# ML200/RoyalTracer-DX

Hardware: AMD Instinct MI355X
Metric: Mrays/s + ms/frame at 1080p, 8-bounce Cornell Box (higher is better)
Workload: dtype f32; 1 GPU; cornell_1080p_64spp_8b; scene=generated: Cornell Box (32 triangles, 2 emissive), width=1920, height=1080, spp=64, max_bounces=8, nee_samples=1, rr_start=3, flags=1, triangles=32, parallelism=pixel-tiles/1, tile_size=64

## Files before the change

### include/rtx.h

```cpp
#ifndef RTX_H
#define RTX_H
#include <stdint.h>
#include <stddef.h>

#ifdef __cplusplus
extern "C" {
#endif

#define RTX_OK               0
#define RTX_ERR_INVALID     -1
#define RTX_ERR_NO_DEVICE   -2
#define RTX_ERR_HIP         -3
#define RTX_ERR_STATE       -4
#define RTX_ERR_OOM         -5

typedef struct rtx_ctx rtx_ctx;

typedef struct rtx_params {
    uint32_t width, height;
    uint32_t spp;
    uint32_t sample_base;
    uint32_t max_bounces;
    uint32_t nee_samples;
    uint32_t rr_start;
// ... 17 lines not shown
typedef struct rtx_stats {
    uint64_t rays_primary, rays_extension, rays_shadow;
    uint64_t paths;
    double   kernel_ms[RTX_K_COUNT];
    uint64_t kernel_launches[RTX_K_COUNT];
    uint64_t kernel_items[RTX_K_COUNT];
    double   render_ms;
    uint32_t bvh_nodes, triangles, lights, materials;
    uint64_t primary_hits;
    uint32_t bvh_refits, bvh_refs;
    uint64_t restir_stale_history_reads;
} rtx_stats;

enum { RTX_OPT_KERNEL_TIMING = 1,
       RTX_OPT_PATHS_PER_BATCH = 2,
       RTX_OPT_SORT_MATERIALS = 3,
       RTX_OPT_LDS_NODES = 4,
       RTX_OPT_SMALL_SCENE = 5,
       RTX_OPT_FUSED_BOUNCE = 6,
       RTX_OPT_BOUNCE_VARIANT = 7,
       RTX_OPT_REFILL_MIN = 8,
       RTX_OPT_STACK_PRIVATE = 9,
       RTX_OPT_TRACE_SCHED = 10,
       RTX_OPT_GPU_REFIT = 11,
       RTX_OPT_RESTIR_WAVEFRONT = 19,
       RTX_OPT_OCCLUDER_CACHE = 21,
       RTX_OPT_SHADE_DENSE = 23,
       RTX_OPT_RESTIR_LANES = 22,
       RTX_OPT_RESTIR_LANE_MIN = 29,
       RTX_OPT_RESTIR_CHUNKS = 20,
       RTX_OPT_OVERLAP_SHADOW = 18,
       RTX_OPT_COMPACT_STATE = 16,
       RTX_OPT_WORK_STEALING = 15,
       RTX_OPT_FUSED_BVH = 14,
       RTX_OPT_LPT_ORDER = 13,
       RTX_OPT_TAPER = 25,
       RTX_OPT_MERGE_RAYS = 24,
       RTX_OPT_OCTANT_SORT = 32,
       RTX_OPT_PARTIAL_REFIT = 37,
       RTX_OPT_LDS_NODES_CLOSEST = 36,
       RTX_OPT_RESTIR_KEYS = 35,
       RTX_OPT_NODE_STRIDE = 34,
       RTX_OPT_SAMPLE_INTERLEAVE = 33,
       RTX_OPT_ASYNC = 31,
       RTX_OPT_TRACE_COUNTERS = 30,
       RTX_OPT_BVH_REINSERT = 26,
       RTX_OPT_BVH_SPLIT = 27,
       RTX_OPT_ANYHIT_ORDER = 28,
       RTX_OPT_GPU_BUILD = 38,
       RTX_OPT_DEFORM_REBUILD = 40,
       RTX_OPT_STACK_CAP = 39,
       RTX_OPT_SHARED_PRIMARY = 41,
       RTX_OPT_DENOISE_LDS_STEP = 42,
       RTX_OPT_BLOCKS_PER_CU = 12     };

int  rtx_create(int device_ordinal, rtx_ctx** out);
void rtx_destroy(rtx_ctx*);
const char* rtx_last_error(rtx_ctx*);
int  rtx_set_option(rtx_ctx*, int option, int64_t value);
int  rtx_set_stream(rtx_ctx*, void* hip_stream);

int  rtx_set_materials(rtx_ctx*, const void* mats128, uint32_t count);
int  rtx_add_mesh(rtx_ctx*, const void* verts28, uint32_t nverts, const uint32_t* indices, uint32_t nidx,
                  const uint32_t* material_ids, uint32_t* mesh_out);
int  rtx_add_instance(rtx_ctx*, uint32_t mesh, const float o2w[16], uint32_t* inst_out);
int  rtx_set_instance_transform(rtx_ctx*, uint32_t inst, const float o2w[16]);
int  rtx_set_instance_visible(rtx_ctx*, uint32_t inst, int visible);
int  rtx_update_mesh_vertices(rtx_ctx*, uint32_t mesh, const void* verts28, uint32_t nverts);
#define RTX_TEX_SRGB 1u
enum { RTX_MAP_KD = 0, RTX_MAP_OPACITY = 2 };
enum { RTX_MAP_NORMAL = 4 };
int  rtx_set_mesh_uvs(rtx_ctx*, uint32_t mesh, const float* uv2 , uint32_t nidx);
int  rtx_set_texture(rtx_ctx*, uint32_t tex , const void* rgba8, uint32_t width, uint32_t height, uint32_t flags);
int  rtx_set_material_map(rtx_ctx*, uint32_t material, uint32_t slot, int32_t tex );
int  rtx_debug_texture_sample(rtx_ctx*, uint32_t tex, const float* uv2, uint32_t n, float* out4);
int  rtx_debug_albedo(rtx_ctx*, const float* rays8, const float* hits4, uint32_t n, float* out4);
int  rtx_debug_opacity(rtx_ctx*, const float* hits4, uint32_t n, float* out2);
int  rtx_debug_shading_normal(rtx_ctx*, const float* rays8, const float* hits4, uint32_t n, float* out4);
int  rtx_debug_tri_tangents(rtx_ctx*, uint32_t first, uint32_t count, float* out6);
#define RTX_ENV_HIDDEN 1u
int  rtx_set_environment(rtx_ctx*, const float* rgb32f , uint32_t n, const float env_to_world[16] , float scale, uint32_t flags);
int  rtx_debug_env_sample(rtx_ctx*, const uint32_t* seeds2, uint32_t n, float* out12);
int  rtx_debug_env_eval(rtx_ctx*, const float* dirs3, uint32_t n, float* out8);
int  rtx_debug_env_tables(rtx_ctx*, float* texels4, float* marginal, float* conditional);
int  rtx_commit_scene(rtx_ctx*);
int  rtx_save_scene_cache(rtx_ctx*, const char* path);
int  rtx_load_scene_cache(rtx_ctx*, const char* path);
int  rtx_set_camera(rtx_ctx*, const float view[16], const float proj[16]);
typedef struct rtx_lens {
    float    aperture_radius;
    float    focus_distance;
    uint32_t reserved[2];
} rtx_lens;
int  rtx_set_lens(rtx_ctx*, const rtx_lens* );
int  rtx_focus_distance_at(rtx_ctx*, uint32_t width, uint32_t height, uint32_t x, uint32_t y, float* distance_out);

int  rtx_bind_accum(rtx_ctx*, void* device_rgba32f, size_t bytes);
int  rtx_clear_accum(rtx_ctx*, uint32_t width, uint32_t height);
int  rtx_render(rtx_ctx*, const rtx_params*);
typedef struct rtx_adaptive {
    uint32_t min_spp, step_spp, max_spp;
    float    threshold, dark_floor;
    uint32_t reserved[3];
} rtx_adaptive;
typedef struct rtx_adaptive_result {
    uint32_t passes;
// ... 73 lines not shown
```

### include/rtx_host.h

```cpp
#ifndef RTX_HOST_H
#define RTX_HOST_H
#include "rtx.h"
#ifdef __cplusplus
extern "C" {
#endif

typedef struct rtxh_scene rtxh_scene;

rtxh_scene* rtxh_scene_cornell(void);
rtxh_scene* rtxh_scene_sponza_class(uint32_t target_tris, uint32_t seed);
rtxh_scene* rtxh_scene_bistro_class(uint32_t target_tris, uint32_t seed);
rtxh_scene* rtxh_scene_sponza_class_hard(uint32_t target_tris, uint32_t seed);
rtxh_scene* rtxh_scene_bistro_class_hard(uint32_t target_tris, uint32_t seed);
rtxh_scene* rtxh_scene_from_obj(const char* const* files, uint32_t nfiles, const char* mtl_dir);
#define RTXH_OBJ_NO_TEXTURES 1u
#define RTXH_OBJ_NO_CUTOUTS  2u
#define RTXH_OBJ_KD_ALPHA    4u
#define RTXH_OBJ_NO_NORMAL_MAPS  8u
#define RTXH_OBJ_BUMP_AS_NORMAL 16u
#define RTXH_OBJ_NORMAL_FLIP_Y  32u
rtxh_scene* rtxh_scene_from_obj_ex(const char* const* files, uint32_t nfiles, const char* mtl_dir, uint32_t flags);
rtxh_scene* rtxh_scene_from_obj_ex2(const char* const* files, uint32_t nfiles, const char* mtl_dir, uint32_t flags, float bump_height);
int         rtxh_scene_save(const rtxh_scene*, const char* path);
rtxh_scene* rtxh_scene_load(const char* path);
void        rtxh_scene_free(rtxh_scene*);
const char* rtxh_last_error(void);

uint32_t    rtxh_scene_num_materials(const rtxh_scene*);
const void* rtxh_scene_materials(const rtxh_scene*);
#define RTXH_NUM_MAP_SLOTS 13
enum { RTXH_MAP_KA = 0, RTXH_MAP_KD, RTXH_MAP_KS, RTXH_MAP_KE, RTXH_MAP_NS, RTXH_MAP_BUMP, RTXH_MAP_D, RTXH_MAP_DISP, RTXH_MAP_REFL, RTXH_MAP_PR, RTXH_MAP_PM, RTXH_MAP_PS, RTXH_MAP_NORM };
typedef struct rtxh_material_ext { float Ni, Ns, Pcr, aniso, anisor; int32_t illum; float Ka[3], Tf[3]; int32_t map[RTXH_NUM_MAP_SLOTS]; } rtxh_material_ext;
int         rtxh_scene_material_ext(const rtxh_scene*, uint32_t material, rtxh_material_ext* out);
uint32_t    rtxh_scene_num_textures(const rtxh_scene*);
const char* rtxh_scene_texture(const rtxh_scene*, uint32_t i);
int         rtxh_scene_texture_pixels(const rtxh_scene*, uint32_t i, const void** rgba8, uint32_t* width, uint32_t* height);
int         rtxh_scene_opacity_map(const rtxh_scene*, uint32_t material);
int         rtxh_scene_normal_map(const rtxh_scene*, uint32_t material);
int         rtxh_scene_mesh_uvs(const rtxh_scene*, uint32_t i, const float** uv2, uint32_t* nidx);
int         rtxh_read_image(const char* path, void* rgba8, uint64_t capacity, uint32_t* width, uint32_t* height);
int         rtxh_read_hdr_image(const char* path, float* rgb32f, uint64_t capacity, uint32_t* width, uint32_t* height);
int         rtxh_env_from_latlong(const float* rgb32f, uint32_t width, uint32_t height, uint32_t n, float* out);
uint32_t    rtxh_scene_num_meshes(const rtxh_scene*);
int         rtxh_scene_mesh(const rtxh_scene*, uint32_t i, const void** verts28, uint32_t* nverts,
                            const uint32_t** indices, uint32_t* nidx, const uint32_t** material_ids);
uint32_t    rtxh_scene_num_instances(const rtxh_scene*);
int         rtxh_scene_instance(const rtxh_scene*, uint32_t i, uint32_t* mesh, float o2w[16]);
uint64_t    rtxh_scene_num_triangles(const rtxh_scene*);
int         rtxh_scene_set_mesh_vertices(rtxh_scene*, uint32_t mesh, const void* verts28, uint32_t nverts);
int         rtxh_scene_camera(const rtxh_scene*, float eye[3], float center[3], float up[3], float* fovy_deg, float* zn, float* zf);
int         rtxh_scene_set_camera(rtxh_scene*, const float eye[3], const float center[3], const float up[3]);
int         rtxh_scene_view_proj(const rtxh_scene*, float aspect, float view[16], float proj[16]);
int         rtxh_scene_upload(const rtxh_scene*, rtx_ctx*, float aspect);

void rtxh_lookat(const float eye[3], const float center[3], const float up[3], float view16[16]);
void rtxh_perspective_fov_rh(float fovy_rad, float aspect, float zn, float zf, float proj16[16]);
void rtxh_generate_ess_lut(float roughness, float lut16[16]);
void rtxh_mat4_inverse(const float m16[16], float out16[16]);
float rtxh_half_round(float x);
int  rtxh_bvh_check(const float* world_tris9, uint32_t ntris, uint32_t* nodes_out, uint32_t* depth_out, uint32_t* max_leaf_out);
int  rtxh_bvh8_check(const float* world_tris9, uint32_t ntris, uint32_t* nodes8_out, uint32_t* stack_out);
int  rtxh_bvh8_stats(const float* world_tris9, uint32_t ntris, uint32_t hist[6], uint32_t* nodes8_out);
int  rtxh_bvh_option(const char* key, double value);
int  rtxh_bvh_replay(const float* world_tris9, uint32_t ntris, const float* rays8, uint32_t nrays, int any, uint32_t any_order, float* out4, uint32_t* refs_out);
int  rtxh_bvh_refit_check(const float* before_tris9, const float* after_tris9, uint32_t ntris);

int  rtxh_scene_small_records(const rtxh_scene*, float* recs20, int32_t* tri_ids2, uint32_t max_recs, uint32_t* nrec_out, float* delta_out, float* cm_out);
int  rtxh_scene_small_occluders(const rtxh_scene*, uint32_t* nocc_out);
int  rtxh_scene_anyhit_order(const rtxh_scene*, uint32_t* order_out);

typedef struct rtxh_renderer rtxh_renderer;
rtxh_renderer* rtxh_renderer_create(uint32_t width, uint32_t height, const char* name, int device);
int  rtxh_renderer_set_scene(rtxh_renderer*, const rtxh_scene*);
rtx_params* rtxh_renderer_params(rtxh_renderer*);
int  rtxh_renderer_set_mode(rtxh_renderer*, int mode);
rtx_params* rtxh_renderer_restir_params(rtxh_renderer*);
rtx_ctx* rtxh_renderer_context(rtxh_renderer*);
int  rtxh_renderer_on_init(rtxh_renderer*);
int  rtxh_renderer_on_update(rtxh_renderer*);
int  rtxh_renderer_set_instance_transform(rtxh_renderer*, uint32_t instance, const float o2w[16]);
int  rtxh_renderer_set_instance_visible(rtxh_renderer*, uint32_t instance, int visible);
int  rtxh_renderer_set_mesh_vertices(rtxh_renderer*, uint32_t mesh, const void* verts28, uint32_t nverts);
int  rtxh_renderer_on_render(rtxh_renderer*);
int  rtxh_renderer_read_accum(rtxh_renderer*, float* rgba32f, size_t bytes);
int  rtxh_renderer_read_output(rtxh_renderer*, uint8_t* rgba8, size_t bytes);
int  rtxh_renderer_on_key_up(rtxh_renderer*, uint8_t key);
uint32_t rtxh_renderer_display_layer(const rtxh_renderer*);
void rtxh_renderer_destroy(rtxh_renderer*);

int  rtxh_write_png(const char* path, const uint8_t* rgba8, uint32_t width, uint32_t height);
int  rtxh_write_ppm(const char* path, const uint8_t* rgba8, uint32_t width, uint32_t height);
int  rtxh_write_exr(const char* path, const float* rgba32f_accum, uint32_t width, uint32_t height);

#ifdef __cplusplus
}
#endif
#endif
```

### royaltracer-dx_amd/__init__.py

```python
import ctypes as C
import os
import numpy as np

_HERE = os.path.dirname(os.path.abspath(__file__))
LIB_PATH = os.environ.get("RTX_LIB_PATH") or os.path.join(_HERE, "librtx_hip.so")

if not os.path.exists(LIB_PATH):
    raise ImportError(
        f"{LIB_PATH} is missing: build it with `make -C {_HERE}` (hipcc --offload-arch=gfx950) "
        "or `python -c 'import __graft_entry__ as g; g.build()'`.  There is no CPU fallback.")

if os.environ.get("RTX_NO_TORCH_PRELOAD", "0") != "1":
    try:
        import torch
    except Exception:
        pass

lib = C.CDLL(LIB_PATH)

RTX_OK = 0
FLAG_LAMBERT_ONLY = 1
FLAG_JITTER = 2
FLAG_TRANSMISSION = 4
FLAG_BLOCK_TILES = 8
K_RAYGEN, K_TRACE, K_SHADE, K_SHADOW, K_ACCUM, K_SORT, K_BOUNCE, K_ADAPT, K_COUNT = 0, 1, 2, 3, 4, 5, 6, 7, 8
KERNEL_NAMES = {K_RAYGEN: "raygen", K_TRACE: "trace_closest", K_SHADE: "shade", K_SHADOW: "trace_shadow", K_ACCUM: "accumulate", K_SORT: "sort", K_BOUNCE: "bounce_fused", K_ADAPT: "adaptive"}
OPT_KERNEL_TIMING, OPT_PATHS_PER_BATCH, OPT_SORT_MATERIALS, OPT_LDS_NODES, OPT_SMALL_SCENE, OPT_FUSED_BOUNCE, OPT_BOUNCE_VARIANT = 1, 2, 3, 4, 5, 6, 7
OPT_REFILL_MIN, OPT_STACK_PRIVATE, OPT_TRACE_SCHED, OPT_GPU_REFIT, OPT_BLOCKS_PER_CU, OPT_LPT_ORDER, OPT_FUSED_BVH, OPT_WORK_STEALING, OPT_COMPACT_STATE, OPT_OVERLAP_SHADOW = 8, 9, 10, 11, 12, 13, 14, 15, 16, 18
OPT_RESTIR_WAVEFRONT, OPT_RESTIR_CHUNKS, OPT_OCCLUDER_CACHE, OPT_RESTIR_LANES, OPT_SHADE_DENSE, OPT_MERGE_RAYS, OPT_TAPER = 19, 20, 21, 22, 23, 24, 25
OPT_BVH_REINSERT, OPT_BVH_SPLIT, OPT_ANYHIT_ORDER, OPT_RESTIR_LANE_MIN, OPT_TRACE_COUNTERS, OPT_ASYNC, OPT_OCTANT_SORT, OPT_SAMPLE_INTERLEAVE, OPT_NODE_STRIDE, OPT_RESTIR_KEYS, OPT_LDS_NODES_CLOSEST, OPT_PARTIAL_REFIT = 26, 27, 28, 29, 30, 31, 32, 33, 34, 35, 36, 37
OPT_GPU_BUILD = 38
OPT_STACK_CAP = 39
OPT_DEFORM_REBUILD = 40
OPT_SHARED_PRIMARY = 41
OPT_DENOISE_LDS_STEP = 42
TEX_SRGB = 1
MAP_KD = 0
MAP_OPACITY = 2
MAP_NORMAL = 4
ENV_HIDDEN = 1


class RtxError(RuntimeError):
    pass


class Params(C.Structure):
    _fields_ = [(n, C.c_uint32) for n in (
        "width", "height", "spp", "sample_base", "max_bounces", "nee_samples", "rr_start",
        "frame_seed", "flags", "tile_size", "shard_rank", "shard_count")]

    def __init__(self, width=1920, height=1080, spp=1, sample_base=1, max_bounces=8, nee_samples=1,
                 rr_start=3, frame_seed=1, flags=0, tile_size=64, shard_rank=0, shard_count=1):
        super().__init__(width, height, spp, sample_base, max_bounces, nee_samples, rr_start,
                         frame_seed, flags, tile_size, shard_rank, shard_count)

    def copy(self, **kw):
        d = {n: getattr(self, n) for n, _ in self._fields_}
        d.update(kw)
        return Params(**d)


class Stats(C.Structure):
    _fields_ = [("rays_primary", C.c_uint64), ("rays_extension", C.c_uint64), ("rays_shadow", C.c_uint64),
                ("paths", C.c_uint64), ("kernel_ms", C.c_double * K_COUNT), ("kernel_launches", C.c_uint64 * K_COUNT),
                ("kernel_items", C.c_uint64 * K_COUNT), ("render_ms", C.c_double),
                ("bvh_nodes", C.c_uint32), ("triangles", C.c_uint32), ("lights", C.c_uint32), ("materials", C.c_uint32),
                ("primary_hits", C.c_uint64), ("bvh_refits", C.c_uint32), ("bvh_refs", C.c_uint32), ("restir_stale_history_reads", C.c_uint64)]

    @property
    def rays(self):
        return self.rays_primary + self.rays_extension + self.rays_shadow


_vp, _u32, _fp = C.c_void_p, C.c_uint32, C.POINTER(C.c_float)
_u32p = C.POINTER(C.c_uint32)


def _sig(name, restype, *argtypes):
    f = getattr(lib, name)
    f.restype = restype
    f.argtypes = list(argtypes)
    return f


_sig("rtx_create", C.c_int, C.c_int, C.POINTER(_vp))
_sig("rtx_destroy", None, _vp)
_sig("rtx_last_error", C.c_char_p, _vp)
# ... 98 lines not shown
_sig("rtxh_scene_bistro_class", _vp, _u32, _u32)
_sig("rtxh_scene_sponza_class_hard", _vp, _u32, _u32)
_sig("rtxh_scene_bistro_class_hard", _vp, _u32, _u32)
_sig("rtxh_scene_from_obj", _vp, C.POINTER(C.c_char_p), _u32, C.c_char_p)
_sig("rtxh_scene_from_obj_ex", _vp, C.POINTER(C.c_char_p), _u32, C.c_char_p, _u32)
_sig("rtxh_scene_opacity_map", C.c_int, _vp, _u32)
_sig("rtxh_scene_from_obj_ex2", _vp, C.POINTER(C.c_char_p), _u32, C.c_char_p, _u32, C.c_float)
_sig("rtxh_scene_normal_map", C.c_int, _vp, _u32)
_sig("rtxh_scene_free", None, _vp)
_sig("rtxh_scene_save", C.c_int, _vp, C.c_char_p)
_sig("rtxh_scene_load", _vp, C.c_char_p)
_sig("rtxh_last_error", C.c_char_p)
_sig("rtxh_scene_num_materials", _u32, _vp)
_sig("rtxh_scene_materials", _vp, _vp)
class MaterialExt(C.Structure):
    _fields_ = [("Ni", C.c_float), ("Ns", C.c_float), ("Pcr", C.c_float), ("aniso", C.c_float), ("anisor", C.c_float), ("illum", C.c_int32),
                ("Ka", C.c_float * 3), ("Tf", C.c_float * 3), ("map", C.c_int32 * 13)]


MAP_SLOTS = ("Ka", "Kd", "Ks", "Ke", "Ns", "bump", "d", "disp", "refl", "Pr", "Pm", "Ps", "norm")
_sig("rtxh_scene_material_ext", C.c_int, _vp, _u32, C.POINTER(MaterialExt))
_sig("rtxh_scene_num_textures", _u32, _vp)
_sig("rtxh_scene_texture", C.c_char_p, _vp, _u32)
_sig("rtxh_scene_texture_pixels", C.c_int, _vp, _u32, C.POINTER(_vp), _u32p, _u32p)
_sig("rtxh_scene_mesh_uvs", C.c_int, _vp, _u32, C.POINTER(_vp), _u32p)
_sig("rtxh_read_image", C.c_int, C.c_char_p, _vp, C.c_uint64, _u32p, _u32p)
_sig("rtxh_read_hdr_image", C.c_int, C.c_char_p, _vp, C.c_uint64, _u32p, _u32p)
_sig("rtxh_env_from_latlong", C.c_int, _vp, _u32, _u32, _u32, _vp)
_sig("rtxh_scene_num_meshes", _u32, _vp)
_sig("rtxh_scene_mesh", C.c_int, _vp, _u32, C.POINTER(_vp), _u32p, C.POINTER(_vp), _u32p, C.POINTER(_vp))
_sig("rtxh_scene_num_instances", _u32, _vp)
_sig("rtxh_scene_instance", C.c_int, _vp, _u32, _u32p, _fp)
_sig("rtxh_scene_num_triangles", C.c_uint64, _vp)
_sig("rtxh_scene_camera", C.c_int, _vp, _fp, _fp, _fp, _fp, _fp, _fp)
_sig("rtxh_scene_view_proj", C.c_int, _vp, C.c_float, _fp, _fp)
_sig("rtxh_scene_upload", C.c_int, _vp, _vp, C.c_float)
_sig("rtxh_lookat", None, _fp, _fp, _fp, _fp)
_sig("rtxh_perspective_fov_rh", None, C.c_float, C.c_float, C.c_float, C.c_float, _fp)
_sig("rtxh_generate_ess_lut", None, C.c_float, _fp)
_sig("rtxh_mat4_inverse", None, _fp, _fp)
_sig("rtxh_half_round", C.c_float, C.c_float)
_sig("rtxh_bvh_check", C.c_int, _vp, _u32, _u32p, _u32p, _u32p)
_sig("rtxh_bvh_refit_check", C.c_int, _vp, _vp, _u32)
_sig("rtxh_bvh8_check", C.c_int, _vp, _u32, _u32p, _u32p)
_sig("rtxh_bvh8_stats", C.c_int, _vp, _u32, _vp, _u32p)
_sig("rtxh_bvh_option", C.c_int, C.c_char_p, C.c_double)
_sig("rtxh_bvh_replay", C.c_int, _vp, _u32, _vp, _u32, C.c_int, _u32, _vp, _u32p)
_sig("rtxh_scene_small_occluders", C.c_int, _vp, _u32p)
_sig("rtxh_scene_anyhit_order", C.c_int, _vp, _u32p)
_sig("rtxh_write_png", C.c_int, C.c_char_p, _vp, _u32, _u32)
_sig("rtxh_write_ppm", C.c_int, C.c_char_p, _vp, _u32, _u32)
_sig("rtxh_write_exr", C.c_int, C.c_char_p, _vp, _u32, _u32)
_sig("rtxh_scene_small_records", C.c_int, _vp, _vp, _vp, _u32, _u32p, _fp, _fp)
_sig("rtxh_scene_set_camera", C.c_int, _vp, _fp, _fp, _fp)
_sig("rtxh_scene_set_mesh_vertices", C.c_int, _vp, _u32, _vp, _u32)
_sig("rtxh_renderer_set_mesh_vertices", C.c_int, _vp, _u32, _vp, _u32)
_sig("rtxh_renderer_create", _vp, _u32, _u32, C.c_char_p, C.c_int)
_sig("rtxh_renderer_set_scene", C.c_int, _vp, _vp)
_sig("rtxh_renderer_params", C.POINTER(Params), _vp)
_sig("rtxh_renderer_restir_params", C.POINTER(Params), _vp)
_sig("rtxh_renderer_set_mode", C.c_int, _vp, C.c_int)
_sig("rtxh_renderer_context", _vp, _vp)
_sig("rtxh_renderer_on_init", C.c_int, _vp)
_sig("rtxh_renderer_on_update", C.c_int, _vp)
_sig("rtxh_renderer_set_instance_transform", C.c_int, _vp, _u32, _vp)
_sig("rtxh_renderer_set_instance_visible", C.c_int, _vp, _u32, C.c_int)
_sig("rtxh_renderer_on_render", C.c_int, _vp)
_sig("rtxh_renderer_read_accum", C.c_int, _vp, _vp, C.c_size_t)
_sig("rtxh_renderer_read_output", C.c_int, _vp, _vp, C.c_size_t)
_sig("rtxh_renderer_on_key_up", C.c_int, _vp, C.c_uint8)
_sig("rtxh_renderer_display_layer", _u32, _vp)
_sig("rtxh_renderer_destroy", None, _vp)


def _f32(a):
    return np.ascontiguousarray(a, dtype=np.float32)


def _ptr(a):
    return a.ctypes.data_as(_vp)


def _fptr(a):
    return a.ctypes.data_as(_fp)


class Scene:

    def __init__(self, handle):
        if not handle:
            raise RtxError("scene creation failed: " + lib.rtxh_last_error().decode())
        self._h = handle
        n = lib.rtxh_scene_num_materials(handle)
        buf = (C.c_float * (n * 32)).from_address(lib.rtxh_scene_materials(handle)) if n else []
        self.materials = np.array(buf, dtype=np.float32).reshape(n, 32)
        self.textures = [lib.rtxh_scene_texture(handle, i).decode() for i in range(lib.rtxh_scene_num_textures(handle))]
        self.material_ext = []
        for i in range(n):
            x = MaterialExt()
            if lib.rtxh_scene_material_ext(handle, i, C.byref(x)) != RTX_OK:
                break
            self.material_ext.append(dict(Ni=x.Ni, Ns=x.Ns, Pcr=x.Pcr, aniso=x.aniso, anisor=x.anisor, illum=x.illum, Ka=list(x.Ka), Tf=list(x.Tf),
                                          maps={MAP_SLOTS[k]: self.textures[x.map[k]] for k in range(13) if x.map[k] >= 0}))
        self.texture_pixels = []
        for i in range(len(self.textures)):
            px, tw, th = _vp(), _u32(), _u32()
# ... 50 lines not shown
        if bump is not None and bump != "normal":
            return cls(lib.rtxh_scene_from_obj_ex2(arr, len(files), mtl_dir.encode(), flags, float(bump)))
        return cls(lib.rtxh_scene_from_obj_ex(arr, len(files), mtl_dir.encode(), flags))

    def set_camera(self, eye, center, up=(0.0, 1.0, 0.0)):
        e, c, u = (np.asarray(v, np.float32) for v in (eye, center, up))
        lib.rtxh_scene_set_camera(self._h, _fptr(e), _fptr(c), _fptr(u))
        self.eye, self.center, self.up = e, c, u

    def set_mesh_vertices(self, mesh, verts):
        v = _f32(verts).reshape(-1, 7)
        if lib.rtxh_scene_set_mesh_vertices(self._h, int(mesh), _ptr(v), len(v)) != RTX_OK:
            raise RtxError("rtxh_scene_set_mesh_vertices failed: " + lib.rtxh_last_error().decode())
        old = self.meshes[mesh]
        self.meshes[mesh] = (v.copy(), old[1], old[2])
        self.cache_path = None

    def bounds(self):
        lo, hi = np.full(3, np.inf, np.float32), np.full(3, -np.inf, np.float32)
        for mesh, m in self.instances:
            v = self.meshes[mesh][0][:, :3]
            if len(v):
                M = np.asarray(m, np.float32).reshape(4, 4)
                w = v @ M[:3, :3] + M[3, :3]
                lo, hi = np.minimum(lo, w.min(0)), np.maximum(hi, w.max(0))
        return lo, hi

    def frame_bounds(self):
        lo, hi = self.bounds()
        c, ext = (lo + hi) * 0.5, hi - lo
        ax = 0 if ext[0] >= ext[2] else 2
        eye, ctr = c.copy(), c.copy()
        eye[1] = ctr[1] = lo[1] + 0.4 * ext[1]
        eye[ax] = c[ax] - 0.35 * ext[ax]
        self.set_camera(eye, ctr)

    def save(self, path):
        if lib.rtxh_scene_save(self._h, str(path).encode()) != RTX_OK:
            raise RtxError("rtxh_scene_save failed: " + lib.rtxh_last_error().decode())

    @classmethod
    def load(cls, path):
        s = cls(lib.rtxh_scene_load(str(path).encode()))
        s.cache_path = str(path)
        return s

    def small_records(self):
        recs, ids = np.zeros((64, 20), np.float32), np.zeros((64, 2), np.int32)
        n, d, cm = _u32(), C.c_float(), C.c_float()
        if lib.rtxh_scene_small_records(self._h, _ptr(recs), _ptr(ids), 64, C.byref(n), C.byref(d), C.byref(cm)) != RTX_OK or n.value == 0:
            return None
        return recs[:n.value], ids[:n.value], d.value, cm.value

    def small_occluders(self):
        n = _u32()
        if lib.rtxh_scene_small_occluders(self._h, C.byref(n)) != RTX_OK:
            raise RtxError("rtxh_scene_small_occluders failed")
        return n.value

    def anyhit_order(self):
        n = _u32()
        if lib.rtxh_scene_anyhit_order(self._h, C.byref(n)) != RTX_OK:
            raise RtxError("rtxh_scene_anyhit_order failed")
        return n.value

    def view_proj(self, aspect):
        v, p = np.zeros(16, np.float32), np.zeros(16, np.float32)
        lib.rtxh_scene_view_proj(self._h, C.c_float(aspect), _fptr(v), _fptr(p))
        return v, p


def lookat(eye, center, up):
    e, c, u, v = _f32(eye), _f32(center), _f32(up), np.zeros(16, np.float32)
    lib.rtxh_lookat(_fptr(e), _fptr(c), _fptr(u), _fptr(v))
    return v


def perspective_fov_rh(fovy_rad, aspect, zn, zf):
    p = np.zeros(16, np.float32)
    lib.rtxh_perspective_fov_rh(fovy_rad, aspect, zn, zf, _fptr(p))
    return p


def generate_ess_lut(roughness):
    lut = np.zeros(16, np.float32)
    lib.rtxh_generate_ess_lut(roughness, _fptr(lut))
    return lut


def mat4_inverse(m):
    m, o = _f32(m).reshape(16), np.zeros(16, np.float32)
    lib.rtxh_mat4_inverse(_fptr(m), _fptr(o))
    return o


def half_round(x):
    return lib.rtxh_half_round(C.c_float(x))


def read_image(path):
    w, h = _u32(), _u32()
    if lib.rtxh_read_image(str(path).encode(), None, 0, C.byref(w), C.byref(h)) != RTX_OK:
        raise RtxError("read_image: " + lib.rtxh_last_error().decode())
    out = np.zeros((h.value, w.value, 4), np.uint8)
    lib.rtxh_read_image(str(path).encode(), _ptr(out), out.nbytes, C.byref(w), C.byref(h))
    return out
# ... 579 lines not shown
```

### royaltracer-dx_amd/csrc/rtx_api.hip

```cpp
#include "rtx_ctx.hpp"
#include <cmath>

thread_local std::string g_create_err;

void options_to_scene(rtx_ctx* c, bool committed) {
    DevScene& s = c->dsc; const rtx_ctx::Options& o = c->opt;
    s.trace_cnt = o.trace_counters ? (unsigned long long*)c->d_trace_cnt.p : nullptr;
    s.refill_min = o.refill_min; s.trace_sched = o.trace_sched; s.sort_materials = o.sort_materials; s.occluder_cache = o.occluder_cache; s.shade_dense = o.shade_dense > 0 ? 1u : 0u;
    if (committed) {
        s.any_order = o.any_order_opt < 0 ? c->scene.built.any_order : (uint32_t)o.any_order_opt;
        s.any_order_occ = o.any_order_opt < 0 ? 0u : (uint32_t)o.any_order_opt;
    }
}

int render_checks(rtx_ctx* c, const rtx_params* p, bool zero_bounces_ok, DevFrame& f) {
    BIND(c);
    if (!c->committed) { c->err = "render: scene not committed"; return RTX_ERR_STATE; }
    if (!c->camera_set) { c->err = "render: camera not set"; return RTX_ERR_STATE; }
    const int r = make_frame(c, p, f);
    if (r) return r;
    if (zero_bounces_ok) {
        if (p->max_bounces > 64 || p->nee_samples > 16) { c->err = "params: max_bounces <= 64, nee_samples <= 16"; return RTX_ERR_INVALID; }
        return RTX_OK;
    }
    if (p->max_bounces == 0 || p->max_bounces > 64) { c->err = "params: max_bounces must be in [1, 64]"; return RTX_ERR_INVALID; }
    if (p->nee_samples > 16) { c->err = "params: nee_samples must be <= 16"; return RTX_ERR_INVALID; }
    return RTX_OK;
}
void stats_begin(rtx_ctx* c) {
    memset(c->stats.kernel_ms, 0, sizeof(c->stats.kernel_ms));
    memset(c->stats.kernel_launches, 0, sizeof(c->stats.kernel_launches));
    memset(c->stats.kernel_items, 0, sizeof(c->stats.kernel_items));
    c->stats.rays_primary = c->stats.rays_extension = c->stats.rays_shadow = c->stats.paths = c->stats.primary_hits = 0; c->stats.render_ms = 0;
    c->ev.used = 0; c->timed.clear();
}

int ensure_accum(rtx_ctx* c, uint32_t w, uint32_t h, bool clear) {
    const size_t need = (size_t)w * h * 16;
    if (c->ext_accum) {
        if (c->ext_accum_bytes < need) { c->err = "bound accumulation buffer is smaller than width*height*16 bytes"; return RTX_ERR_INVALID; }
    } else {
        const bool fresh = !c->d_accum.p || c->acc_w != w || c->acc_h != h;
        HIPCHK(c, c->d_accum.ensure(need));
        clear = clear || fresh;
    }
    c->acc_w = w; c->acc_h = h;
    if (clear) { HIPCHK(c, hipMemsetAsync(c->accum_ptr(), 0, need, c->stream)); c->ad.pure = true; c->ad.cleared = true; }
    return RTX_OK;
}

static void block_grid(uint64_t TX, uint64_t TY, uint32_t N, uint32_t& gx, uint32_t& gy) {
    double best = 1e300; gx = N; gy = 1;
    for (uint32_t a = 1; a <= N; a++) {
        if (N % a) continue;
        const uint32_t b = N / a;
        const double cost = (double)((TX + a - 1) / a) + (double)((TY + b - 1) / b);
        if (cost < best) { best = cost; gx = a; gy = b; }
    }
}
const char* validate_tiling(const rtx_params* p, uint32_t& ts, uint32_t& cnt, uint64_t& npl, uint32_t* gx_out, uint32_t* gy_out) {
    if (!p || !p->width || !p->height) return "params: width/height must be non-zero";
    ts = p->tile_size ? p->tile_size : 64;
    if (ts < 16 || ts > 1024 || (ts & (ts - 1))) return "params: tile_size must be a power of two in [16, 1024] (0 = 64)";
    cnt = p->shard_count ? p->shard_count : 1;
// ... 43 lines not shown
    if (e != hipSuccess || n <= 0) {
        g_create_err = std::string("no HIP device: ") + (e != hipSuccess ? hipGetErrorString(e) : "device count is 0") +
                       " (this library has no CPU fallback)";
        return RTX_ERR_NO_DEVICE;
    }
    if (device_ordinal < 0 || device_ordinal >= n) { g_create_err = "device ordinal out of range"; return RTX_ERR_NO_DEVICE; }
    if ((e = hipSetDevice(device_ordinal)) != hipSuccess) { g_create_err = hipGetErrorString(e); return RTX_ERR_NO_DEVICE; }
    rtx_ctx* c = new rtx_ctx();
    c->device = device_ordinal;
    hipDeviceProp_t prop;
    if (hipGetDeviceProperties(&prop, device_ordinal) == hipSuccess) c->num_cus = prop.multiProcessorCount;
    if ((e = c->streams.acquire(device_ordinal)) != hipSuccess) {
        g_create_err = hipGetErrorString(e); delete c; return RTX_ERR_HIP;
    }
    c->stream = c->streams.set.s[0]; c->own_stream = true;
    (void)hipEventCreate(&c->ev.begin); (void)hipEventCreate(&c->ev.end);
    *out = c;
    return RTX_OK;
}

void rtx_destroy(rtx_ctx* c) {
    if (!c) return;
    (void)hipSetDevice(c->device);
    if (c->own_stream && c->stream) (void)hipStreamSynchronize(c->stream);
    else (void)hipDeviceSynchronize();
    delete c;
}

const char* rtx_last_error(rtx_ctx* c) { return c ? c->err.c_str() : g_create_err.c_str(); }

int rtx_set_option(rtx_ctx* c, int option, int64_t value) {
    if (!c) return RTX_ERR_INVALID;
    switch (option) {
    case RTX_OPT_KERNEL_TIMING: c->opt.timing = value != 0; return RTX_OK;
    case RTX_OPT_ASYNC: c->opt.async = value != 0; return RTX_OK;
    case RTX_OPT_OCTANT_SORT: c->opt.octant_sort = (int)value; return RTX_OK;
    case RTX_OPT_NODE_STRIDE: if (value != 0 && value != 80 && value != 128) { c->err = "node stride must be 0 (auto), 80 or 128"; return RTX_ERR_INVALID; } if (c->opt.node_stride != (int)value) { c->opt.node_stride = (int)value; c->committed = false; } return RTX_OK;
    case RTX_OPT_RESTIR_KEYS: c->opt.restir_keys = value != 0; return RTX_OK;
    case RTX_OPT_SAMPLE_INTERLEAVE: c->opt.sample_interleave = value != 0; return RTX_OK;
    case RTX_OPT_TRACE_COUNTERS:
        c->opt.trace_counters = value != 0;
        if (c->opt.trace_counters) { HIPCHK(c, c->d_trace_cnt.ensure(4 * sizeof(unsigned long long))); HIPCHK(c, hipMemsetAsync(c->d_trace_cnt.p, 0, 32, c->stream)); }
        options_to_scene(c, c->committed);
        return RTX_OK;
    case RTX_OPT_BVH_REINSERT: if (value < 0 || value > 16) { c->err = "bvh_reinsert must be in [0, 16]"; return RTX_ERR_INVALID; } c->host.bvh.reinsert_passes = (int)value; c->host.topo_dirty = true; c->committed = false; return RTX_OK;
    case RTX_OPT_BVH_SPLIT: if (value < 0 || value > 1000000000) { c->err = "bvh_split must be in [0, 1e9] (parts per billion of the scene's surface area)"; return RTX_ERR_INVALID; } c->host.bvh.split_alpha = (double)value * 1e-9; c->host.topo_dirty = true; c->committed = false; return RTX_OK;
    case RTX_OPT_ANYHIT_ORDER: if (value < -1 || value > 2) { c->err = "anyhit_order must be -1 (probe), 0, 1 or 2"; return RTX_ERR_INVALID; } c->opt.any_order_opt = (int)value; options_to_scene(c, c->committed); return RTX_OK;
    case RTX_OPT_PATHS_PER_BATCH: if (value < 4096) { c->err = "paths_per_batch must be >= 4096"; return RTX_ERR_INVALID; } c->opt.paths_per_batch = (uint64_t)value; return RTX_OK;
    case RTX_OPT_SORT_MATERIALS: c->opt.sort_materials = value != 0; options_to_scene(c, c->committed); return RTX_OK;
    case RTX_OPT_LDS_NODES: c->opt.lds_nodes_opt = (int)value; c->committed = false; return RTX_OK;
    case RTX_OPT_PARTIAL_REFIT: c->opt.partial_refit = value != 0; return RTX_OK;
    case RTX_OPT_LDS_NODES_CLOSEST: c->opt.lds_closest_opt = (int)value; if (c->committed) pick_lds_closest(c); return RTX_OK;
    case RTX_OPT_SMALL_SCENE: c->opt.small_scene = value != 0; c->committed = false; return RTX_OK;
    case RTX_OPT_FUSED_BOUNCE: c->opt.fused = value != 0; return RTX_OK;
    case RTX_OPT_BOUNCE_VARIANT: c->opt.bounce_variant = value == 2 ? 2 : (value != 0 ? 1 : 0); return RTX_OK;
    case RTX_OPT_SHARED_PRIMARY: c->opt.shared_primary = value != 0; return RTX_OK;
    case RTX_OPT_STACK_PRIVATE: c->opt.stack_private = (int)value; c->committed = false; return RTX_OK;
    case RTX_OPT_LPT_ORDER: c->opt.lpt_order = value != 0; return RTX_OK;
    case RTX_OPT_FUSED_BVH: c->opt.fused_bvh = value != 0; return RTX_OK;
    case RTX_OPT_WORK_STEALING: c->opt.work_stealing = value != 0; return RTX_OK;
    case RTX_OPT_COMPACT_STATE: c->opt.compact_state = value != 0; return RTX_OK;
    case RTX_OPT_OVERLAP_SHADOW: c->opt.overlap_shadow = value != 0; return RTX_OK;
    case RTX_OPT_BLOCKS_PER_CU: if (value < 0 || value > 64) { c->err = "blocks_per_cu must be in [0, 64]"; return RTX_ERR_INVALID; } c->opt.blocks_per_cu = (uint32_t)value; return RTX_OK;
    case RTX_OPT_TAPER: if (value < 0 || value > 8) { c->err = "taper must be in [0, 8]"; return RTX_ERR_INVALID; } c->opt.taper = value != 0; c->opt.taper_levels = value == 1 ? 4u : (uint32_t)std::max<long long>(value, 1); return RTX_OK;
    case RTX_OPT_MERGE_RAYS: if (value < 0 || value > (1 << 20)) { c->err = "merge_rays must be in [0, 2^20]"; return RTX_ERR_INVALID; } c->opt.merge_rays = (uint32_t)value; return RTX_OK;
    case RTX_OPT_GPU_REFIT: c->opt.gpu_refit = value != 0; return RTX_OK;
    case RTX_OPT_GPU_BUILD: c->opt.gpu_build = value != 0; return RTX_OK;
    case RTX_OPT_DEFORM_REBUILD: if (value < 0 || value > 1000000) { c->err = "deform_rebuild must be 0 (refit), 1 (rebuild) or a percentage >= 2"; return RTX_ERR_INVALID; } c->opt.deform_rebuild = (int)value; return RTX_OK;
    case RTX_OPT_STACK_CAP: if (value < 0 || value > 30 || (value > 0 && value < 4)) { c->err = "stack_cap must be 0 (the whole stack in LDS) or in [4, 30]"; return RTX_ERR_INVALID; } c->opt.stack_cap = (uint32_t)value; c->committed = false; return RTX_OK;
    case RTX_OPT_SHADE_DENSE: c->opt.shade_dense = (int)value; options_to_scene(c, c->committed); return RTX_OK;
    case RTX_OPT_OCCLUDER_CACHE: c->opt.occluder_cache = value != 0; options_to_scene(c, c->committed); return RTX_OK;
    case RTX_OPT_RESTIR_WAVEFRONT: c->opt.restir_wave = value != 0; return RTX_OK;
    case RTX_OPT_RESTIR_LANE_MIN: if (value < 256 || value > (1ll << 31)) { c->err = "restir_lane_min must be in [256, 2^31]"; return RTX_ERR_INVALID; } c->opt.restir_lane_min = (uint32_t)value; return RTX_OK;
    case RTX_OPT_RESTIR_LANES: if (value < 1 || value > 4) { c->err = "restir_lanes must be in [1, 4]"; return RTX_ERR_INVALID; } c->opt.restir_lanes = (uint32_t)value; return RTX_OK;
    case RTX_OPT_RESTIR_CHUNKS: if (value < 1 || value > 64) { c->err = "restir_chunks must be in [1, 64]"; return RTX_ERR_INVALID; } c->opt.restir_chunks = (uint32_t)value; return RTX_OK;
    case RTX_OPT_TRACE_SCHED: if (value > 7) { c->err = "trace_sched must be in [0, 7]"; return RTX_ERR_INVALID; } c->opt.trace_sched = (uint32_t)value; options_to_scene(c, c->committed); return RTX_OK;
    case RTX_OPT_REFILL_MIN: if (value < 1 || value > 64) { c->err = "refill_min must be in [1, 64]"; return RTX_ERR_INVALID; } c->opt.refill_min = (uint32_t)value; options_to_scene(c, c->committed); return RTX_OK;
    case RTX_OPT_DENOISE_LDS_STEP: if (value != 0 && value != 1 && value != 2 && value != 4) { c->err = "denoise_lds_step must be 0, 1, 2 or 4"; return RTX_ERR_INVALID; } c->dn.lds_step = (uint32_t)value; return RTX_OK;
    default: c->err = "unknown option"; return RTX_ERR_INVALID;
    }
}

int rtx_set_stream(rtx_ctx* c, void* s) {
    BIND(c);
    if (c->own_stream && c->stream) HIPCHK(c, hipStreamSynchronize(c->stream));
    else HIPCHK(c, hipDeviceSynchronize());
    if (c->own_stream) { c->stream = nullptr; c->own_stream = false; }
    if (s) { c->stream = (hipStream_t)s; c->own_stream = false; }
    else { c->stream = c->streams.set.s[0]; c->own_stream = true; }
    return RTX_OK;
}

int rtx_set_materials(rtx_ctx* c, const void* mats128, uint32_t count) {
    if (!c) return RTX_ERR_INVALID;
    if (!c->host.set_materials(mats128, count)) { c->err = c->host.err; return RTX_ERR_INVALID; }
    c->committed = false; return RTX_OK;
}
int rtx_add_mesh(rtx_ctx* c, const void* verts28, uint32_t nverts, const uint32_t* indices, uint32_t nidx, const uint32_t* material_ids, uint32_t* mesh_out) {
    if (!c) return RTX_ERR_INVALID;
    if (!c->host.add_mesh(verts28, nverts, indices, nidx, material_ids, mesh_out)) { c->err = c->host.err; return RTX_ERR_INVALID; }
    c->committed = false; return RTX_OK;
}
int rtx_add_instance(rtx_ctx* c, uint32_t mesh, const float o2w[16], uint32_t* inst_out) {
    if (!c || !o2w) return RTX_ERR_INVALID;
    if (!c->host.add_instance(mesh, o2w, inst_out)) { c->err = c->host.err; return RTX_ERR_INVALID; }
    c->committed = false; return RTX_OK;
// ... 151 lines not shown
```

### royaltracer-dx_amd/csrc/rtx_commit.hip

```cpp
#include "rtx_ctx.hpp"

void pick_lds_closest(rtx_ctx* c) {
    DevScene& s = c->dsc;
    c->scene.lds_nodes_closest = 0;
    const bool small_tree = (size_t)s.nnodes * sizeof(Node8GPU) <= ((size_t)16 << 20);
    if (!s.nsmall && s.nnodes > s.lds_nodes && c->opt.lds_nodes_opt < 0 && (c->opt.lds_closest_opt >= 0 || small_tree)) {
        auto fit1k = [&](uint32_t nodes) { DevScene t = s; t.lds_nodes = nodes; return (160u * 1024u) / (uint32_t)((trace_lds_bytes(t) + 64 + 1023) & ~(size_t)1023); };
        uint32_t n = c->opt.lds_closest_opt >= 0 ? std::min<uint32_t>((uint32_t)c->opt.lds_closest_opt, s.nnodes) : std::min<uint32_t>(73u, s.nnodes);
        if (c->opt.lds_closest_opt < 0) while (n > s.lds_nodes && fit1k(n) < 6u) n--;
        DevScene t = s; t.lds_nodes = n;
        if (n > s.lds_nodes && trace_lds_bytes(t) <= 64 * 1024) c->scene.lds_nodes_closest = n;
    }
}

extern "C" {

static int upload_lights(rtx_ctx* c) {
    const BuiltScene& B = c->scene.built;
    std::vector<float>& cdf = c->scene.h_cdf;
    cdf.resize(B.lights.size());
    for (size_t i = 0; i < cdf.size(); i++) cdf[i] = B.lights[i].cdf;
    int r = upload(c, c->scene.d_lights, B.lights);
    if (r) return r;
    return upload(c, c->scene.d_cdf, cdf);
}
static int upload_built(rtx_ctx* c) {
    BuiltScene& B = c->scene.built;
    int r;
    if ((r = upload(c, c->scene.d_nodes, B.nodes8))) return r;
    if ((r = upload(c, c->scene.d_tris, B.tris8))) return r;
    c->scene.n_nodes8 = (uint32_t)B.nodes8.size(); c->scene.n_tris8 = (uint32_t)B.tris8.size(); c->scene.dev_built = false;
    if (!B.nodes8.empty()) c->scene.root8 = B.nodes8[0]; else memset(&c->scene.root8, 0, sizeof(c->scene.root8));
    if ((r = upload(c, c->scene.d_shade, B.shade))) return r;
    if ((r = upload(c, c->scene.d_small, B.small_recs))) return r;
    if ((r = upload(c, c->scene.d_small_tris, B.small_tris))) return r;
    if ((r = upload(c, c->scene.d_small_poly, B.small_poly))) return r;
    if ((r = upload(c, c->scene.d_mats, B.mats))) return r;
    if ((r = upload(c, c->scene.d_insts, B.insts))) return r;
    return upload_lights(c);
}
static int finalise_scene(rtx_ctx* c);

static void fill_tex_lut(std::vector<float>& lut) {
    lut.resize(768);
    for (int b = 0; b < 256; b++) {
        lut[512 + b] = std::max(((float)b - 128.0f) / 127.0f, -1.0f);
        lut[b] = (float)b / 255.0f;
        const double cs = b / 255.0;
        lut[256 + b] = (float)(cs <= 0.04045 ? cs / 12.92 : pow((cs + 0.055) / 1.055, 2.4));
    }
}
static int sync_textures(rtx_ctx* c, bool renumbered, bool deformed) {
    SceneHost& H = c->host; rtx_ctx::Scene& S = c->scene;
    S.built.maps_active = H.maps_active();
    const bool cut = S.built.cutouts_active = H.cutouts_active();
    const bool nrm = S.built.normals_active = H.normals_active();
    const bool active = S.built.maps_active || cut || nrm;
    int r;
    if (H.tex_dirty) {
        std::vector<TexDesc> desc(H.textures.size()); std::vector<uint32_t> pool;
        for (size_t i = 0; i < H.textures.size(); i++) {
            const TexHost& t = H.textures[i];
            desc[i] = TexDesc{(uint32_t)pool.size(), t.width, t.height, t.flags};
            pool.insert(pool.end(), t.rgba.begin(), t.rgba.end());
        }
        std::vector<int32_t> maps(H.mats128.size() / 32, -1);
        for (size_t m = 0; m < maps.size() && m < H.map_kd.size(); m++) maps[m] = H.map_kd[m];
        if ((r = upload(c, S.d_tex_desc, desc)) || (r = upload(c, S.d_texels, pool)) || (r = upload(c, S.d_map_kd, maps))) return r;
        if (!H.any_normal_map()) S.d_map_nrm.release();
        else {
            std::vector<int32_t> nmaps(H.mats128.size() / 32, -1);
            for (size_t m = 0; m < nmaps.size() && m < H.map_normal.size(); m++) nmaps[m] = H.map_normal[m];
            if ((r = upload(c, S.d_map_nrm, nmaps))) return r;
        }
        if (!S.d_tex_lut.p) { std::vector<float> lut; fill_tex_lut(lut); if ((r = upload(c, S.d_tex_lut, lut))) return r; }
        S.ntex = (uint32_t)desc.size();
    }
    if (active && (H.tex_dirty || renumbered || !S.tri_uv_valid)) {
        std::vector<float> uv; H.fill_tri_uv(uv);
        if ((r = upload(c, S.d_tri_uv, uv))) return r;
        S.tri_uv_valid = true;
    }
    if (!active && S.tri_uv_valid) { S.d_tri_uv.release(); S.tri_uv_valid = false; }
    if (cut && (H.tex_dirty || renumbered || !S.tri_cut_valid)) {
        std::vector<int32_t> tc; H.fill_tri_cut(tc);
        if ((r = upload(c, S.d_tri_cut, tc))) return r;
        S.tri_cut_valid = true;
    }
    if (!cut && S.tri_cut_valid) { S.d_tri_cut.release(); S.tri_cut_valid = false; }
// ... 195 lines not shown
    for (uint32_t ord = 1; ord < 3u; ord++) if (cost[ord] < 0.95 * cost[0] && cost[ord] < cost[best_out]) best_out = ord;
    return RTX_OK;
}

static int refit_resident(rtx_ctx* c, bool deform) {
    BuiltScene& B = c->scene.built;
    int r;
    if (deform && (r = ensure_cost_baseline(c, nullptr))) return r;
    const bool mats_changed = c->host.mats_dirty;
    if (!c->host.refresh_transforms(B)) { c->err = c->host.err; return RTX_ERR_INVALID; }
    if (mats_changed && (r = upload(c, c->scene.d_mats, B.mats))) return r;
    if ((r = upload(c, c->scene.d_insts, B.insts))) return r;
    if ((r = upload_lights(c))) return r;
    if ((r = upload_objtris_once(c))) return r;
    if (deform) {
        if ((r = reflatten_dirty_meshes(c))) return r;
        if (!c->scene.dev_built) { B.objtris.clear(); B.objtris.shrink_to_fit(); c->scene.host_mirror_stale = true; }
    }
    HIPCHK(c, c->scene.d_node_aabb.ensure((size_t)c->scene.n_nodes8 * 32));
    size_t nmoved = 0; for (uint32_t m : B.inst_moved) nmoved += m;
    const bool partial = c->opt.partial_refit && c->scene.node_aabb_valid && B.inst_moved.size() == B.insts.size() && nmoved < B.insts.size();
    if (!partial) return full_refit(c);
    if ((r = upload(c, c->scene.d_inst_moved, B.inst_moved))) return r;
    if ((r = upload_hidden(c))) return r;
    HIPCHK(c, c->scene.d_tri_dirty.ensure(c->scene.n_tris8)); HIPCHK(c, c->scene.d_node_dirty.ensure(c->scene.n_nodes8));
    launch_refit(c->stream, (Node8GPU*)c->scene.d_nodes.p, B.level_start8.data(), (uint32_t)B.level_start8.size() - 1, (TriGPU*)c->scene.d_tris.p, c->scene.n_tris8,
                 (const TriShade*)c->scene.d_shade.p, (const InstGPU*)c->scene.d_insts.p, (const F4*)c->scene.d_objtris.p, (F4*)c->scene.d_node_aabb.p, (uint32_t*)c->scene.d_scale.p,
                 (const uint32_t*)c->scene.d_inst_moved.p, (uint8_t*)c->scene.d_tri_dirty.p, (uint8_t*)c->scene.d_node_dirty.p, hidden_words(c));
    HIPCHK(c, hipGetLastError());
    return RTX_OK;
}

static int build_and_upload(rtx_ctx* c) {
    BuiltScene& B = c->scene.built;
    int r;
    c->scene.device_scene_valid = false; c->scene.objtris_uploaded = false; c->scene.node_aabb_valid = false; c->scene.host_mirror_stale = false;
    size_t ntri_all = 0; for (const InstHost& in : c->host.insts) ntri_all += c->host.meshes[in.mesh].idx.size() / 3;
    const bool on_gpu = c->opt.gpu_build && ntri_all > 4096u && c->host.bvh.split_alpha <= 0.0;
    if (!(on_gpu ? c->host.prepare_device_build(B) : c->host.build(B))) { c->err = c->host.err; return RTX_ERR_INVALID; }
    if (!on_gpu) {
        if ((r = upload_built(c))) return r;
        if (B.any_hidden && c->scene.n_nodes8 && B.level_start8.size() >= 2) {
            if ((r = upload_objtris_once(c))) return r;
            if ((r = full_refit(c))) return r;
            TO_HOST(c, &c->scene.root8, c->scene.d_nodes.p, sizeof(Node8GPU));
        }
        return RTX_OK;
    }
    const uint32_t nt = B.built_tris;
    if ((r = upload(c, c->scene.d_mats, B.mats))) return r;
    if ((r = upload(c, c->scene.d_insts, B.insts))) return r;
    if ((r = upload_lights(c))) return r;
    if ((r = flatten_on_device(c, nt))) return r; c->scene.objtris_uploaded = true;
    for (DevBuf* b : {&c->scene.d_small, &c->scene.d_small_tris, &c->scene.d_small_poly}) HIPCHK(c, b->ensure(16));
    HIPCHK(c, c->scene.d_tris.ensure((size_t)nt * sizeof(TriGPU)));
    if (!c->scene.builder) c->scene.builder.reset(new GpuBvhBuilder());
    BvhBuildOptions bo = c->host.bvh; if (bo.ploc_radius <= 0) bo.ploc_radius = 16;
    const std::string e = c->scene.builder->build(c->stream, (const F4*)c->scene.d_objtris.p, (const TriShade*)c->scene.d_shade.p, (const InstGPU*)c->scene.d_insts.p, nt, bo, (TriGPU*)c->scene.d_tris.p, c->scene.build_info);
    if (!e.empty()) { c->err = e; return RTX_ERR_HIP; }
    const GpuBuildResult& G = c->scene.build_info;
    HIPCHK(c, c->scene.d_nodes.ensure((size_t)G.nnodes8 * sizeof(Node8GPU)));
    HIPCHK(c, hipMemcpyAsync(c->scene.d_nodes.p, c->scene.builder->nodes(), (size_t)G.nnodes8 * sizeof(Node8GPU), hipMemcpyDeviceToDevice, c->stream));
    c->scene.n_nodes8 = G.nnodes8; c->scene.n_tris8 = G.ntris8; c->scene.dev_built = true; B.bvh_pad = 2e-6f * G.scale;
    B.level_start8 = G.level_start8; B.stack8 = G.stack8;
    if ((r = full_refit(c))) return r;
    if (c->scene.n_nodes8) { if ((r = enqueue_tree_cost(c, c->scene.d_cost_base))) return r; c->scene.cost_base_state = 1; }
    TO_HOST(c, &c->scene.root8, c->scene.d_nodes.p, sizeof(Node8GPU));
    if (getenv("RTX_BUILD_TIMES")) fprintf(stderr, "[build] GPU: prims %.2f ms, sort %.2f ms, PLOC %.2f ms (%u rounds -> %u clusters), top on the host %.2f ms, layout %.2f ms: %u wide nodes, stack %u\n",
                                           G.ms_prims, G.ms_sort, G.ms_ploc, G.ploc_iterations, G.clusters_top, G.ms_top_host, G.ms_layout, G.nnodes8, G.stack8);
    return RTX_OK;
}

int rtx_commit_scene(rtx_ctx* c) {
    BIND(c);
    const bool deform = !c->host.dirty_meshes.empty();
    for (uint32_t m : c->host.dirty_meshes)
        if (m < c->scene.pool_meshes && std::find(c->scene.pool_dirty.begin(), c->scene.pool_dirty.end(), m) == c->scene.pool_dirty.end()) c->scene.pool_dirty.push_back(m);
    if (deform && c->opt.deform_rebuild == 1) c->host.topo_dirty = true;
    if (c->host.topo_dirty || c->host.mats_dirty || !c->scene.committed_once)
        for (size_t i = 0; i < c->host.matids.size(); i++)
            if (c->host.matids[i] >= c->host.mats128.size() / 32) { c->err = "commit: material id out of range"; return RTX_ERR_INVALID; }
    c->scene.committed_once = true;
    int r;
    {   size_t ntri_all = 0; for (const InstHost& in : c->host.insts) ntri_all += c->host.meshes[in.mesh].idx.size() / 3;
        if (c->host.tex_dirty && ntri_all <= kSmallSceneMaxTris && (c->host.maps_active() != c->scene.built.maps_active || c->host.cutouts_active() != c->scene.built.cutouts_active || c->host.normals_active() != c->scene.built.normals_active)) c->host.topo_dirty = true;
        if (c->host.env_dirty && ntri_all <= kSmallSceneMaxTris && (c->host.env.n != 0) != c->scene.built.env_active) c->host.topo_dirty = true; }
    bool build = !(c->opt.gpu_refit && gpu_refittable(c) && !c->host.topo_dirty);
    const BuiltScene& B0 = c->scene.built;
    if (!build && !c->scene.dev_built && !B0.leaf_order.empty() && B0.leaf_order.size() <= kSmallSceneMaxTris && B0.any_hidden && !c->host.any_hidden()) build = true;
    bool flipped = false;
    for (size_t ii = 0; ii < c->host.insts.size() && !flipped; ii++) flipped = (ii < B0.inst_hidden.size() && B0.inst_hidden[ii] != 0u) != c->host.is_hidden(ii);
    const bool tex_only = !build && (c->host.tex_dirty || c->host.env_dirty) && c->host.only_maps_changed(B0);
    const bool probe = (build || !flipped) && !tex_only;
    if (!build && !tex_only) {
        if ((r = refit_resident(c, deform))) return r;
        c->scene.cost_now_state = 0;
        if (deform && c->opt.deform_rebuild >= 2) {
            double cost[2];
            if ((r = tree_costs(c, cost))) return r;
            if (cost[0] * 100.0 > cost[1] * (double)c->opt.deform_rebuild) { c->host.topo_dirty = true; build = true; }
        }
    }
    if (build) {
        c->scene.cost_base_state = c->scene.cost_now_state = 0;
        if ((r = build_and_upload(c))) return r;
    }
    c->host.dirty_meshes.clear();
// ... 5 lines not shown
        if ((r = probe_anyhit_order_on_device(c, best))) return r;
        c->scene.built.any_order = best;
        if (c->opt.any_order_opt < 0) c->dsc.any_order = best;
    }
    return r;
}

int rtx_save_scene_cache(rtx_ctx* c, const char* path) {
    if (!c) return RTX_ERR_INVALID;
    if (!c->committed) { c->err = "save_scene_cache: scene not committed"; return RTX_ERR_STATE; }
    if (c->scene.host_mirror_stale) { c->err = "save_scene_cache: the per-triangle records were re-derived on the GPU after rtx_update_mesh_vertices and the host holds no current copy; commit with RTX_OPT_DEFORM_REBUILD 1 (host builder) to save a cache"; return RTX_ERR_STATE; }
    if (c->scene.built.any_hidden) { c->err = "save_scene_cache: an instance is hidden (rtx_set_instance_visible): the device's boxes and triangle records leave it out and the file format holds no visibility; show every instance and commit to save a cache"; return RTX_ERR_STATE; }
    if (c->host.env.n) { c->err = "save_scene_cache: an environment is bound (rtx_set_environment) and the file format holds no environment; clear it and commit to save a cache"; return RTX_ERR_STATE; }
    if (c->host.any_normal_map()) { c->err = "save_scene_cache: a material has a normal map (rtx_set_material_map, RTX_MAP_NORMAL) and the file format holds no texels; unmap every material and commit to save a cache"; return RTX_ERR_STATE; }
    if (c->host.any_opacity_map()) { c->err = "save_scene_cache: a material has an opacity map (rtx_set_material_map, RTX_MAP_OPACITY) and the file format holds no texels; unmap every material and commit to save a cache"; return RTX_ERR_STATE; }
    if (c->host.any_map()) { c->err = "save_scene_cache: a material has a texture map (rtx_set_material_map) and the file format holds no texels; unmap every material and commit to save a cache"; return RTX_ERR_STATE; }
    if (c->scene.dev_built) { c->err = "save_scene_cache: the tree was built on the GPU (RTX_OPT_GPU_BUILD) and has no host mirror; commit with the host builder to save a cache"; return RTX_ERR_STATE; }
    if (!save_scene_cache(c->host, c->scene.built, path, c->err)) return RTX_ERR_INVALID;
    return RTX_OK;
}
int rtx_load_scene_cache(rtx_ctx* c, const char* path) {
    BIND(c);
    if (!load_scene_cache(path, c->host, c->scene.built, c->err)) return RTX_ERR_INVALID;
    c->committed = false; c->scene.device_scene_valid = false; c->scene.objtris_uploaded = false; c->scene.node_aabb_valid = false;
    c->scene.host_mirror_stale = false; c->scene.cost_base_state = c->scene.cost_now_state = 0;
    c->scene.pool_meshes = 0; c->scene.pool_verts = c->scene.pool_idx = c->scene.pool_matids = 0; c->scene.pool_vert_base.clear(); c->scene.pool_idx_base.clear(); c->scene.pool_dirty.clear();
    int r = upload_built(c);
    if (r) return r;
    c->host.tex_dirty = true;
    if ((r = sync_textures(c, true, false))) return r;
    c->host.env = EnvHost{}; c->host.env_dirty = true;
    if ((r = sync_environment(c))) return r;
    return finalise_scene(c);
}

static int refresh_wide_nodes(rtx_ctx* c) {
    if (!c->scene.wide_nodes || !c->scene.n_nodes8) return RTX_OK;
    HIPCHK(c, c->scene.d_nodes_wide.ensure((size_t)c->scene.n_nodes8 * 128));
    HIPCHK(c, hipMemcpy2DAsync(c->scene.d_nodes_wide.p, 128, c->scene.d_nodes.p, sizeof(Node8GPU), sizeof(Node8GPU), c->scene.n_nodes8, hipMemcpyDeviceToDevice, c->stream));
    return RTX_OK;
}
static int finalise_scene(rtx_ctx* c) {
    BuiltScene& B = c->scene.built;
    HIPCHK(c, hipStreamSynchronize(c->stream));
    c->scene.device_scene_valid = true;
    DevScene& s = c->dsc;
    s.nodes = (const Node8GPU*)c->scene.d_nodes.p; s.nnodes = c->scene.n_nodes8;
    s.nodes_f = (const F4*)c->scene.d_nodes.p; s.node_v4 = 5u;
    c->scene.wide_nodes = s.nnodes && (c->opt.node_stride == 128 || (c->opt.node_stride == 0 && (size_t)s.nnodes * sizeof(Node8GPU) > ((size_t)16 << 20)));
    { const int rw = refresh_wide_nodes(c); if (rw) return rw; }
    if (c->scene.wide_nodes && c->opt.node_stride == 128) { s.nodes_f = (const F4*)c->scene.d_nodes_wide.p; s.node_v4 = 8u; }
    s.tris = (const TriGPU*)c->scene.d_tris.p; s.ntris = c->scene.n_tris8;
    s.shade = (const TriShade*)c->scene.d_shade.p;
    s.small = (const SmallRecPair*)c->scene.d_small.p; s.small_tris = (const TriGPU*)c->scene.d_small_tris.p; s.small_poly = (const F4*)c->scene.d_small_poly.p; s.small_cm = B.small_cm; s.small_delta = B.small_delta;
    s.mats = (const MatGPU*)c->scene.d_mats.p; s.nmat = (uint32_t)B.mats.size();
    s.insts = (const InstGPU*)c->scene.d_insts.p; s.ninst = (uint32_t)B.insts.size();
    s.lights = (const LightGPU*)c->scene.d_lights.p; s.nlights = (uint32_t)B.lights.size(); s.cdf = (const float*)c->scene.d_cdf.p;
    s.total_weight = B.total_weight;
    s.tex_desc = (const TexDesc*)c->scene.d_tex_desc.p; s.ntex = c->scene.ntex; s.texels = (const uint32_t*)c->scene.d_texels.p; s.tex_lut = (const float*)c->scene.d_tex_lut.p;
    s.env_n = c->host.env.n; s.env_flags = c->host.env.flags; memcpy(s.env_rot, c->host.env.rot, sizeof(s.env_rot));
    const bool env_lit = s.env_n && c->scene.env_total > 0.0;
    s.env_tex = env_lit ? (const F4*)c->scene.d_env_tex.p : nullptr; s.env_marg = env_lit ? (const float*)c->scene.d_env_marg.p : nullptr; s.env_cond = env_lit ? (const float*)c->scene.d_env_cond.p : nullptr;
    const bool uv_active = B.maps_active || B.cutouts_active || B.normals_active;
    s.tri_uv = uv_active ? (const float*)c->scene.d_tri_uv.p : nullptr; s.map_kd = uv_active ? (const int32_t*)c->scene.d_map_kd.p : nullptr;
    s.tri_cut = B.cutouts_active ? (const int32_t*)c->scene.d_tri_cut.p : nullptr;
    s.tri_tan = B.normals_active ? (const float*)c->scene.d_tri_tan.p : nullptr; s.map_nrm = B.normals_active ? (const int32_t*)c->scene.d_map_nrm.p : nullptr;
    s.stack_depth = B.stack8;
    s.stack_ovf = nullptr; s.stack_ovf_stride = 0;
    if (c->opt.stack_cap && B.stack8 > c->opt.stack_cap && B.stack8 <= 30) {
        const uint32_t stride = 1u << 22;
        HIPCHK(c, c->scene.d_stack_ovf.ensure((size_t)(B.stack8 - c->opt.stack_cap) * stride * 8));
        s.stack_depth = c->opt.stack_cap; s.stack_ovf = (unsigned long long*)c->scene.d_stack_ovf.p; s.stack_ovf_stride = stride;
    }
    s.stack_private = c->opt.stack_private == 1 ? 1u : 0u;
    if (s.stack_depth > 30) { c->err = "commit: BVH too deep for the traversal stack (more than 30 levels of 8-wide nodes with two or more internal children)"; return RTX_ERR_INVALID; }
    const size_t stack_bytes = (size_t)s.stack_depth * 256 * kStackEntryBytes;
    const size_t hard = 64 * 1024;
    size_t budget = hard > stack_bytes ? hard - stack_bytes : 0;
    uint32_t want_nodes;
    if (c->opt.lds_nodes_opt >= 0) want_nodes = (uint32_t)c->opt.lds_nodes_opt;
    else {
        want_nodes = 73;
    }
    s.lds_nodes = std::min<uint32_t>(std::min<uint32_t>(want_nodes, s.nnodes), (uint32_t)(budget / 80));
    budget -= (size_t)s.lds_nodes * 80;
    uint32_t want_tris = s.ntris <= 256 ? s.ntris : 0u;
    s.lds_tris = (size_t)want_tris * 48 <= budget ? want_tris : 0u;
    s.nsmall = 0; s.nsmall_occ = 0;
    {
        float ext[3] = {1.0f, 1.0f, 1.0f}; uint32_t bits[3] = {0, 0, 0};
        s.cell_o[0] = s.cell_o[1] = s.cell_o[2] = 0.0f;
        if (c->scene.n_nodes8) {
            const Node8GPU& R0 = c->scene.root8;
            s.cell_o[0] = R0.px; s.cell_o[1] = R0.py; s.cell_o[2] = R0.pz;
            for (int a = 0; a < 3; a++) ext[a] = std::max(1e-20f, 255.0f * std::ldexp(1.0f, (int)((R0.e_imask >> (8 * a)) & 0xffu) - 127));
        }
        for (int k = 0; k < 8; k++) { int best = 0; for (int a = 1; a < 3; a++) if (ext[a] / (float)(1u << bits[a]) > ext[best] / (float)(1u << bits[best])) best = a; bits[best]++; }
        for (int a = 0; a < 3; a++) s.cell_s[a] = (float)(1u << bits[a]) / ext[a];
        s.cell_bits = bits[0] | (bits[1] << 4) | (bits[2] << 8);
    }
    options_to_scene(c, true);
    if (c->opt.small_scene && B.small_nrec && B.small_tris.size() * 48 <= budget + (size_t)s.lds_tris * 48) {
        s.nsmall = B.small_nrec; s.nsmall_occ = B.small_nocc; s.lds_tris = (uint32_t)B.small_tris.size();
    }
    if (trace_lds_bytes(s) > 64 * 1024) { c->err = "commit: BVH too deep for the LDS traversal stack"; return RTX_ERR_INVALID; }
    if (c->opt.lds_nodes_opt < 0 && !s.nsmall && s.lds_nodes > 9u) {
        auto fit = [&](uint32_t nodes) { DevScene t = s; t.lds_nodes = nodes; return (160u * 1024u) / (uint32_t)((trace_lds_bytes(t) + 64 + 1023) & ~(size_t)1023); };
// ... 26 lines not shown
```

### royaltracer-dx_amd/csrc/rtx_ctx.hpp

```cpp
#pragma once
#include <hip/hip_runtime.h>
#include <algorithm>
#include <cstdio>
#include <cstdlib>
#include <cstring>
#include <memory>
#include <string>
#include <vector>
#include "../../include/rtx.h"
#include "rtx_kernels.hpp"
#include "rtx_scene_host.hpp"
#include "rtx_build.hpp"
#include "rtx_devmem.hpp"
#include "rtx_staging.hpp"

using namespace rtx;

#pragma GCC visibility push(hidden)

struct TimedLaunch { int cls; hipEvent_t a, b; };

struct rtx_ctx {
    StreamLease streams;
    int device = 0;
    hipStream_t stream = nullptr; bool own_stream = false;
    int num_cus = 256;
    std::string err;
    Staging staging;
    Events ev;
    std::vector<TimedLaunch> timed;
    rtx_stats stats{};

    struct Options {
        bool timing = false;
        bool async = false;
        int octant_sort = 0;
        int node_stride = 0;
        int restir_keys = 1;
        int sample_interleave = 1;
        bool trace_counters = false;
        int any_order_opt = -1;
        uint64_t paths_per_batch = 128u << 20;
        uint32_t sort_materials = 0;
        int lds_nodes_opt = -1;
        int partial_refit = 1;
        int lds_closest_opt = -1;
        bool small_scene = true;
        bool fused = true;
        int bounce_variant = 2;
        bool shared_primary = true;
        int stack_private = -1;
        bool lpt_order = true;
        bool fused_bvh = false;
        bool work_stealing = false;
        bool compact_state = true;
        bool overlap_shadow = true;
        uint32_t blocks_per_cu = 0;
        bool taper = true; uint32_t taper_levels = 4;
        uint32_t merge_rays = 1024;
        bool gpu_refit = true;
        int gpu_build = 0;
        int deform_rebuild = 0;
        uint32_t stack_cap = 11;
        int shade_dense = 0;
        uint32_t occluder_cache = 0;
        bool restir_wave = true;
        uint32_t restir_lane_min = 1u << 16;
        uint32_t restir_lanes = 2;
        uint32_t restir_chunks = 4;
        uint32_t trace_sched = 6;
        uint32_t refill_min = 12;
    } opt;
    DevBuf d_trace_cnt;

    SceneHost host;
    bool committed = false;
    float view[16], proj[16], prev_view[16], prev_proj[16]; bool camera_set = false; DevBuf d_cam;
    rtx_lens lens{};
    DevBuf d_accum; void* ext_accum = nullptr; size_t ext_accum_bytes = 0; uint32_t acc_w = 0, acc_h = 0;
    DevBuf d_srgb;
    F4* accum_ptr() { return (F4*)(ext_accum ? ext_accum : d_accum.p); }

    DevScene dsc{};
    struct Scene {
        BuiltScene built;
        bool committed_once = false;
        DevBuf d_nodes, d_tris, d_small, d_small_tris, d_small_poly, d_shade, d_mats, d_insts, d_lights, d_cdf;
        std::vector<float> h_cdf; std::vector<uint32_t> h_one;
        uint32_t n_nodes8 = 0, n_tris8 = 0; Node8GPU root8{}; bool dev_built = false; std::unique_ptr<GpuBvhBuilder> builder; GpuBuildResult build_info;
        DevBuf d_work_insts; std::vector<FlatInst> h_work; std::vector<uint32_t> pool_dirty;
        bool host_mirror_stale = false;
        DevBuf d_cost_base, d_cost_now; int cost_base_state = 0, cost_now_state = 0; double cost_base = 0.0, cost_now = 0.0;
        DevBuf d_pool_verts, d_pool_idx, d_pool_matids, d_flat_insts; size_t pool_verts = 0, pool_idx = 0, pool_matids = 0, pool_meshes = 0; std::vector<uint32_t> pool_vert_base, pool_idx_base; std::vector<FlatInst> h_flat;
        DevBuf d_inst_hidden;
        DevBuf d_inst_moved, d_tri_dirty, d_node_dirty; bool node_aabb_valid = false;
        DevBuf d_objtris, d_node_aabb, d_scale;
        bool device_scene_valid = false, objtris_uploaded = false;
        DevBuf d_nodes_wide; bool wide_nodes = false;
        uint32_t lds_nodes_closest = 0;
        DevBuf d_stack_ovf;
        DevBuf d_tri_uv, d_map_kd, d_tex_desc, d_texels, d_tex_lut; bool tri_uv_valid = false; uint32_t ntex = 0;
        DevBuf d_tri_cut; bool tri_cut_valid = false;
        DevBuf d_tri_tan, d_map_nrm; bool tri_tan_valid = false;
        DevBuf d_env_tex, d_env_marg, d_env_cond; double env_total = 0.0;
    } scene;

    struct PathFrame {
        DevBuf d_ray_o, d_ray_d, d_thr, d_rad, d_hit, d_sh_o, d_sh_d, d_sh_c, d_queue[2], d_counters;
        DevBuf d_alt_o, d_alt_d, d_alt_thr;
        DevBuf d_hitmask, d_order, d_pmask;
        DevBuf d_prim_rec, d_prim_hits;
        DevBuf d_oct[2], d_perm;
        DevBuf d_hitq;
        DevBuf d_heads;
        PinnedBuf h_counters;
        uint64_t pred_paths = 0; std::vector<uint64_t> pred_q, pred_s; uint32_t pred_nee1 = 0;
        hipStream_t aux = nullptr;
        struct Pending { bool active = false; size_t ncnt = 0; uint32_t nbatches = 0, G = 0, mb = 0, nee = 0, nee1 = 1; bool fused = false, fused_bvh = false; } pending;
    } pt;

    struct Adaptive {
        DevBuf d_half, d_count, d_flag, d_list, d_out;
        bool pure = true;
        bool cleared = true;
        uint32_t key[3] = {0, 0, 0};
    } ad;

    struct Denoise {
        DevBuf d_guides, d_pp[2], d_out, d_partial, d_count;
        uint32_t w = 0, h = 0; bool valid = false;
        Events ev;
        uint32_t lds_step = 4;
    } dn;

    struct Restir {
        DevBuf d_res_di, d_res_gi, d_sdata, d_last_di, d_last_gi, d_last_sd, d_p1cnt, d_p1scratch; size_t p1_slots = 0, last_slots = 0;
        DevBuf d_rs_key_a, d_rs_key_b;
        DevBuf d_halo, d_own; uint32_t halo_count = 0, own_count = 0; uint32_t halo_key[6] = {0, 0, 0, 0, 0, 0};
        uint32_t hist[4] = {0, 0, 0, 0}; bool hist_all = true;
        struct RsArea { DevBuf state, hit, cls, fin, cold, occ, cand, sho, shd, pay, cnt; } rs_area[4];
// ... 44 lines not shown
```

### royaltracer-dx_amd/csrc/rtx_k_bounce_small.hpp

```cpp
#pragma once
#include "rtx_bounce_small_parts.hpp"
#include "rtx_k_bounce_wave.hpp"

namespace rtx {

struct ShadowLds { F4* o; F4* d; uint32_t* n ; uint8_t* occ; };
__device__ __forceinline__ ShadowLds block_shadow_lds() {
    __shared__ F4 s_sho[kBlock], s_shd[kBlock];
    __shared__ uint32_t s_shn[2];
    __shared__ uint8_t s_occ[kBlock];
    if (threadIdx.x < 2) s_shn[threadIdx.x] = 0;
    return {s_sho, s_shd, s_shn, s_occ};
}
__device__ __forceinline__ bool block_shadow(const DevScene& sc, const SmallRecPair* small, const TraceLds& L, const ShadowLds& sh, uint32_t& par, bool push, const F4& so, const F4& sd, uint32_t* s_cnt_j, Prof* pf) {
    const uint32_t slot = block_push(push, &sh.n[par]);
    if (push) { sh.o[slot] = so; sh.d[slot] = sd; }
    __syncthreads();
    PF_MARK(5);
    const uint32_t ns = sh.n[par];
    if ((threadIdx.x & ~63u) < ns) {
        const bool mine = threadIdx.x < ns;
        const F4 ro = mine ? sh.o[threadIdx.x] : F4{0, 0, 0, 0}, rd = mine ? sh.d[threadIdx.x] : F4{0, 0, 1, 0};
        float st_, su_, sv_; uint32_t sprim;
        traverse_small<true>(sc, small, L, mk3(ro.x, ro.y, ro.z), mk3(rd.x, rd.y, rd.z), fabsf(ro.w), mine ? rd.w : 0.0f, st_, su_, sv_, sprim, shadow_records(sc, mine, ro.w), ~0ull, pf, 6);
// ... 68 lines not shown
                if (active) {
                    S.pid = myq[i];
                    const uint32_t sl = __umulhi(S.pid, pin.div_mul) >> pin.div_shift, v = S.pid - sl * f.npl;
                    const uint32_t pl = f.list ? f.list[v >> 8] * (uint32_t)kBlock + (v & 255u) : v;
                    const F4 r0 = pin.rec[pl], r1 = pin.rec[(size_t)pin.npl + pl], r2 = pin.rec[(size_t)2 * pin.npl + pl], ro = pin.rec[(size_t)3 * pin.npl];
                    seed_sample(f2u(r2.w), f2u(r1.w), f.sample_first + sl, f.frame_seed, S.s0, S.s1);
                    S.o = mk3(ro.x, ro.y, ro.z); S.d = mk3(r0.x, r0.y, r0.z); S.thr = mk3(1.0f, 1.0f, 1.0f); S.prev_pdf = 1.0f;
                    sf.pos = mk3(r1.x, r1.y, r1.z); sf.normal = mk3(r2.x, r2.y, r2.z); sf.mat = f2u(r0.w) & 0x7FFFFFFFu; sf.near_hull = (f2u(r0.w) >> 31) != 0u;
                    prim = 0u;
                }
            } else {
                if (active) { S = load_path(p, myq[i]); const F4 h = p.hit[S.pid]; t = h.x; u = h.y; v = h.z; prim = f2u(h.w); }
            }
            PF_MARK(2);
            shade_block<HAVE_HIT, LAMBERT, COMPACT>(sc, small, L, f, p, T, sh, par, S, sf, t, u, v, prim, active, sbounce, nee, last, s_cnt, mynext, state_out((uint32_t)qb, stride, bounce), pf);
        }
        n = end_bounce<false>(s_cnt, nullptr, qrows, srows, bounce, G, qid, nee);
    }
    PF_FLUSH;
}

template <bool LAMBERT, int RING>
__device__ __forceinline__ void bounce_small_block(const DevScene& sc, const SmallRecPair* small, const DevFrame& f_in, const DevPaths& p, uint32_t bounce_first, uint32_t bounce_end,
                                                   uint32_t* queue_a, uint32_t* queue_b, uint32_t* qrows, uint32_t* srows, const uint32_t* order) {
    extern __shared__ F4 lds[];
    __shared__ uint32_t s_cnt[1 + kMaxNee];
    const DevFrame f = frame_with_lambert<LAMBERT>(f_in);
    const uint32_t qid = order ? order[blockIdx.x] : blockIdx.x;
    wave_stamp(0u);
    if (threadIdx.x <= kMaxNee) s_cnt[threadIdx.x] = 0;
    const ShadowLds sh = block_shadow_lds();
    STAGE_SMALL_TABLES(T, sc);
    const uint32_t G = gridDim.x;
    uint32_t n = qrows[(size_t)bounce_first * G + qid];
    const uint32_t nee = sc.nlights ? f.nee_samples : 0u;
    const TraceLds L = stage_lds(sc, lds);
    __syncthreads();
    const size_t qb = (size_t)qid * f.qcap;
    uint32_t par = 0;
    PF_BEGIN;
    for (uint32_t bounce = bounce_first; bounce < bounce_end; bounce++) {
        const bool last = (bounce + 1u == f.max_bounces);
        const float tmin = bounce_tmin(bounce);
        const uint32_t* myq = ((bounce & 1u) ? queue_b : queue_a) + qb;
        uint32_t* mynext = ((bounce & 1u) ? queue_a : queue_b) + qb;
        if constexpr (!RING) {
            for (uint32_t base = 0; base < n; base += kBlock) {
                PF_MARK(0);
                PathState S = idle_path(); Surf sf = idle_surf();
                float t = 0.0f, u = 0.0f, v = 0.0f; uint32_t prim = kMissPrim;
                const uint32_t i = base + threadIdx.x;
                const bool active = i < n;
                if (active) S = load_path(p, myq[i]);
                traverse_small<false>(sc, small, L, S.o, S.d, tmin, active ? kTMax : 0.0f, t, u, v, prim, sc.nsmall, ~0ull, pf, 1);
                PF_MARK(2);
                shade_block<0, LAMBERT, false>(sc, small, L, f, p, T, sh, par, S, sf, t, u, v, prim, active, bounce, nee, last, s_cnt, mynext, 0u, pf);
            }
        } else {
            constexpr uint32_t kRing = 512u;
            __shared__ uint32_t s_rpid[kRing];
            __shared__ F4 s_rhit[kRing];
            __shared__ uint32_t s_ring[1], s_rc[3];
            if (threadIdx.x < 3) s_rc[threadIdx.x] = 0;
            if (threadIdx.x == 3) s_ring[0] = 0;
            __syncthreads();
            uint32_t next_in = 0;
            uint32_t prod = 0, rk = 0;
            for (;;) {
                PF_MARK(0);
                PathState S = idle_path(); Surf sf = idle_surf();
                float t = 0.0f, u = 0.0f, v = 0.0f; uint32_t prim = kMissPrim;
                while (next_in < n && prod - s_ring[0] < kBlock) {
                    const uint32_t i = next_in + threadIdx.x;
                    const bool act = i < n;
                    uint32_t pid = 0; f3 ro = mk3(0, 0, 0), rd = mk3(0, 0, 1);
                    if (act) { pid = myq[i]; const F4 a = p.ray_o[pid], b = p.ray_d[pid]; ro = mk3(a.x, a.y, a.z); rd = mk3(b.x, b.y, b.z); }
                    float ht, hu, hv; uint32_t hp;
                    traverse_small<false>(sc, small, L, ro, rd, tmin, act ? kTMax : 0.0f, ht, hu, hv, hp, sc.nsmall, ~0ull, pf, 1);
                    const bool hit = act && hp != kMissPrim;
                    const uint32_t slot = prod + block_push(hit, &s_rc[rk]);
                    if (hit) { s_rpid[slot & (kRing - 1u)] = pid; s_rhit[slot & (kRing - 1u)] = {ht, hu, hv, u2f(hp)}; }
                    next_in += kBlock;
                    __syncthreads();
                    prod += s_rc[rk];
                    if (threadIdx.x == 0) s_rc[rk == 0u ? 2u : rk - 1u] = 0;
                    rk = rk == 2u ? 0u : rk + 1u;
                }
                const uint32_t head = s_ring[0], avail = prod - head;
                if (avail == 0u) break;
                const uint32_t take = avail < (uint32_t)kBlock ? avail : (uint32_t)kBlock;
                const bool active = threadIdx.x < take;
                if (active) {
                    const uint32_t e = (head + threadIdx.x) & (kRing - 1u);
                    S = load_path(p, s_rpid[e]);
                    const F4 h = s_rhit[e]; t = h.x; u = h.y; v = h.z; prim = f2u(h.w);
                }
                __syncthreads();
                if (threadIdx.x == 0) s_ring[0] = head + take;
                PF_MARK(2);
                shade_block<0, LAMBERT, false>(sc, small, L, f, p, T, sh, par, S, sf, t, u, v, prim, active, bounce, nee, last, s_cnt, mynext, 0u, pf);
                __syncthreads();
            }
        }
        n = end_bounce<false>(s_cnt, nullptr, qrows, srows, bounce, G, qid, nee);
    }
    PF_FLUSH;
    wave_stamp(1u);
}

template <int WAVES, int HAVE_HIT, bool LAMBERT, int RING, bool COMPACT>
__global__ __launch_bounds__(kBlock, WAVES) void k_bounce_small(DevScene sc, const SmallRecPair* __restrict__ small, DevFrame f_in, DevPaths p,
                                                         uint32_t bounce_first, uint32_t bounce_end,
                                                         uint32_t* __restrict__ queue_a, uint32_t* __restrict__ queue_b ,
                                                         uint32_t* __restrict__ qrows ,
                                                         uint32_t* __restrict__ srows ,
                                                         const uint32_t* __restrict__ order ,
                                                         PrimIn pin ) {
    static_assert(HAVE_HIT == 0 || RING == 0, "bounce 0 has no extension trace, hence no ring: launch_bounce_small");
    static_assert(!COMPACT || HAVE_HIT != 0 || RING == 2, "the block-scheduled bodies keep the path state in place: launch_bounce_small");
    if constexpr (HAVE_HIT != 0) bounce_small_first<HAVE_HIT, LAMBERT, COMPACT>(sc, small, f_in, p, bounce_first, bounce_end, queue_a, queue_b, qrows, srows, order, pin);
    else if constexpr (RING == 2) bounce_small_wave<LAMBERT, COMPACT>(sc, small, f_in, p, bounce_first, bounce_end, queue_a, queue_b, qrows, srows, order);
    else bounce_small_block<LAMBERT, RING>(sc, small, f_in, p, bounce_first, bounce_end, queue_a, queue_b, qrows, srows, order);
}

}
```

### royaltracer-dx_amd/csrc/rtx_k_bounce_wave.hpp

```cpp
#pragma once
#include "rtx_bounce_small_parts.hpp"

namespace rtx {

__device__ __forceinline__ void wave_lds_sync() {
    __builtin_amdgcn_fence(__ATOMIC_RELEASE, "wavefront");
    __builtin_amdgcn_wave_barrier();
    __builtin_amdgcn_fence(__ATOMIC_ACQUIRE, "wavefront");
}

template <bool LAMBERT, bool COMPACT>
__device__ __forceinline__ void bounce_small_wave(const DevScene& sc, const SmallRecPair* __restrict__ small, const DevFrame& f_in, const DevPaths& p, uint32_t bounce_first, uint32_t bounce_end,
                                                  uint32_t* __restrict__ queue_a, uint32_t* __restrict__ queue_b, uint32_t* __restrict__ qrows, uint32_t* __restrict__ srows, const uint32_t* __restrict__ order) {
    extern __shared__ F4 lds[];
    constexpr uint32_t kWaves = kBlock / 64u, kHitBuf = 64u, kShBuf = 64u;
    __shared__ uint32_t s_cnt[1 + kMaxNee];
    __shared__ uint32_t s_in;
    __shared__ uint32_t s_hpid[kWaves * kHitBuf];
    __shared__ F4 s_hhit[kWaves * kHitBuf];
    __shared__ F4 s_so[kWaves * kShBuf], s_sd[kWaves * kShBuf], s_sc[kWaves * kShBuf];
    const DevFrame f = frame_with_lambert<LAMBERT>(f_in);
    const uint32_t qid = order ? order[blockIdx.x] : blockIdx.x;
    wave_stamp(0u);
    if (threadIdx.x <= kMaxNee) s_cnt[threadIdx.x] = 0;
// ... 2 lines not shown
    const uint32_t G = gridDim.x;
    uint32_t n = qrows[(size_t)bounce_first * G + qid];
    const uint32_t nee = sc.nlights ? f.nee_samples : 0u;
    const TraceLds L = stage_lds(sc, lds);
    __syncthreads();
    const size_t qb = (size_t)qid * f.qcap;
    const uint32_t stride = COMPACT ? state_set_stride(p) : 0u;
    const uint32_t lane = lane_id();
    const uint32_t wv = (uint32_t)__builtin_amdgcn_readfirstlane((int)(threadIdx.x >> 6));
    uint32_t* const hpid = s_hpid + wv * kHitBuf; F4* const hhit = s_hhit + wv * kHitBuf;
    F4* const sho = s_so + wv * kShBuf; F4* const shd = s_sd + wv * kShBuf; F4* const shc = s_sc + wv * kShBuf;
    PF_BEGIN;
    for (uint32_t bounce = bounce_first; bounce < bounce_end; bounce++) {
        const bool last = (bounce + 1u == f.max_bounces);
        const float tmin = bounce_tmin(bounce);
        const uint32_t* myq = ((bounce & 1u) ? queue_b : queue_a) + qb;
        uint32_t* mynext = ((bounce & 1u) ? queue_a : queue_b) + qb;
        const uint32_t in0 = state_in((uint32_t)qb, stride, bounce), out0 = state_out((uint32_t)qb, stride, bounce);
        uint32_t hcnt = 0;
        uint32_t shcnt = 0;
        bool in_done = false;
        uint32_t scnt = 0;
        auto shadow_block = [&](uint32_t k) {
            wave_lds_sync();
            const bool mine = lane < k;
            const uint32_t e = lane;
            const F4 ro = mine ? sho[e] : F4{0, 0, 0, 0}, rd = mine ? shd[e] : F4{0, 0, 1, 0};
            float st_, su_, sv_; uint32_t sprim;
            traverse_small<true>(sc, small, L, mk3(ro.x, ro.y, ro.z), mk3(rd.x, rd.y, rd.z), fabsf(ro.w), mine ? rd.w : 0.0f, st_, su_, sv_, sprim, shadow_records(sc, mine, ro.w), ~0ull, pf, 6);
            if (mine && sprim == kMissPrim) {
                const F4 c = shc[e];
                const uint32_t pid = f2u(c.w);
                F4 radv = p.rad[pid];
                radv.x = radv.x + c.x; radv.y = radv.y + c.y; radv.z = radv.z + c.z;
                p.rad[pid] = radv;
            }
            wave_lds_sync();
            PF_MARK(8);
        };
        for (;;) {
            PF_MARK(0);
            bool full = false, carry = false;
            uint32_t cpid = 0, cprim = kMissPrim, ce = 0, hnext = 0; float ct = 0.0f, cu = 0.0f, cv = 0.0f;
            while (!in_done && !full) {
                uint32_t c0 = 0;
                if (lane == 0) c0 = atomicAdd(&s_in, 64u);
                c0 = (uint32_t)__builtin_amdgcn_readfirstlane((int)c0);
                if (c0 >= n) { in_done = true; break; }
                const uint32_t i = c0 + lane;
                const bool act = i < n;
                uint32_t pid = 0; f3 ro = mk3(0, 0, 0), rd = mk3(0, 0, 1);
                if (act) { pid = COMPACT ? i : myq[i]; const uint32_t src = COMPACT ? in0 + i : pid; const F4 a = p.ray_o[src], b = p.ray_d[src]; ro = mk3(a.x, a.y, a.z); rd = mk3(b.x, b.y, b.z); }
                float ht, hu, hv; uint32_t hp;
                traverse_small<false>(sc, small, L, ro, rd, tmin, act ? kTMax : 0.0f, ht, hu, hv, hp, sc.nsmall, ~0ull, pf, 1);
                const bool hit = act && hp != kMissPrim;
                const unsigned long long hmask = __ballot(hit);
                const uint32_t e = hcnt + __builtin_amdgcn_mbcnt_hi((uint32_t)(hmask >> 32), __builtin_amdgcn_mbcnt_lo((uint32_t)hmask, 0u));
                if (hit && e < kHitBuf) { hpid[e] = pid; hhit[e] = {ht, hu, hv, u2f(hp)}; }
                const uint32_t tot = hcnt + (uint32_t)__popcll(hmask);
                if (tot >= kHitBuf) { full = true; hnext = tot - kHitBuf; carry = hit && e >= kHitBuf; ce = e - kHitBuf; cpid = pid; ct = ht; cu = hu; cv = hv; cprim = hp; }
                else hcnt = tot;
            }
            const uint32_t take = full ? 64u : hcnt;
            if (take == 0u) break;
            const bool active = lane < take;
            PathState S = idle_path();
            float t = 0.0f, u = 0.0f, v = 0.0f; uint32_t prim = kMissPrim;
            wave_lds_sync();
            if (active) {
                const uint32_t e = hpid[lane];
                S = load_path(p, COMPACT ? in0 + e : e);
                if (COMPACT) S.pid = myq[e];
                const F4 h = hhit[lane]; t = h.x; u = h.y; v = h.z; prim = f2u(h.w);
            }
            wave_lds_sync();
            if (carry) { hpid[ce] = cpid; hhit[ce] = {ct, cu, cv, u2f(cprim)}; }
            hcnt = full ? hnext : 0u;
            PF_MARK(2);
            Surf sf = idle_surf();
            bool shading = false;
            if (active && prim != kMissPrim) { PF_COUNT(3); shading = hit_to_shading<0>(sc, p, T.mats, S, sf, t, u, v, prim, bounce, nee); }
            const f3 outgoing = -S.d, pos = sf.pos;
            const MatGPU* mp = T.mats + (shading ? sf.mat : 0u);
            f3 normal = sf.normal;
            const float eta_p = LAMBERT ? 0.0f : transmission_eta(*mp, f.flags, outgoing, normal);
            PF_MARK(3);
            for (uint32_t j = 0; j < nee; j++) {
                bool push = false;
                F4 so = {0, 0, 0, 0}, sd = {0, 0, 1, 0}; f3 con = mk3(0, 0, 0);
                if (shading) { PF_COUNT(4); push = nee_sample(sc, *mp, f.flags, nee, S, pos, normal, outgoing, so, sd, con, sf.near_hull, eta_p, nullptr, T.cdf, T.lights); }
                PF_MARK(4);
                const unsigned long long pmask = __ballot(push);
                const uint32_t npush = (uint32_t)__popcll(pmask);
                if (lane == j) shcnt += npush;
                const uint32_t e = scnt + __builtin_amdgcn_mbcnt_hi((uint32_t)(pmask >> 32), __builtin_amdgcn_mbcnt_lo((uint32_t)pmask, 0u));
                if (push && e < kShBuf) { sho[e] = so; shd[e] = sd; shc[e] = {con.x, con.y, con.z, u2f(S.pid)}; }
                const uint32_t tot = scnt + npush;
                PF_MARK(5);
                if (tot >= kShBuf) {
                    shadow_block(kShBuf);
                    if (push && e >= kShBuf) { sho[e - kShBuf] = so; shd[e - kShBuf] = sd; shc[e - kShBuf] = {con.x, con.y, con.z, u2f(S.pid)}; }
                    scnt = tot - kShBuf;
                } else scnt = tot;
                if (nee > 1u && scnt) { shadow_block(scnt); scnt = 0; }
            }
            continue_path<COMPACT>(*mp, f, p, bounce, shading && !last, S, pos, normal, outgoing, eta_p, &s_cnt[0], mynext, out0, pf);
            PF_MARK(9);
// ... 11 lines not shown
```

### royaltracer-dx_amd/csrc/rtx_k_raygen.hpp

```cpp
#pragma once
#include "rtx_shade.hpp"

namespace rtx {

template <bool LIST, bool LENS>
__global__ __launch_bounds__(kBlock) void k_raygen(DevFrame f, DevPaths p, const CameraGPU* __restrict__ cam_p, uint32_t* __restrict__ queue, uint32_t* __restrict__ qcount, uint32_t compact) {
    __shared__ CameraGPU cam;
    __shared__ uint32_t s_n;
    stage_camera(cam, cam_p);
    if (threadIdx.x == 0) s_n = 0;
    __syncthreads();
    uint32_t* myq = queue + (size_t)blockIdx.x * f.qcap;
    const uint32_t nchunks = f.chunks_per_sample * f.batch_spp;
    for (uint32_t k = 0, row0 = 0, c; row0 < nchunks; k++) {
        if (!dealt_chunk(f, k, row0, nchunks, c)) continue;
        uint32_t sl = c / f.chunks_per_sample, cl = c - sl * f.chunks_per_sample;
        uint32_t pl = cl * kBlock + threadIdx.x;
        if (f.interleave) {
            const uint32_t sh = f.interleave, S = 1u << sh;
            const uint32_t per = S * f.chunks_per_sample, sg = c / per, r = c - sg * per;
            sl = sg * S + (threadIdx.x & (S - 1u));
            pl = r * (kBlock >> sh) + (threadIdx.x >> sh);
        }
        const uint32_t pid = sl * f.npl + pl;
// ... 11 lines not shown
            myq[slot] = pid;
        }
    }
    __syncthreads();
    if (threadIdx.x == 0) qcount[blockIdx.x] = s_n;
}

__global__ __launch_bounds__(kBlock) void k_packet_masks(DevScene sc, DevFrame f, const CameraGPU* __restrict__ cam_p, unsigned long long* __restrict__ masks) {
    __shared__ CameraGPU cam;
    stage_camera(cam, cam_p);
    __syncthreads();
    const uint32_t blk = blockIdx.x * (kBlock / 64u) + (threadIdx.x >> 6);
    if (blk >= f.npl / 64u) return;
    uint32_t x = 0, y = 0;
    (void)slot_to_pixel(f, blk * 64u, x, y);
    const unsigned long long keep = packet_keep_mask(sc, cam, f, x & ~7u, y & ~7u);
    if (lane_id() == 0) masks[blk] = keep;
}

template <bool LIST, bool LENS>
__global__ __launch_bounds__(kBlock) void k_raygen_trace_small(DevScene sc, const SmallRecPair* __restrict__ small, DevFrame f, DevPaths p, const CameraGPU* __restrict__ cam_p,
                                                               uint32_t* __restrict__ queue, uint32_t* __restrict__ qcount, uint32_t* __restrict__ gencount,
                                                               const unsigned long long* __restrict__ masks ) {
    extern __shared__ F4 lds[];
    __shared__ CameraGPU cam;
    __shared__ uint32_t s_n[2];
    stage_camera(cam, cam_p);
    if (threadIdx.x < 2) s_n[threadIdx.x] = 0;
    const TraceLds L = stage_lds(sc, lds);
    __syncthreads();
    uint32_t* myq = queue + (size_t)blockIdx.x * f.qcap;
    uint32_t generated = 0;
    const uint32_t nchunks = f.chunks_per_sample * f.batch_spp;
    for (uint32_t k = 0, row0 = 0; row0 < nchunks; k++) {
        const uint32_t nk = f.taper_levels ? taper_row_width(k, gridDim.x, f.taper_levels) : gridDim.x;
        uint32_t pos = blockIdx.x;
        if (f.taper_levels && blockIdx.x < nk) { pos += (k * 2654435761u) % nk; if (pos >= nk) pos -= nk; }
        const uint32_t c = row0 + pos;
        row0 += nk;
        if (blockIdx.x >= nk || c >= nchunks) continue;
        const uint32_t sl = c / f.chunks_per_sample, cl = c - sl * f.chunks_per_sample;
        const uint32_t pl = real_slot<LIST>(f, cl * kBlock + threadIdx.x);
        const uint32_t pid = sl * f.npl + cl * kBlock + threadIdx.x;
        uint32_t x = 0, y = 0, s0 = 0, s1 = 0;
        const bool valid = slot_to_pixel(f, pl, x, y);
        f3 o = mk3(0, 0, 0), d = mk3(0, 0, 1);
        if (valid) {
            camera_sample<LENS>(cam, f, x, y, f.sample_first + sl, o, d, s0, s1);
            generated++;
        }
        const unsigned long long km = masks[pl >> 6];
        const unsigned long long keep = ((unsigned long long)(uint32_t)__builtin_amdgcn_readfirstlane((int)(uint32_t)(km >> 32)) << 32) | (uint32_t)__builtin_amdgcn_readfirstlane((int)(uint32_t)km);
        float t, u, v; uint32_t prim;
        traverse_small<false>(sc, small, L, o, d, kTMinCam, valid ? kTMax : 0.0f, t, u, v, prim, sc.nsmall, keep);
        const bool hit = valid && prim != kMissPrim;
        const unsigned long long hm = __ballot(hit);
        if (lane_id() == 0) p.hitmask[pid >> 6] = hm;
        if (hit) {
            if (f.max_bounces == 0u) p.rad[pid] = {0.0f, 0.0f, 0.0f, 0.0f};
            p.ray_o[pid] = {o.x, o.y, o.z, u2f(s1)};
            p.ray_d[pid] = {d.x, d.y, d.z, 1.0f};
            p.thr[pid] = {1.0f, 1.0f, 1.0f, u2f(s0)};
            p.hit[pid] = {t, u, v, u2f(prim)};
        }
        const uint32_t slot = block_push(hit, &s_n[0]);
        if (hit) myq[slot] = pid;
    }
    atomicAdd(&s_n[1], generated);
    __syncthreads();
    if (threadIdx.x == 0) { qcount[blockIdx.x] = s_n[0]; gencount[blockIdx.x] = s_n[1]; }
}

__global__ __launch_bounds__(kBlock) void k_primary_surface(DevScene sc, const SmallRecPair* __restrict__ small, DevFrame f, const CameraGPU* __restrict__ cam_p,
                                                            unsigned long long* __restrict__ masks, unsigned long long* __restrict__ hits, F4* __restrict__ rec) {
    extern __shared__ F4 lds[];
    __shared__ CameraGPU cam;
    stage_camera(cam, cam_p);
    const TraceLds L = stage_lds(sc, lds);
    __syncthreads();
    const uint32_t pl = blockIdx.x * kBlock + threadIdx.x;
    if (pl >= f.npl) return;
    uint32_t x0 = 0, y0 = 0, x = 0, y = 0;
    (void)slot_to_pixel(f, pl & ~63u, x0, y0);
    const unsigned long long keep = packet_keep_mask(sc, cam, f, x0 & ~7u, y0 & ~7u);
    const bool valid = slot_to_pixel(f, pl, x, y);
    f3 o = mk3(0, 0, 0), d = mk3(0, 0, 1);
    if (valid) primary_ray(cam, f.width, f.height, x, y, 0.0f, 0.0f, o, d);
    float t, u, v; uint32_t prim;
    traverse_small<false>(sc, small, L, o, d, kTMinCam, valid ? kTMax : 0.0f, t, u, v, prim, sc.nsmall, keep);
    const bool hit = valid && prim != kMissPrim;
    const unsigned long long hm = __ballot(hit);
    const unsigned long long vm = __ballot(valid);
    if (lane_id() == 0) { masks[pl >> 6] = keep; hits[pl >> 6] = hm; hits[(f.npl >> 6) + (pl >> 6)] = vm; }
    if (pl == 0) rec[(size_t)3 * f.npl] = {cam.viewI[12], cam.viewI[13], cam.viewI[14], 0.0f};
    if (hit) {
        const Surf sf = surface(sc, o, d, t, u, v, prim);
        uint32_t h0, h1; seed_pixel(x, y, h0, h1);
        rec[pl] = {d.x, d.y, d.z, u2f((sf.mat < 0x7FFFFFFFu ? sf.mat : 0x7FFFFFFFu) | (sf.near_hull ? 0x80000000u : 0u))};
        rec[(size_t)f.npl + pl] = {sf.pos.x, sf.pos.y, sf.pos.z, u2f(h1)};
        rec[(size_t)2 * f.npl + pl] = {sf.normal.x, sf.normal.y, sf.normal.z, u2f(h0)};
    }
}

template <bool LIST>
__global__ __launch_bounds__(kBlock) void k_raygen_shared(DevFrame f, uint32_t* __restrict__ queue, uint32_t* __restrict__ qcount, uint32_t* __restrict__ gencount,
                                                          const unsigned long long* __restrict__ hits, uint32_t nblk) {
    __shared__ unsigned long long s_hm[kBlock];
    __shared__ uint32_t s_pid[kBlock], s_off[kBlock], s_wave[4], s_gen;
    if (threadIdx.x == 0) s_gen = 0;
    __syncthreads();
    uint32_t* myq = queue + (size_t)blockIdx.x * f.qcap;
    const uint32_t nchunks = f.chunks_per_sample * f.batch_spp;
    const uint32_t period = f.taper_levels ? 1u << (f.taper_levels - 1u) : 1u;
    uint32_t period_sum = 0;
    for (uint32_t j = 0; j < period; j++) period_sum += deal_width(f, j);
    const uint32_t lane = threadIdx.x & 63u, wave = threadIdx.x >> 6;
    uint32_t generated = 0, qn = 0;
    for (uint32_t k0 = 0; deal_row0(f, k0, period, period_sum) < nchunks; k0 += 64u) {
        const uint32_t k = k0 + (threadIdx.x >> 2);
        uint32_t row0 = deal_row0(f, k, period, period_sum), c;
        const bool dealt = dealt_chunk(f, k, row0, nchunks, c);
        unsigned long long hm = 0ull;
        uint32_t pid0 = 0;
        if (dealt) {
            const uint32_t sl = c / f.chunks_per_sample, cl = c - sl * f.chunks_per_sample;
            const uint32_t v = cl * kBlock + (threadIdx.x & 3u) * 64u;
            const uint32_t blk = real_slot<LIST>(f, v) >> 6;
            hm = hits[blk];
            generated += (uint32_t)__popcll(hits[nblk + blk]);
            pid0 = sl * f.npl + v;
        }
        const uint32_t cnt = (uint32_t)__popcll(hm);
        uint32_t inc = cnt;
        for (uint32_t d = 1; d < 64u; d <<= 1) { const uint32_t y = __shfl_up(inc, d); if (lane >= d) inc += y; }
        if (lane == 63u) s_wave[wave] = inc;
        s_hm[threadIdx.x] = hm; s_pid[threadIdx.x] = pid0;
        __syncthreads();
        uint32_t before = 0, total = 0;
        for (uint32_t w = 0; w < 4u; w++) { const uint32_t t = s_wave[w]; if (w < wave) before += t; total += t; }
        s_off[threadIdx.x] = before + inc - cnt;
        __syncthreads();
        for (uint32_t i = wave; i < (uint32_t)kBlock; i += 4u) {
// ... 15 lines not shown
```

### royaltracer-dx_amd/csrc/rtx_kernels.hpp

```cpp
#pragma once
#include <hip/hip_runtime.h>
#include "rtx_types.hpp"

namespace rtx {

struct DevScene {
    const Node8GPU* nodes;  uint32_t nnodes;
    const F4* nodes_f; uint32_t node_v4;
    const TriGPU*   tris;   uint32_t ntris;
    const TriShade* shade;
    const SmallRecPair* small; uint32_t nsmall;
    uint32_t nsmall_occ;
    const F4* small_poly;
    const TriGPU* small_tris;
    float small_cm, small_delta;
    const MatGPU*   mats;   uint32_t nmat;
    const InstGPU*  insts;  uint32_t ninst;
    const LightGPU* lights; uint32_t nlights;
    const float* cdf;
    float total_weight;
    uint32_t lds_nodes, lds_tris;
    uint32_t stack_depth;
    unsigned long long* stack_ovf; uint32_t stack_ovf_stride;
    uint32_t stack_private;
    uint32_t sort_materials;
    uint32_t refill_min, trace_sched;
    uint32_t shade_dense;
    uint32_t any_order;
    float cell_o[3], cell_s[3]; uint32_t cell_bits;
    uint32_t any_order_occ;
    unsigned long long* trace_cnt;
    uint32_t occluder_cache;
    const float* tri_uv;
    const int32_t* map_kd;
    const TexDesc* tex_desc; uint32_t ntex;
    const uint32_t* texels;
    const float* tex_lut;
    const F4* env_tex;
    const float* env_marg;
    const float* env_cond;
    uint32_t env_n, env_flags;
    float env_rot[9];
    const int32_t* tri_cut;
    const float* tri_tan;
    const int32_t* map_nrm;
};

struct DevFrame {
    uint32_t width, height;
    uint32_t tile_size, tile_shift, tiles_x, tiles_y;
    uint32_t shard_rank, shard_count;
    uint32_t blk_gx, blk_gy;
    uint32_t npl;
    uint32_t batch_spp;
    uint32_t sample_first;
    uint32_t max_bounces, nee_samples, rr_start, frame_seed, flags;
    uint32_t nblocks, qcap, chunks_per_sample;
    uint32_t interleave;
    uint32_t taper_levels;
    uint32_t hist_x0, hist_y0, hist_x1, hist_y1; unsigned long long* hist_stale;
    const uint32_t* list;
    float lens_radius, lens_focus;
};

#if defined(__HIPCC__)
#define RTX_TAPER_HD __host__ __device__ __forceinline__
#else
#define RTX_TAPER_HD inline
#endif
RTX_TAPER_HD uint32_t taper_row_width(uint32_t k, uint32_t G, uint32_t levels) {
    const uint32_t m = k & ((1u << (levels - 1u)) - 1u);
    if (m == 0u) return G;
    uint32_t lg = 0; while ((m >> (lg + 1u)) != 0u) lg++;
    return G - (G >> (levels - 1u - lg));
}
#if defined(__HIPCC__)
#define RTX_TILE_HD __host__ __device__ __forceinline__
#else
#define RTX_TILE_HD inline
#endif
RTX_TILE_HD bool shard_tile(const DevFrame& f, uint32_t k, uint32_t& tx, uint32_t& ty) {
    if (f.blk_gx) {
        const uint32_t bx = f.shard_rank % f.blk_gx, by = f.shard_rank / f.blk_gx;
        const uint32_t tx0 = bx * f.tiles_x / f.blk_gx, tx1 = (bx + 1u) * f.tiles_x / f.blk_gx, ty0 = by * f.tiles_y / f.blk_gy, ty1 = (by + 1u) * f.tiles_y / f.blk_gy;
        const uint32_t bw = (f.tiles_x + f.blk_gx - 1u) / f.blk_gx;
        tx = tx0 + k % bw; ty = ty0 + k / bw;
        return tx < tx1 && ty < ty1;
    }
    const uint32_t t = f.shard_rank + k * f.shard_count;
    if (t >= f.tiles_x * f.tiles_y) return false;
    ty = t / f.tiles_x; tx = t - ty * f.tiles_x;
    return true;
}

struct DevPaths {
    F4* ray_o;
    F4* ray_d;
    F4* thr;
// ... 110 lines not shown
```

### royaltracer-dx_amd/csrc/rtx_scene_cache.cpp

```cpp
#include <algorithm>
#include <cstdio>
#include <cstring>
#include <new>
#include <stdexcept>
#include <thread>
#include <fcntl.h>
#include <sys/mman.h>
#include <sys/stat.h>
#include <unistd.h>
#include "rtx_scene_host.hpp"

namespace rtx {
namespace {

constexpr char kMagic[8] = {'R', 'T', 'X', 'S', 'C', 'N', '0', '1'};
constexpr uint32_t kVersion = 3;
struct Header { char magic[8]; uint32_t version, endian; uint32_t layout[8]; uint64_t payload, checksum, nsections; };
struct SecHead { uint32_t tag, elem; uint64_t count; };
static_assert(sizeof(Header) == 72 && sizeof(SecHead) == 16, "cache header layout");
constexpr size_t kHeaderBytes = 80;

void fill_layout(uint32_t l[8]) {
    l[0] = sizeof(Node8GPU); l[1] = sizeof(TriGPU); l[2] = sizeof(TriShade); l[3] = sizeof(MatGPU);
    l[4] = sizeof(InstGPU); l[5] = sizeof(LightGPU); l[6] = sizeof(SmallRecPair); l[7] = sizeof(InstHost);
}

constexpr size_t kChunk = 4u << 20;
inline uint64_t mix(uint64_t h, uint64_t w) { h = (h ^ w) * 0x9E3779B97F4A7C15ull; return h ^ (h >> 29); }
uint64_t hash_chunk(const uint8_t* p, size_t n) {
    uint64_t h[4] = {0x243F6A8885A308D3ull, 0x13198A2E03707344ull, 0xA4093822299F31D0ull, 0x082EFA98EC4E6C89ull};
    size_t i = 0;
    for (; i + 32 <= n; i += 32) { uint64_t w[4]; memcpy(w, p + i, 32); for (int k = 0; k < 4; k++) h[k] = mix(h[k], w[k]); }
    uint64_t tail[4] = {0, 0, 0, 0};
    memcpy(tail, p + i, n - i);
    for (int k = 0; k < 4; k++) h[k] = mix(h[k], tail[k]);
    return mix(mix(mix(mix(n, h[0]), h[1]), h[2]), h[3]);
}
unsigned pool_size() { unsigned n = std::thread::hardware_concurrency(); return n ? std::min(n, 16u) : 4u; }
uint64_t hash_payload(const uint8_t* p, size_t n) {
    const size_t nchunks = (n + kChunk - 1) / kChunk;
    std::vector<uint64_t> part(nchunks);
    const unsigned T = (unsigned)std::min<size_t>(pool_size(), std::max<size_t>(nchunks, 1));
    std::vector<std::thread> th;
    for (unsigned t = 0; t < T; t++)
        th.emplace_back([&, t] { for (size_t c = t; c < nchunks; c += T) part[c] = hash_chunk(p + c * kChunk, std::min(kChunk, n - c * kChunk)); });
    for (auto& x : th) x.join();
    uint64_t h = 0x452821E638D01377ull ^ n;
    for (uint64_t v : part) h = mix(h, v);
    return h;
}
void parallel_copy(void* dst, const void* src, size_t n) {
    if (!n) return;
    if (n < (8u << 20)) { memcpy(dst, src, n); return; }
    const unsigned T = pool_size();
    const size_t per = ((n / T) + 4095) & ~(size_t)4095;
    std::vector<std::thread> th;
    for (unsigned t = 0; t < T; t++) {
        const size_t off = (size_t)t * per;
        if (off >= n) break;
        th.emplace_back([=] { memcpy((uint8_t*)dst + off, (const uint8_t*)src + off, std::min(per, n - off)); });
    }
    for (auto& x : th) x.join();
}

struct Writer {
    std::vector<uint8_t> buf; uint64_t nsec = 0;
    void raw(uint32_t tag, uint32_t elem, uint64_t count, const void* data) {
        SecHead s{tag, elem, count};
        const size_t at = buf.size(), bytes = (size_t)elem * count, padded = (bytes + 15) & ~(size_t)15;
        buf.resize(at + sizeof(s) + padded, 0);
        memcpy(&buf[at], &s, sizeof(s));
        if (bytes) memcpy(&buf[at + sizeof(s)], data, bytes);
        nsec++;
    }
    template <class T> void vec(uint32_t tag, const std::vector<T>& v) { raw(tag, (uint32_t)sizeof(T), v.size(), v.data()); }
};
struct Scalars { uint32_t stack8, small_nrec, small_nocc, max_depth, nmesh, has_cam, pad1, pad2; float bvh_pad, small_cm, small_delta, small_hull_margin, total_weight, f0, f1, f2;
                 float cam[12]; };

struct Reader {
    const uint8_t* p; size_t n, at = 0; std::string* err;
    bool head(uint32_t tag, uint32_t elem, SecHead& s) {
        if (at + sizeof(SecHead) > n) { *err = "scene cache: truncated section table"; return false; }
        memcpy(&s, p + at, sizeof(s)); at += sizeof(s);
        const size_t bytes = (size_t)s.elem * s.count, padded = (bytes + 15) & ~(size_t)15;
        if (s.tag != tag || s.elem != elem || s.count > n || at + padded > n) { *err = "scene cache: unexpected section (tag " + std::to_string(s.tag) + ")"; return false; }
        return true;
    }
    template <class T> bool vec(uint32_t tag, std::vector<T>& v) {
        SecHead s; if (!head(tag, (uint32_t)sizeof(T), s)) return false;
        v.resize(s.count);
        parallel_copy(v.data(), p + at, sizeof(T) * s.count);
        at += (sizeof(T) * s.count + 15) & ~(size_t)15;
        return true;
    }
};

enum : uint32_t { T_SCAL = 1, T_MATS128, T_MATIDS, T_INSTH, T_MESHV, T_MESHI, T_MESHB, T_BMATS, T_NODES8, T_SLOTS8, T_TRIS8, T_LEVELS, T_SMALLR, T_SMALLT, T_SMALLP,
                T_SHADE, T_BINST, T_LIGHTS, T_LIGHTS80, T_AUXREC, T_AUXTXT };

}

bool save_scene_cache(const SceneHost& H, const BuiltScene& B, const char* path, std::string& err, const float* cam12, const CacheAux* aux) {
    if (!path || !*path) { err = "scene cache: empty path"; return false; }
    if (H.topo_dirty || H.mats_dirty || B.tris8.size() < B.shade.size() || B.tris8.size() != B.tri_slots8.size() || (!B.tris8.empty() && B.nodes8.empty())) { err = "scene cache: scene not built"; return false; }
    Writer w;
    Scalars sc{}; sc.stack8 = B.stack8; sc.small_nrec = B.small_nrec; sc.small_nocc = B.small_nocc; sc.max_depth = B.max_depth; sc.nmesh = (uint32_t)H.meshes.size();
    sc.bvh_pad = B.bvh_pad; sc.small_cm = B.small_cm; sc.small_delta = B.small_delta; sc.small_hull_margin = B.small_hull_margin; sc.total_weight = B.total_weight;
    if (cam12) { sc.has_cam = 1; memcpy(sc.cam, cam12, sizeof(sc.cam)); }
    w.raw(T_SCAL, sizeof(Scalars), 1, &sc);
    w.vec(T_MATS128, H.mats128); w.vec(T_MATIDS, H.matids); w.vec(T_INSTH, H.insts);
    for (const MeshHost& m : H.meshes) { w.vec(T_MESHV, m.verts); w.vec(T_MESHI, m.idx); w.raw(T_MESHB, 4, 1, &m.matid_base); }
    w.vec(T_BMATS, B.mats); w.vec(T_NODES8, B.nodes8); w.vec(T_SLOTS8, B.tri_slots8); w.vec(T_TRIS8, B.tris8); w.vec(T_LEVELS, B.level_start8);
    w.vec(T_SMALLR, B.small_recs); w.vec(T_SMALLT, B.small_tris); w.vec(T_SMALLP, B.small_poly);
    w.vec(T_SHADE, B.shade); w.vec(T_BINST, B.insts); w.vec(T_LIGHTS, B.lights); w.vec(T_LIGHTS80, B.lights80);
    const CacheAux none;
    const CacheAux& ax = aux ? *aux : none;
    w.raw(T_AUXREC, ax.rec_bytes ? ax.rec_bytes : 1u, ax.rec_bytes ? ax.records.size() / ax.rec_bytes : 0u, ax.records.data()); w.vec(T_AUXTXT, ax.text);
    Header h{}; memcpy(h.magic, kMagic, 8); h.version = kVersion; h.endian = 0x01020304u; fill_layout(h.layout);
    h.payload = w.buf.size(); h.checksum = hash_payload(w.buf.data(), w.buf.size()); h.nsections = w.nsec;
    uint8_t hb[kHeaderBytes] = {0}; memcpy(hb, &h, sizeof(h));
    const std::string tmp = std::string(path) + ".tmp";
    FILE* f = fopen(tmp.c_str(), "wb");
    if (!f) { err = "scene cache: cannot create " + tmp; return false; }
    const bool ok = fwrite(hb, 1, kHeaderBytes, f) == kHeaderBytes && fwrite(w.buf.data(), 1, w.buf.size(), f) == w.buf.size();
    if (fclose(f) != 0 || !ok) { remove(tmp.c_str()); err = "scene cache: write failed"; return false; }
    if (rename(tmp.c_str(), path) != 0) { remove(tmp.c_str()); err = "scene cache: cannot move into place"; return false; }
    return true;
}

static bool load_scene_cache_impl(const char* path, SceneHost& H, BuiltScene& B, std::string& err, float* cam12, CacheAux* aux) {
    const int fd = path ? open(path, O_RDONLY) : -1;
    if (fd < 0) { err = std::string("scene cache: cannot open ") + (path ? path : "(null)"); return false; }
    struct stat st;
    if (fstat(fd, &st) != 0 || (size_t)st.st_size < kHeaderBytes) { close(fd); err = "scene cache: file too short"; return false; }
    const size_t total = (size_t)st.st_size;
    void* map = mmap(nullptr, total, PROT_READ, MAP_PRIVATE, fd, 0);
    close(fd);
    if (map == MAP_FAILED) { err = "scene cache: mmap failed"; return false; }
    struct Unmap { void* p; size_t n; ~Unmap() { munmap(p, n); } } guard{map, total};
    const uint8_t* base = (const uint8_t*)map;
    Header h; memcpy(&h, base, sizeof(h));
    uint32_t lay[8]; fill_layout(lay);
    if (memcmp(h.magic, kMagic, 8) != 0) { err = "scene cache: not a scene cache file"; return false; }
    if (h.version != kVersion) { err = "scene cache: version " + std::to_string(h.version) + ", this library reads version " + std::to_string(kVersion); return false; }
    if (h.endian != 0x01020304u || memcmp(h.layout, lay, sizeof(lay)) != 0) { err = "scene cache: written with another record layout"; return false; }
    if (h.payload != total - kHeaderBytes) { err = "scene cache: length does not match the header"; return false; }
    if (hash_payload(base + kHeaderBytes, h.payload) != h.checksum) { err = "scene cache: checksum mismatch (corrupt file)"; return false; }
    SceneHost Hn; BuiltScene Bn;
    Reader r{base + kHeaderBytes, (size_t)h.payload, 0, &err};
    SecHead s; Scalars sc;
    if (!r.head(T_SCAL, sizeof(Scalars), s) || s.count != 1) { if (err.empty()) err = "scene cache: bad scalar block"; return false; }
    memcpy(&sc, r.p + r.at, sizeof(sc)); r.at += sizeof(sc);
    if (!r.vec(T_MATS128, Hn.mats128) || !r.vec(T_MATIDS, Hn.matids) || !r.vec(T_INSTH, Hn.insts)) return false;
    if ((uint64_t)sc.nmesh * (3 * sizeof(SecHead) + 16) > h.payload - r.at || (uint64_t)sc.nmesh * 3 > h.nsections) { err = "scene cache: mesh count does not fit the file"; return false; }
    Hn.meshes.resize(sc.nmesh);
    for (MeshHost& m : Hn.meshes) {
        if (!r.vec(T_MESHV, m.verts) || !r.vec(T_MESHI, m.idx)) return false;
        if (!r.head(T_MESHB, 4, s) || s.count != 1) return false;
        memcpy(&m.matid_base, r.p + r.at, 4); r.at += 16;
    }
    if (!r.vec(T_BMATS, Bn.mats) || !r.vec(T_NODES8, Bn.nodes8) || !r.vec(T_SLOTS8, Bn.tri_slots8) || !r.vec(T_TRIS8, Bn.tris8) || !r.vec(T_LEVELS, Bn.level_start8) ||
        !r.vec(T_SMALLR, Bn.small_recs) || !r.vec(T_SMALLT, Bn.small_tris) || !r.vec(T_SMALLP, Bn.small_poly) || !r.vec(T_SHADE, Bn.shade) || !r.vec(T_BINST, Bn.insts) ||
        !r.vec(T_LIGHTS, Bn.lights) || !r.vec(T_LIGHTS80, Bn.lights80)) return false;
    CacheAux ax;
    {
        if (r.at + sizeof(SecHead) > r.n) { err = "scene cache: truncated section table"; return false; }
        SecHead a; memcpy(&a, r.p + r.at, sizeof(a));
        if (a.tag != T_AUXREC || !a.elem || a.elem > 4096u || !r.head(T_AUXREC, a.elem, a)) { if (err.empty()) err = "scene cache: bad auxiliary section"; return false; }
        ax.rec_bytes = a.elem; ax.records.assign(r.p + r.at, r.p + r.at + (size_t)a.elem * a.count);
        r.at += ((size_t)a.elem * a.count + 15) & ~(size_t)15;
        if (!r.vec(T_AUXTXT, ax.text)) return false;
    }
    if (r.at != h.payload) { err = "scene cache: trailing bytes"; return false; }
    const size_t nt = Bn.shade.size(), nmat = Hn.mats128.size() / 32;
    const size_t nrec_pad = ((size_t)sc.small_nrec + 1) & ~(size_t)1;
    const size_t nrefs = Bn.tris8.size();
    bool ok = nrefs >= nt && Bn.tri_slots8.size() == nrefs && Bn.mats.size() == nmat && Bn.insts.size() == Hn.insts.size() && Bn.lights80.size() == Bn.lights.size() * 20 &&
              Hn.mats128.size() % 32 == 0 && (Bn.nodes8.empty() || Bn.level_start8.size() >= 2) && sc.small_nocc <= sc.small_nrec && sc.small_nrec <= kSmallSceneMaxTris &&
              Bn.small_recs.size() * 2 >= nrec_pad && (sc.small_nrec == 0 || (Bn.small_tris.size() >= nrec_pad * 2 && Bn.small_poly.size() >= nrec_pad * 4)) &&
              nrefs < (1u << 31);
    for (uint32_t id : Hn.matids) ok = ok && id < nmat;
    for (const MeshHost& m : Hn.meshes) {
        ok = ok && m.verts.size() % 7 == 0 && m.idx.size() % 3 == 0 && (size_t)m.matid_base + m.idx.size() <= Hn.matids.size();
        const size_t nv = m.verts.size() / 7;
        for (size_t i = 0; ok && i < m.idx.size(); i++) ok = m.idx[i] < nv;
    }
    size_t tri_at = 0;
    for (const InstHost& in : Hn.insts) {
        ok = ok && in.mesh < Hn.meshes.size() && in.tri_base == tri_at;
        if (ok) tri_at += Hn.meshes[in.mesh].idx.size() / 3;
    }
    ok = ok && tri_at == nt;
    for (size_t i = 0; ok && i < nt; i++) ok = Bn.shade[i].inst < Bn.insts.size();
    for (size_t i = 0; ok && i < nrefs; i++) ok = f2u(Bn.tris8[i].v0.w) < nt && Bn.tri_slots8[i] < nrefs;
    for (size_t i = 0; ok && i < Bn.small_tris.size(); i++) { const uint32_t g = f2u(Bn.small_tris[i].v0.w); ok = g < nt || g == kMissPrim; }
    for (size_t i = 0; ok && i < Bn.lights.size(); i++) ok = f2u(Bn.lights80[i * 20 + 7]) < Bn.insts.size();
    for (size_t i = 0; ok && i < Bn.nodes8.size(); i++) {
        const Node8GPU& N = Bn.nodes8[i];
        const uint32_t ninternal = (uint32_t)__builtin_popcount(N.e_imask >> 24);
        uint32_t ntri = 0; for (int sl = 0; sl < 8; sl++) ntri += (uint32_t)__builtin_popcount((N.trivalid >> (4 * sl)) & 0xfu);
        ok = (ninternal == 0 || ((size_t)N.child_base + ninternal <= Bn.nodes8.size() && N.child_base > i)) && (size_t)N.tri_base + ntri <= nrefs;
    }
    if (!ok) { err = "scene cache: inconsistent contents"; return false; }
    {
        const size_t nn = Bn.nodes8.size();
        std::vector<uint32_t> need(nn, 0), level(nn, 0);
        for (size_t i = nn; i-- > 0;) {
            const uint32_t nint = (uint32_t)__builtin_popcount(Bn.nodes8[i].e_imask >> 24);
            uint32_t deep = 0;
            for (uint32_t k = 0; k < nint; k++) deep = std::max(deep, need[(size_t)Bn.nodes8[i].child_base + k]);
            need[i] = (nint > 1 ? 1u : 0u) + deep;
        }
        const uint32_t stack8 = nn ? need[0] : 0u;
        std::vector<uint32_t> levels;
        for (size_t i = 0; i < nn; i++) {
            const uint32_t nint = (uint32_t)__builtin_popcount(Bn.nodes8[i].e_imask >> 24);
            for (uint32_t k = 0; k < nint; k++) level[(size_t)Bn.nodes8[i].child_base + k] = level[i] + 1;
        }
        for (size_t i = 0; i < nn; i++) {
            if (i && level[i] < level[i - 1]) { err = "scene cache: nodes are not in breadth-first order"; return false; }
            if (i == 0 || level[i] != level[i - 1]) levels.push_back((uint32_t)i);
        }
        if (nn) levels.push_back((uint32_t)nn);
        if (stack8 != sc.stack8 || (nn && levels != Bn.level_start8)) { err = "scene cache: stack depth / level table do not match the nodes"; return false; }
    }
    Bn.stack8 = sc.stack8; Bn.small_nrec = sc.small_nrec; Bn.small_nocc = sc.small_nocc; Bn.max_depth = sc.max_depth; Bn.bvh_pad = sc.bvh_pad;
    Bn.small_cm = sc.small_cm; Bn.small_delta = sc.small_delta; Bn.small_hull_margin = sc.small_hull_margin; Bn.total_weight = sc.total_weight; Bn.refit_count = 0;
    Bn.any_order = probe_anyhit_order(Bn);
    Hn.topo_dirty = false; Hn.mats_dirty = false;
    if (cam12) { if (!sc.has_cam) { err = "scene cache: the file holds no camera (written by rtx_save_scene_cache, not rtxh_scene_save)"; return false; } memcpy(cam12, sc.cam, sizeof(sc.cam)); }
    H = std::move(Hn); B = std::move(Bn);
    if (aux) *aux = std::move(ax);
    return true;
}

bool load_scene_cache(const char* path, SceneHost& H, BuiltScene& B, std::string& err, float* cam12, CacheAux* aux) {
    try { return load_scene_cache_impl(path, H, B, err, cam12, aux); }
    catch (const std::bad_alloc&) { err = "scene cache: out of memory while reading"; }
    catch (const std::exception& e) { err = std::string("scene cache: ") + e.what(); }
    return false;
}

}
```

### royaltracer-dx_amd/csrc/rtx_scene_host.cpp

```cpp
#include "rtx_scene_host.hpp"
#include "rtx_normalmap_host.hpp"
#include <algorithm>
#include <cmath>
#include <cstring>
#include <system_error>
#include <thread>

namespace rtx {

float half_round(float x) {
    uint32_t u = f2u(x), sign = u & 0x80000000u, a = u & 0x7FFFFFFFu;
    if (a >= 0x7F800000u) return x;
    if (a >= 0x477FF000u) return u2f(sign | 0x7F800000u);
    if (a < 0x33000001u) return u2f(sign);
    if (a < 0x38800000u) {
        float r = nearbyintf(u2f(a) * 16777216.0f);
        return u2f(sign | f2u(r * (1.0f / 16777216.0f)));
    }
    uint32_t rem = a & 0x1FFFu, base = a & ~0x1FFFu;
    if (rem > 0x1000u || (rem == 0x1000u && (base & 0x2000u))) base += 0x2000u;
    return u2f(sign | base);
}

void mat4_inverse(const float* mf, float* out) {
// ... 266 lines not shown
    }
}

bool SceneHost::refresh_transforms(BuiltScene& B) {
    if (topo_dirty || B.insts.size() != insts.size()) { err = "refresh_transforms: topology changed"; return false; }
    const bool mats_changed = mats_dirty;
    if (mats_dirty) build_materials(B);
    B.inst_moved.assign(insts.size(), 0u);
    B.inst_hidden.resize(insts.size(), 0u);
    bool emitter_flipped = false;
    for (size_t ii = 0; ii < insts.size(); ii++) {
        const InstHost& in = insts[ii];
        const bool flipped = (B.inst_hidden[ii] != 0u) != is_hidden(ii);
        B.inst_moved[ii] = (memcmp(B.insts[ii].o2w, in.o2w, 64) != 0 || mesh_is_dirty(in.mesh) || flipped) ? 1u : 0u;
        if (flipped && !emitter_flipped && instance_emits(ii)) emitter_flipped = true;
        copy_instance(B.insts[ii], in);
    }
    commit_visibility(B);
    if (mats_changed || dirty_mesh_emits() || emitter_flipped) build_lights(B); else refresh_lights(B);
    B.refit_count++;
    return true;
}

void SceneHost::build_materials(BuiltScene& B) {
    const uint32_t nmat = (uint32_t)(mats128.size() / 32);
    B.mats.resize(nmat);
    for (uint32_t i = 0; i < nmat; i++) {
        const float* m = &mats128[(size_t)i * 32];
        MatGPU& g = B.mats[i];
        for (int k = 0; k < 3; k++) { g.Kd[k] = half_round(m[k]); g.Ks[k] = half_round(m[4 + k]); g.Ke[k] = half_round(m[8 + k]); }
        g.Pr = half_round(m[12]); g.Pm = half_round(m[13]);
        g.KeFull[0] = m[8]; g.KeFull[1] = m[9]; g.KeFull[2] = m[10]; g.KeFullLen = length(mk3(m[8], m[9], m[10]));
        g.Ke_len = length(mk3(g.Ke[0], g.Ke[1], g.Ke[2]));
        for (int k = 0; k < 3; k++) g.KdPi[k] = g.Kd[k] / kPI;
        g.pad = 0.0f;
        g.alpha = half_round(m[3]); g.Ni = m[7]; g.pad1 = g.pad2 = 0.0f;
        memcpy(g.LUT, m + 16, 64);
    }
    mats_dirty = false;
}

static uint32_t number_triangle_ranges(SceneHost& H, BuiltScene& B) {
    uint32_t nt = 0;
    for (auto& in : H.insts) { in.tri_base = nt; nt += (uint32_t)(H.meshes[in.mesh].idx.size() / 3); }
    B.insts.resize(H.insts.size());
    for (size_t ii = 0; ii < H.insts.size(); ii++) copy_instance(B.insts[ii], H.insts[ii]);
    H.commit_visibility(B);
    return nt;
}

static void forget_tree(BuiltScene& B, uint32_t nt) {
    B.shade.clear(); B.shade.shrink_to_fit(); B.objtris.clear(); B.objtris.shrink_to_fit();
    B.bvh_pad = 2e-6f; B.nodes.clear(); B.nodes8.clear(); B.tri_slots8.clear(); B.tris8.clear(); B.tris.clear(); B.leaf_order.clear(); B.level_start8.clear();
    B.small_recs.clear(); B.small_tris.clear(); B.small_poly.clear(); B.small_nrec = 0; B.small_nocc = 0; B.built_tris = nt; B.refit_count = 0; B.any_order = 0;
}

bool SceneHost::prepare_device_build(BuiltScene& B) {
    BuildStopwatch sw("[build] ", 28);
    build_materials(B);
    const uint32_t nt = number_triangle_ranges(*this, B);
    sw.lap("materials + instances");
    build_lights(B);
    sw.lap("lights");
    forget_tree(B, nt);
    topo_dirty = false;
    return true;
}

void SceneHost::fill_objtris(BuiltScene& B) const {
    size_t nt = 0; for (const InstHost& in : insts) nt += meshes[in.mesh].idx.size() / 3;
    B.objtris.resize(nt * 3);
    for (const InstHost& in : insts) {
        const MeshHost& m = meshes[in.mesh];
        for (uint32_t t = 0; t < m.idx.size() / 3; t++) put_objtri(m, t, &B.objtris[((size_t)in.tri_base + t) * 3]);
    }
}

static void flatten_range(const SceneHost& H, size_t ii, uint32_t t_lo, uint32_t t_hi, BuiltScene& B, std::vector<float>& wtri, float& scale) {
    const InstHost& in = H.insts[ii]; const MeshHost& m = H.meshes[in.mesh];
    for (uint32_t t = t_lo; t < t_hi; t++) {
        uint32_t g = in.tri_base + t;
        uint32_t i0 = m.idx[t * 3], i1 = m.idx[t * 3 + 1], i2 = m.idx[t * 3 + 2];
        const uint32_t vi[3] = {i0, i1, i2};
        put_objtri(m, t, &B.objtris[(size_t)g * 3]);
        for (int k = 0; k < 3; k++) {
            f3 w = xform_point(in.o2w, vpos(m, vi[k]));
            wtri[(size_t)g * 9 + k * 3] = w.x; wtri[(size_t)g * 9 + k * 3 + 1] = w.y; wtri[(size_t)g * 9 + k * 3 + 2] = w.z;
            scale = std::max(scale, std::max(fabsf(w.x), std::max(fabsf(w.y), fabsf(w.z))));
        }
        TriShade& s = B.shade[g];
        uint32_t mi = m.matid_base + 3 * t;
        s.mat = mi < H.matids.size() ? H.matids[mi] : kMissMat;
        s.inst = (uint32_t)ii;
        f3 p0 = vpos(m, i0);
        f3 cr = cross(vpos(m, i1) - p0, vpos(m, i2) - p0);
        s.area = fabsf(length(cr) * 0.5f);
        f3 flat = normalize(cr);
        s.flat[0] = flat.x; s.flat[1] = flat.y; s.flat[2] = flat.z;
        float* dst[3] = {s.n0, s.n1, s.n2};
        for (int k = 0; k < 3; k++) {
            f3 nk = vnrm(m, vi[k]);
            f3 use = (nk.x != 0.0f && nk.y != 0.0f && nk.z != 0.0f) ? nk : flat;
            dst[k][0] = use.x; dst[k][1] = use.y; dst[k][2] = use.z;
        }
        s.guard_tau = 0.0f;
    }
}

static float flatten_instances(const SceneHost& H, uint32_t nt, BuiltScene& B, std::vector<float>& wtri) {
    wtri.resize((size_t)nt * 9);
    B.shade.resize(nt);
    B.objtris.resize((size_t)nt * 3);
    float scale = 1.0f;
    for (size_t ii = 0; ii < H.insts.size(); ii++) {
        const uint32_t ntm = (uint32_t)(H.meshes[H.insts[ii].mesh].idx.size() / 3);
        const unsigned hwc = std::thread::hardware_concurrency();
        const uint32_t nth = ntm >= 65536u ? std::min<uint32_t>(16u, std::max(1u, hwc ? hwc : 4u)) : 1u;
        std::vector<float> tscale(nth, 1.0f);
        if (nth <= 1) flatten_range(H, ii, 0, ntm, B, wtri, tscale[0]);
        else {
            std::vector<std::thread> pool;
            for (uint32_t k = 0; k < nth; k++) {
                const uint32_t lo_t = (uint32_t)((uint64_t)ntm * k / nth), hi_t = (uint32_t)((uint64_t)ntm * (k + 1) / nth);
                try { pool.emplace_back([&, lo_t, hi_t, k] { flatten_range(H, ii, lo_t, hi_t, B, wtri, tscale[k]); }); } catch (const std::system_error&) { flatten_range(H, ii, lo_t, hi_t, B, wtri, tscale[k]); }
            }
            for (std::thread& th : pool) th.join();
        }
        for (float v : tscale) scale = std::max(scale, v);
    }
    return scale;
}

static void build_or_refit_bvh(SceneHost& H, BuiltScene& B, const std::vector<float>& wtri, uint32_t nt) {
    const bool refit = !H.topo_dirty && B.built_tris == nt && !B.leaf_order.empty() && !B.nodes.empty();
    if (refit) refit_bvh(wtri, B.bvh_pad, B.nodes, B.leaf_order);
    else { build_bvh(wtri, B.bvh_pad, B.nodes, B.leaf_order, B.max_depth, H.bvh); B.built_tris = nt; }
    B.refit_count = refit ? B.refit_count + 1 : 0;
    H.topo_dirty = false;
}

bool SceneHost::build(BuiltScene& B) {
    BuildStopwatch sw("[build] ", 28);
    build_materials(B);
    const uint32_t nt = number_triangle_ranges(*this, B);
    std::vector<float> wtri;
    const float scale = flatten_instances(*this, nt, B, wtri);
    sw.lap("flatten + shade records");
    build_lights(B);
    sw.lap("lights");
    B.bvh_pad = 2e-6f * scale;
    build_or_refit_bvh(*this, B, wtri, nt);
    sw.lap("build_bvh");
    leaf_triangles(wtri, B.leaf_order, B.tris);
    if (!wide_from_binary(B, bvh)) { err = "build: BVH collapse failed"; return false; }
    sw.lap("collapse_bvh8");
    B.maps_active = maps_active(); B.cutouts_active = cutouts_active(); B.normals_active = normals_active(); B.env_active = env.n != 0;
    if (B.any_hidden || B.maps_active || B.cutouts_active || B.normals_active || B.env_active) { B.small_recs.clear(); B.small_tris.clear(); B.small_poly.clear(); B.small_nrec = 0; B.small_nocc = 0; }
    else build_small_scene(B, wtri, scale);
    sw.lap("tris8 / small scene");
    B.any_order = probe_anyhit_order(B);
    sw.lap("probe");
    return true;
}

}
```

### royaltracer-dx_amd/csrc/rtx_scene_host.hpp

```cpp
#pragma once
#include <vector>
#include <string>
#include <stdint.h>
#include "rtx_types.hpp"
#include "rtx_bvh_host.hpp"
#include "rtx_env_host.hpp"

namespace rtx {

float half_round(float x);
void  mat4_inverse(const float* m16, float* out16);
void  normal_matrix(const float* o2w16, float* out16);

struct MeshHost { std::vector<float> verts; std::vector<uint32_t> idx; uint32_t matid_base = 0; std::vector<float> uvs; };
struct TexHost { uint32_t width = 0, height = 0, flags = 0; std::vector<uint32_t> rgba; };
struct InstHost { uint32_t mesh; float o2w[16]; float nrm[16]; float o2w_inv[16]; float prev_o2w[16]; uint32_t tri_base; };

struct BuiltScene {
    std::vector<MatGPU>   mats;
    std::vector<NodeGPU>  nodes;
    std::vector<Node8GPU> nodes8;
    std::vector<uint32_t> tri_slots8;
    std::vector<TriGPU>   tris8;
    uint32_t stack8 = 0;
    std::vector<uint32_t> level_start8;
    std::vector<F4>       objtris;
    float bvh_pad = 0.0f;
    std::vector<TriGPU>   tris;
    std::vector<SmallRecPair> small_recs; std::vector<TriGPU> small_tris; uint32_t small_nrec = 0;
    std::vector<F4> small_poly;
    uint32_t small_nocc = 0;
    float small_cm = 0.0f, small_delta = 0.0f;
    float small_hull_margin = 0.0f;
    std::vector<TriShade> shade;
    std::vector<InstGPU>  insts;
    std::vector<LightGPU> lights;
    std::vector<float>    lights80;
    std::vector<uint32_t> leaf_order;
    uint32_t any_order = 0;
    uint32_t built_tris = 0;
    float total_weight = 0.0f;
    uint32_t max_depth = 0;
    uint32_t refit_count = 0;
    std::vector<uint32_t> inst_hidden;
    bool any_hidden = false;
    bool maps_active = false;
    bool cutouts_active = false;
    bool normals_active = false;
    bool env_active = false;
    std::vector<uint32_t> inst_moved;
};

struct SceneHost {
    std::vector<float> mats128;
    std::vector<MeshHost> meshes;
    std::vector<uint32_t> matids;
    std::vector<InstHost> insts;
    std::string err;
    bool topo_dirty = true;
    bool mats_dirty = true;
    std::vector<uint32_t> dirty_meshes;
    std::vector<uint8_t> inst_hidden;
    std::vector<TexHost> textures;
    std::vector<int32_t> map_kd;
    std::vector<int32_t> map_opacity;
    std::vector<int32_t> map_normal;
    bool tex_dirty = false;
    EnvHost env;
    bool env_dirty = false;
    BvhBuildOptions bvh = bvh_build_options();

    bool set_materials(const void* mats, uint32_t count);
    bool add_mesh(const void* verts28, uint32_t nverts, const uint32_t* idx, uint32_t nidx, const uint32_t* matids, uint32_t* out);
    bool add_instance(uint32_t mesh, const float* o2w, uint32_t* out);
    bool set_instance_transform(uint32_t inst, const float* o2w);
    bool set_instance_visible(uint32_t inst, bool visible, bool* changed);
    bool is_hidden(size_t inst) const { return inst < inst_hidden.size() && inst_hidden[inst] != 0; }
    bool any_hidden() const { for (uint8_t h : inst_hidden) if (h) return true; return false; }
    void commit_visibility(BuiltScene& out) const;
    bool instance_emits(size_t inst) const;
    bool update_mesh_vertices(uint32_t mesh, const void* verts28, uint32_t nverts);
    bool mesh_is_dirty(uint32_t mesh) const { for (uint32_t m : dirty_meshes) if (m == mesh) return true; return false; }
    bool dirty_mesh_emits() const;
// ... 32 lines not shown
```

### royaltracer-dx_amd/csrc/rtx_small_scene.cpp

```cpp
#include "rtx_scene_host.hpp"
#include <algorithm>
#include <array>
#include <cmath>

namespace rtx {

namespace {
struct D3 { double x, y, z; };
inline D3 sub(D3 a, D3 b) { return D3{a.x - b.x, a.y - b.y, a.z - b.z}; }
inline D3 crs(D3 a, D3 b) { return D3{a.y * b.z - a.z * b.y, a.z * b.x - a.x * b.z, a.x * b.y - a.y * b.x}; }
inline double dt(D3 a, D3 b) { return a.x * b.x + a.y * b.y + a.z * b.z; }
inline D3 nrm(D3 a) { double l = sqrt(dt(a, a)); return l > 0 ? D3{a.x / l, a.y / l, a.z / l} : D3{0, 0, 0}; }
inline bool same(D3 a, D3 b) { return a.x == b.x && a.y == b.y && a.z == b.z; }
using TriVerts = std::vector<std::array<D3, 3>>;
struct Rec { double pl[4]; double e[4][4]; int s0, s1; double pv[4][3]; };

Rec make_rec(const std::vector<D3>& poly, D3 nu, int s0, int s1) {
    Rec R; R.s0 = s0; R.s1 = s1;
    for (int k = 0; k < 4; k++) { const D3& q = poly[std::min<size_t>((size_t)k, poly.size() - 1)]; R.pv[k][0] = q.x; R.pv[k][1] = q.y; R.pv[k][2] = q.z; }
    R.pl[0] = nu.x; R.pl[1] = nu.y; R.pl[2] = nu.z; R.pl[3] = dt(nu, poly[0]);
    for (int k = 0; k < 4; k++) { R.e[k][0] = R.e[k][1] = R.e[k][2] = 0.0; R.e[k][3] = 1e30; }
    for (size_t k = 0; k < poly.size(); k++) {
        D3 A = poly[k], Bv = poly[(k + 1) % poly.size()];
        D3 m = nrm(crs(nu, sub(Bv, A)));
// ... 49 lines not shown
        if (g >= B.shade.size()) continue;
        const TriShade& ts = B.shade[g];
        const f3 nw = normalize(xform_dir(B.insts[ts.inst].nrm, mk3(ts.flat[0], ts.flat[1], ts.flat[2])));
        double tau = 0.0;
        for (const Rec& Hf : hull) {
            double dmax = 0.0, side = 0.0;
            for (size_t s2 = 0; s2 < n; s2++) for (int k = 0; k < 3; k++) {
                const double dd = Hf.pl[0] * V[s2][k].x + Hf.pl[1] * V[s2][k].y + Hf.pl[2] * V[s2][k].z - Hf.pl[3];
                if (fabs(dd) > fabs(side)) side = dd;
            }
            const double sgn = side >= 0.0 ? 1.0 : -1.0;
            for (int k = 0; k < 3; k++) dmax = std::max(dmax, fabs(Hf.pl[0] * V[si][k].x + Hf.pl[1] * V[si][k].y + Hf.pl[2] * V[si][k].z - Hf.pl[3]));
            const double ndot = sgn * (Hf.pl[0] * (double)nw.x + Hf.pl[1] * (double)nw.y + Hf.pl[2] * (double)nw.z);
            const double need = safety - (double)kSBias * ndot + 1e-7 * (double)kSBias;
            if (!(need > 0.0)) continue;
            tau = dmax > 0.0 ? std::max(tau, need / dmax) : 2.0;
        }
        B.shade[g].guard_tau = (float)std::min(2.0, tau * 1.000001);
    }
}

void hull_faces_last(BuiltScene& B, const TriVerts& V, double tol, float scale, std::vector<Rec>& recs) {
    const size_t n = V.size();
    auto emissive = [&](int slot) {
        if (slot < 0) return false;
        const uint32_t g = f2u(B.tris[(size_t)slot].v0.w);
        const uint32_t m = g < B.shade.size() ? B.shade[g].mat : 0xFFFFFFFFu;
        return m < B.mats.size() && B.mats[m].Ke_len > 0.0f;
    };
    std::vector<D3> light_verts;
    for (size_t s = 0; s < n; s++) if (emissive((int)s)) for (int k = 0; k < 3; k++) light_verts.push_back(V[s][k]);
    const double near_plane = 5.0 * (double)kSBias + 2e-4 * (double)scale;
    bool all_flat = B.small_hull_margin < 0.9f * kSBias;
    for (const TriShade& ts : B.shade) for (int k = 0; k < 3; k++)
        if (ts.n0[k] != ts.flat[k] || ts.n1[k] != ts.flat[k] || ts.n2[k] != ts.flat[k]) all_flat = false;
    std::vector<Rec> occ, hull;
    for (const Rec& R : recs) {
        if (!all_flat) { occ.push_back(R); continue; }
        bool pos = false, neg = false;
        const bool degenerate = R.pl[0] == 0.0 && R.pl[1] == 0.0 && R.pl[2] == 0.0;
        bool light = emissive(R.s0) || emissive(R.s1);
        for (const D3& q : light_verts) if (fabs(R.pl[0] * q.x + R.pl[1] * q.y + R.pl[2] * q.z - R.pl[3]) <= near_plane) light = true;
        for (size_t s = 0; s < n && !degenerate; s++) for (int k = 0; k < 3; k++) {
            const double dd = R.pl[0] * V[s][k].x + R.pl[1] * V[s][k].y + R.pl[2] * V[s][k].z - R.pl[3];
            if (dd > tol) pos = true; else if (dd < -tol) neg = true;
        }
        (((pos && neg) || light) ? occ : hull).push_back(R);
    }
    B.small_nocc = (uint32_t)occ.size();
    set_guard_tau(B, V, hull);
    recs = occ; recs.insert(recs.end(), hull.begin(), hull.end());
}

void pack_records(BuiltScene& B, const std::vector<Rec>& recs, double delta) {
    B.small_nrec = (uint32_t)recs.size();
    B.small_tris.assign(((recs.size() + 1) & ~(size_t)1) * 2, TriGPU{{0, 0, 0, u2f(kMissPrim)}, {0, 0, 0, 0}, {0, 0, 0, 0}});
    const TriGPU none{{0, 0, 0, u2f(kMissPrim)}, {0, 0, 0, 0}, {0, 0, 0, 0}};
    for (size_t r = 0; r < recs.size(); r++) { B.small_tris[2 * r] = B.tris[recs[r].s0]; B.small_tris[2 * r + 1] = recs[r].s1 >= 0 ? B.tris[recs[r].s1] : none; }
    B.small_poly.assign(((recs.size() + 1) & ~(size_t)1) * 4, F4{0.0f, 0.0f, 0.0f, 0.0f});
    for (size_t r = 0; r < recs.size(); r++) for (int k = 0; k < 4; k++) B.small_poly[r * 4 + k] = {(float)recs[r].pv[k][0], (float)recs[r].pv[k][1], (float)recs[r].pv[k][2], 0.0f};
    for (size_t r = 0; r < recs.size(); r += 2) {
        SmallRecPair P;
        for (int e = 0; e < 2; e++) {
            const bool have = r + e < recs.size();
            for (int row = 0; row < 20; row++) {
                double v;
                if (!have) v = (row == 7 || row == 11 || row == 15 || row == 19) ? -1e30 : 0.0;
                else v = row < 4 ? recs[r + e].pl[row] : recs[r + e].e[(row - 4) / 4][(row - 4) % 4] + ((row - 4) % 4 == 3 ? delta : 0.0);
                P.r[row][e] = (float)v;
            }
        }
        B.small_recs.push_back(P);
    }
}
}

void build_small_scene(BuiltScene& B, const std::vector<float>& wtri, float scale) {
    const std::vector<uint32_t>& leaf_order = B.leaf_order;
    B.small_recs.clear(); B.small_tris.clear(); B.small_poly.clear(); B.small_nrec = 0; B.small_nocc = 0;
    if (leaf_order.empty() || leaf_order.size() > kSmallSceneMaxTris) return;
    const double delta = 2e-5 * (double)scale, tol = 1e-6 * (double)scale;
    B.small_delta = (float)delta; B.small_cm = 4e-6f * scale; B.small_hull_margin = 2e-6f * scale;
    const size_t n = leaf_order.size();
    TriVerts V(n);
    for (size_t s = 0; s < n; s++) { const float* t = &wtri[(size_t)leaf_order[s] * 9]; for (int k = 0; k < 3; k++) V[s][k] = D3{t[k * 3], t[k * 3 + 1], t[k * 3 + 2]}; }
    std::vector<Rec> recs = merge_quads(V, tol, scale);
    hull_faces_last(B, V, tol, scale, recs);
    pack_records(B, recs, delta);
}

}
```

### royaltracer-dx_amd/csrc/rtx_traverse.hpp

```cpp
#pragma once
#include <type_traits>
#include "rtx_dev_common.hpp"
#include "rtx_cutout.hpp"

namespace rtx {

#ifdef RTX_PROFILE_SECTIONS
struct Prof {
    unsigned long long t, acc[12], lanes[12], calls[12];
    __device__ __forceinline__ void begin() { t = __builtin_readcyclecounter(); for (int i = 0; i < 12; i++) { acc[i] = 0; lanes[i] = 0; calls[i] = 0; } }
    __device__ __forceinline__ void mark(int i) { const unsigned long long n = __builtin_readcyclecounter(); acc[i] += n - t; t = n; }
    __device__ __forceinline__ void count(int i) { lanes[i] += (unsigned long long)__builtin_popcountll(__builtin_amdgcn_read_exec()); calls[i] += 1; }
};
#define RTX_PROF_MARK(pf, i) do { if (pf) (pf)->mark(i); } while (0)
#define RTX_PROF_COUNT(pf, i) do { if (pf) (pf)->count(i); } while (0)
#else
struct Prof {};
#define RTX_PROF_MARK(pf, i) do { } while (0)
#define RTX_PROF_COUNT(pf, i) do { } while (0)
#endif

typedef float v4f __attribute__((ext_vector_type(4)));
typedef __attribute__((address_space(3))) v4f lds_v4f;
typedef __attribute__((address_space(3))) uint32_t lds_u32;
typedef float f2v __attribute__((ext_vector_type(2)));
__device__ __forceinline__ f2v fma2(f2v a, f2v b, f2v c) { return __builtin_elementwise_fma(a, b, c); }
__device__ __forceinline__ f2v splat2(float x) { f2v r = {x, x}; return r; }
__device__ __forceinline__ uint32_t shift_in(uint32_t acc, unsigned long long m) {
    uint32_t r;
    asm("v_addc_co_u32_e64 %0, vcc, %1, %1, %2" : "=v"(r) : "v"(acc), "s"(m) : "vcc");
    return r;
}
__device__ __forceinline__ float margin_t(float cm, float ind, float t) {
    float a, r;
    asm("v_mul_f32_e64 %0, |%1|, %2" : "=v"(a) : "v"(t), "v"(1e-5f));
    asm("v_fma_f32 %0, |%1|, %2, %3" : "=v"(r) : "v"(ind), "s"(cm), "v"(a));
    return r;
}
typedef uint32_t v2u __attribute__((ext_vector_type(2)));
typedef uint32_t v4u __attribute__((ext_vector_type(4)));
typedef __attribute__((address_space(3))) v2u lds_u2;
typedef __attribute__((address_space(3))) uint16_t lds_u16;
struct TraceLds {
    const lds_v4f* nodes;
    const lds_v4f* tris;
    const lds_v4f* planes;
    lds_u32* stack;
    lds_u16* stack_bits;
    unsigned long long* ovf; uint32_t cap, ovf_stride;
};
__host__ __device__ inline uint32_t small_planes_count(uint32_t nsmall) { return (nsmall + 1u) & ~1u; }

__device__ __forceinline__ TraceLds stage_lds(const DevScene& sc, F4* lds_generic) {
    TraceLds L;
    lds_v4f* ln = (lds_v4f*)lds_generic; lds_v4f* lt = ln + (size_t)sc.lds_nodes * 5;
    const v4f* gn = (const v4f*)sc.nodes; const v4f* gt = (const v4f*)(sc.nsmall ? sc.small_tris : sc.tris);
    for (uint32_t i = threadIdx.x; i < sc.lds_nodes * 5u; i += kBlock) ln[i] = gn[i];
    for (uint32_t i = threadIdx.x; i < sc.lds_tris * 3u; i += kBlock) lt[i] = gt[i];
    lds_v4f* lp = lt + (size_t)sc.lds_tris * 3;
    const uint32_t npl = sc.nsmall ? small_planes_count(sc.nsmall) : 0u;
    for (uint32_t i = threadIdx.x; i < npl; i += kBlock) {
        const float* r = &sc.small[i >> 1].r[0][i & 1u];
        const v4f pl = {r[0], r[2], r[4], r[6]};
        lp[i] = pl;
    }
    L.nodes = ln; L.tris = lt; L.planes = lp;
    L.stack = (lds_u32*)(lp + npl);
    L.stack_bits = (lds_u16*)(L.stack + (size_t)sc.stack_depth * kBlock);
    L.cap = sc.stack_depth; L.ovf_stride = sc.stack_ovf_stride;
    L.ovf = sc.stack_ovf ? sc.stack_ovf + ((blockIdx.x * kBlock + threadIdx.x) & (sc.stack_ovf_stride - 1u)) : nullptr;
    return L;
}

__device__ __forceinline__ bool tri_test(f3 o, f3 d, v4f v0w, v4f e1w, v4f e2w, float tmin, float tmax, float& t, float& u, float& v) {
    const f3 v0 = mk3(v0w.x, v0w.y, v0w.z), e1 = mk3(e1w.x, e1w.y, e1w.z), e2 = mk3(e2w.x, e2w.y, e2w.z);
    const f3 p = cross(d, e2);
    const float det = dot(e1, p);
    if (!(fabsf(det) > e1w.w)) return false;
    const float inv = 1.0f / det;
    const f3 s = o - v0;
    u = dot(s, p) * inv;
    if (!(u >= 0.0f && u <= 1.0f)) return false;
    const f3 q = cross(s, e1);
    v = dot(d, q) * inv;
    if (!(v >= 0.0f && u + v <= 1.0f)) return false;
    t = dot(e2, q) * inv;
    return t > tmin && t < tmax;
}

__device__ __forceinline__ bool tri_test_flat(f3 o, f3 d, v4f v0w, v4f e1w, v4f e2w, float tmin, float tmax, float& t, float& u, float& v) {
    const f3 v0 = mk3(v0w.x, v0w.y, v0w.z), e1 = mk3(e1w.x, e1w.y, e1w.z), e2 = mk3(e2w.x, e2w.y, e2w.z);
// ... 107 lines not shown
}
__device__ __forceinline__ uint32_t tri_slot8(const TriGrp& T, uint32_t bit) { return T.base + (uint32_t)__builtin_popcount(T.valid & ((1u << bit) - 1u)); }

__device__ __forceinline__ f3 safe_idir(f3 d) {
    const float dxs = fabsf(d.x) < 1e-30f ? copysignf(1e-30f, d.x) : d.x;
    const float dys = fabsf(d.y) < 1e-30f ? copysignf(1e-30f, d.y) : d.y;
    const float dzs = fabsf(d.z) < 1e-30f ? copysignf(1e-30f, d.z) : d.z;
    return mk3(__builtin_amdgcn_rcpf(dxs), __builtin_amdgcn_rcpf(dys), __builtin_amdgcn_rcpf(dzs));
}
__device__ __forceinline__ Grp root_group(uint32_t oct, bool ordered, uint32_t aord) {
    return Grp{0u, (ordered ? (1u << oct) : (aord ? 1u << (oct ^ (aord == 2u ? 7u : 0u)) : 1u)) | (1u << 8)};
}
__device__ __forceinline__ void load_tri(const DevScene& sc, const TraceLds& L, uint32_t slot, v4f& v0, v4f& e1, v4f& e2) {
    if (slot < sc.lds_tris) { const lds_v4f* t = L.tris + slot * 3u; v0 = t[0]; e1 = t[1]; e2 = t[2]; }
    else { const v4f* t = (const v4f*)(sc.tris + slot); v0 = t[0]; e1 = t[1]; e2 = t[2]; }
}
__device__ __forceinline__ bool closer(float t, uint32_t gid, const float& bt, const uint32_t& bprim) { return t < bt || (t == bt && gid < bprim); }

template <bool ANY, bool COUNT = false, bool CUT = false>
__device__ __forceinline__ void traverse(const DevScene& sc, const TraceLds& L, f3 o, f3 d, float tmin, float tmax,
                                         float& bt, float& bu, float& bv, uint32_t& bprim) {
    uint32_t nsteps = 0, ntris = 0;
    const f3 idir = safe_idir(d);
    const uint32_t oct = ray_octant(idir);
    bt = tmax; bu = 0.0f; bv = 0.0f; bprim = kMissPrim;
    StackLds stk; stk.init(L);
    int sp = 0;
    Grp G = root_group(oct, !ANY, sc.any_order);
    TriGrp T{0u, 0u, 0u};
    while (true) {
        if (G.bits & 0xffu) { descend8<!ANY>(sc, L, o, idir, oct, tmin, bt, G, T, stk, sp); if (COUNT) nsteps++; }
        while (T.bits) {
            const uint32_t bit = (uint32_t)__builtin_ctz(T.bits);
            T.bits &= T.bits - 1u; if (COUNT) ntris++;
            v4f v0, e1, e2;
            load_tri(sc, L, tri_slot8(T, bit), v0, e1, e2);
            float t, u, w;
            if (tri_test(o, d, v0, e1, e2, tmin, tmax, t, u, w)) {
                if (CUT && !cut_accept(sc, f2u(v0.w), u, w)) continue;
                if (ANY) { bprim = 0u; if (COUNT) { bu = (float)nsteps; bv = (float)ntris; } return; }
                const uint32_t gid = f2u(v0.w);
                if (closer(t, gid, bt, bprim)) { bt = t; bu = u; bv = w; bprim = gid; }
            }
        }
        if (!(G.bits & 0xffu)) {
            if (sp == 0) break;
            sp--; G = stk.get(sp);
        }
    }
    if (COUNT) { bu = (float)nsteps; bv = (float)ntris; }
}


template <bool ANY>
__device__ __forceinline__ void traverse_small(const DevScene& sc, const SmallRecPair* __restrict__ sp, const TraceLds& L, f3 o, f3 d, float tmin, float tmax,
                                               float& bt, float& bu, float& bv, uint32_t& bprim, uint32_t nrec, unsigned long long keep = ~0ull, Prof* pf = nullptr, int pf_sec = 0) {
    bt = tmax; bu = 0.0f; bv = 0.0f; bprim = kMissPrim;
    uint32_t cand_lo = 0u, cand_hi = 0u;
    const uint32_t npairs = (nrec + 1u) >> 1;
    const f2v dx = splat2(d.x), dy = splat2(d.y), dz = splat2(d.z), ox = splat2(o.x), oy = splat2(o.y), oz = splat2(o.z);
    const f2v vtmin = splat2(tmin), vtmax = splat2(tmax);
    const float cm = sc.small_cm;
    uint32_t near = ~0u;
    auto pair = [&](uint32_t kp, uint32_t& acc) {
        const f2v* __restrict__ R = (const f2v*)sp[kp].r;
        const f2v nd = fma2(R[2], dz, fma2(R[1], dy, R[0] * dx));
        const f2v no = R[3] - fma2(R[2], oz, fma2(R[1], oy, R[0] * ox));
        f2v ind; ind.x = __builtin_amdgcn_rcpf(nd.x); ind.y = __builtin_amdgcn_rcpf(nd.y);
        const f2v t = no * ind;
        const f2v px = fma2(t, dx, ox), py = fma2(t, dy, oy), pz = fma2(t, dz, oz);
        const f2v e0 = fma2(R[6], pz, fma2(R[5], py, R[4] * px)) + R[7];
        const f2v e1 = fma2(R[10], pz, fma2(R[9], py, R[8] * px)) + R[11];
        const f2v e2 = fma2(R[14], pz, fma2(R[13], py, R[12] * px)) + R[15];
        const f2v e3 = fma2(R[18], pz, fma2(R[17], py, R[16] * px)) + R[19];
        f2v mt; mt.x = margin_t(cm, ind.x, t.x); mt.y = margin_t(cm, ind.y, t.y);
        const f2v a0 = (t + mt) - vtmin, a1 = (vtmax + mt) - t;
        const float ma0 = fminf(a0.x, a1.x), ma1 = fminf(a0.y, a1.y);
        const float me0 = fminf(e0.x, fminf(fminf(e1.x, e2.x), e3.x)), me1 = fminf(e0.y, fminf(fminf(e1.y, e2.y), e3.y));
        const unsigned long long c0 = (__builtin_amdgcn_ballot_w64(ma0 >= 0.0f) & __builtin_amdgcn_ballot_w64(me0 >= -mt.x)) | __builtin_amdgcn_ballot_w64(fabsf(nd.x) < 1e-3f);
        const unsigned long long c1 = (__builtin_amdgcn_ballot_w64(ma1 >= 0.0f) & __builtin_amdgcn_ballot_w64(me1 >= -mt.y)) | __builtin_amdgcn_ballot_w64(fabsf(nd.y) < 1e-3f);
        acc = shift_in(shift_in(acc, c1), c0);
        if (!ANY) {
            const uint32_t k0 = (f2u(t.x) & ~63u) | (2u * kp), k1 = (f2u(t.y) & ~63u) | (2u * kp + 1u);
            const bool in0 = (ma0 >= 0.0f && me0 >= -mt.x) || (fabsf(nd.x) < 1e-3f), in1 = (ma1 >= 0.0f && me1 >= -mt.y) || (fabsf(nd.y) < 1e-3f);
            near = min(near, min(in0 ? k0 : ~0u, in1 ? k1 : ~0u));
        }
    };
#pragma unroll 1
    for (uint32_t kp = npairs; kp > 16u; kp--) {
        if (!((keep >> (2u * (kp - 1u))) & 3ull)) { cand_hi <<= 2; continue; }
        pair(kp - 1u, cand_hi);
    }
#pragma unroll 1
    for (uint32_t kp = npairs < 16u ? npairs : 16u; kp > 0u; kp--) {
        if (!((keep >> (2u * (kp - 1u))) & 3ull)) { cand_lo <<= 2; continue; }
        pair(kp - 1u, cand_lo);
    }
    RTX_PROF_MARK(pf, pf_sec);
    unsigned long long cand = ((unsigned long long)cand_hi << 32) | cand_lo;
    cand &= nrec >= 64u ? ~0ull : ((1ull << nrec) - 1ull);
    auto exact = [&](uint32_t k) -> bool {
        RTX_PROF_COUNT(pf, pf_sec + 1);
#pragma unroll
        for (uint32_t h = 0; h < 2u; h++) {
            const lds_v4f* tp = L.tris + (2u * k + h) * 3u;
            const v4f v0 = tp[0], e1 = tp[1], e2 = tp[2];
            float t, u, w;
            if (tri_test(o, d, v0, e1, e2, tmin, tmax, t, u, w)) {
                if (ANY) { bprim = 0u; return true; }
                const uint32_t gid = f2u(v0.w);
                if (closer(t, gid, bt, bprim)) { bt = t; bu = u; bv = w; bprim = gid; }
            }
        }
        return false;
    };
    if (ANY) {
        while (cand) {
            const uint32_t k = (uint32_t)__builtin_ctzll(cand);
            cand &= cand - 1ull;
            if (exact(k)) return;
        }
        return;
    }
    if (!cand) return;
    uint32_t k = near & 63u;
    if (!((cand >> k) & 1ull)) k = (uint32_t)__builtin_ctzll(cand);
    cand &= ~(1ull << k);
    bool go = true;
    while (go) {
        exact(k);
        go = false;
        while (cand) {
            k = (uint32_t)__builtin_ctzll(cand);
            cand &= cand - 1ull;
            const v4f pl = L.planes[k];
            const float nd = __builtin_fmaf(pl.z, d.z, __builtin_fmaf(pl.y, d.y, pl.x * d.x));
            const float no = pl.w - __builtin_fmaf(pl.z, o.z, __builtin_fmaf(pl.y, o.y, pl.x * o.x));
            const float ind = __builtin_amdgcn_rcpf(nd);
            const float t = no * ind;
            const float mt = margin_t(cm, ind, t);
            if ((fabsf(nd) < 1e-3f) || !((t - mt) > bt)) { go = true; break; }
        }
    }
}

template <bool ANY, bool CUT = false>
__device__ __forceinline__ void trace_ray(const DevScene& sc, const SmallRecPair* __restrict__ small, const TraceLds& L, f3 o, f3 d, float tmin, float tmax,
                                          float& bt, float& bu, float& bv, uint32_t& bprim) {
    if (!CUT && sc.nsmall) traverse_small<ANY>(sc, small, L, o, d, tmin, tmax, bt, bu, bv, bprim, sc.nsmall);
    else traverse<ANY, false, CUT>(sc, L, o, d, tmin, tmax, bt, bu, bv, bprim);
}

// ... 315 lines not shown
```

### royaltracer-dx_amd/csrc/rtx_types.hpp

```cpp
#pragma once
#include <stdint.h>
#include "rtx_bsdf.hpp"

namespace rtx {

struct alignas(16) F4 { float x, y, z, w; };

struct alignas(16) NodeGPU { F4 a, b, c, d; };
constexpr int32_t kEmptyChild = 0x7FFFFFFF;

constexpr uint32_t kStackEntryBytes = 6;
struct alignas(16) Node8GPU { float px, py, pz; uint32_t e_imask; uint32_t child_base, tri_base, trivalid, pad; uint32_t q[12]; };
static_assert(sizeof(Node8GPU) == 80, "Node8GPU must be 80 bytes");

struct alignas(16) TriGPU { F4 v0, e1, e2; };

struct alignas(16) SmallRecPair { float r[20][2]; };
static_assert(sizeof(SmallRecPair) == 160, "SmallRecPair must be 160 bytes");
constexpr uint32_t kSmallSceneMaxTris = 64;

struct alignas(16) TriShade {
    uint32_t mat, inst;
    float flat[3];
    float n0[3], n1[3], n2[3];
    float area;
    float guard_tau;
};
static_assert(sizeof(TriShade) == 64, "TriShade must be 64 bytes");

struct alignas(16) InstGPU { float o2w[16]; float nrm[16]; float o2w_inv[16]; float prev_o2w[16]; };

struct alignas(16) LightGPU {
    float xv[3]; float cdf;
    float yv[3]; float pdf_l;
    float zv[3]; float pad0;
    float em[3]; float pad1;
    float nl[3]; float pad2;
};
static_assert(sizeof(LightGPU) == 80, "LightGPU must be 80 bytes");

struct alignas(16) TexDesc { uint32_t offset, width, height, flags; };
static_assert(sizeof(TexDesc) == 16, "TexDesc must be 16 bytes");

struct CameraGPU { float viewI[16]; float projI[16]; float prev_view[16]; float prev_proj[16]; };

}
```

### royaltracer-dx_amd/host/rtx_host_c.cpp

```cpp
#include "../../include/rtx_host.h"
#include <cstring>
#include <type_traits>
#include <exception>
#include <stdexcept>
#include <algorithm>
#include <cmath>
#include <string>
#include "../csrc/rtx_scene_host.hpp"
#include "ObjLoader.h"
#include "Renderer.h"
#include "ImageIO.h"
#include "Scenes.h"
#include "manipulator.h"

struct rtxh_scene { Scene s; std::string cache_path; };
struct rtxh_renderer { Renderer* r; };
static thread_local std::string g_err;

template <class F> static rtxh_scene* guarded(F&& f) {
    try { rtxh_scene* h = new rtxh_scene(); h->s = f(); return h; }
    catch (const std::exception& e) { g_err = e.what(); return nullptr; }
}
template <class F> static int guarded_rc(F&& f) {
    try { f(); return RTX_OK; } catch (const std::exception& e) { g_err = e.what(); return RTX_ERR_INVALID; }
// ... 280 lines not shown
        for (int sl = 0; sl < 8; sl++) {
            if ((imask >> sl) & 1u) { hist[5]++; continue; }
            hist[__builtin_popcount((N.trivalid >> (4 * sl)) & 0xfu)]++;
        }
    }
    if (nodes8_out) *nodes8_out = (uint32_t)B.nodes8.size();
    return 0;
}

int rtxh_bvh_check(const float* wt, uint32_t ntris, uint32_t* nodes_out, uint32_t* depth_out, uint32_t* max_leaf_out) {
    std::vector<float> w(wt, wt + (size_t)ntris * 9);
    std::vector<rtx::NodeGPU> nodes; std::vector<uint32_t> order; uint32_t depth = 0;
    rtx::build_bvh(w, 0.0f, nodes, order, depth);
    if (nodes_out) *nodes_out = (uint32_t)nodes.size();
    if (depth_out) *depth_out = depth;
    return bvh_validate(w, nodes, order, max_leaf_out);
}

int rtxh_bvh_refit_check(const float* before, const float* after, uint32_t ntris) {
    std::vector<float> a(before, before + (size_t)ntris * 9), b(after, after + (size_t)ntris * 9);
    rtx::BuiltScene B;
    rtx::build_bvh(a, 0.0f, B.nodes, B.leaf_order, B.max_depth);
    rtx::refit_bvh(b, 0.0f, B.nodes, B.leaf_order);
    if (int r = bvh_validate(b, B.nodes, B.leaf_order, nullptr)) return r;
    rtx::leaf_triangles(b, B.leaf_order, B.tris);
    if (!rtx::wide_from_binary(B)) return 30;
    return rtx::validate_bvh8(b, B.nodes8, B.leaf_order, B.tri_slots8, nullptr);
}

int rtxh_scene_small_occluders(const rtxh_scene* sc, uint32_t* nocc_out) {
    rtx::BuiltScene B;
    if (!sc || !nocc_out || !build_for_inspection(sc, B)) return RTX_ERR_INVALID;
    *nocc_out = B.small_nocc;
    return RTX_OK;
}
int rtxh_scene_anyhit_order(const rtxh_scene* sc, uint32_t* order_out) {
    rtx::BuiltScene B;
    if (!sc || !order_out || !build_for_inspection(sc, B)) return RTX_ERR_INVALID;
    *order_out = B.any_order;
    return RTX_OK;
}
int rtxh_scene_small_records(const rtxh_scene* sc, float* recs20, int32_t* tri_ids2, uint32_t max_recs, uint32_t* nrec_out, float* delta_out, float* cm_out) {
    rtx::BuiltScene B;
    if (!build_for_inspection(sc, B)) return RTX_ERR_INVALID;
    if (nrec_out) *nrec_out = B.small_nrec;
    if (delta_out) *delta_out = 0.0f;
    if (cm_out) *cm_out = B.small_cm;
    for (uint32_t r = 0; r < B.small_nrec && r < max_recs; r++) {
        for (int row = 0; row < 20; row++) recs20[(size_t)r * 20 + row] = B.small_recs[r / 2].r[row][r & 1];
        for (int h = 0; h < 2; h++) { uint32_t g = rtx::f2u(B.small_tris[2 * r + h].v0.w); tri_ids2[2 * r + h] = g == rtx::kMissPrim ? -1 : (int32_t)g; }
    }
    return RTX_OK;
}

rtxh_renderer* rtxh_renderer_create(uint32_t w, uint32_t h, const char* name, int device) {
    rtxh_renderer* r = new rtxh_renderer(); r->r = new Renderer(w, h, name ? name : "rtx"); r->r->SetDevice(device); return r;
}
int rtxh_renderer_set_scene(rtxh_renderer* r, const rtxh_scene* s) { r->r->SetScene(s->s); return RTX_OK; }
rtx_params* rtxh_renderer_params(rtxh_renderer* r) { return &r->r->Params(); }
int rtxh_renderer_set_mode(rtxh_renderer* r, int mode) {
    if (mode != 0 && mode != 1) { g_err = "renderer mode must be 0 (path tracer) or 1 (ReSTIR frame)"; return RTX_ERR_INVALID; }
    r->r->SetMode(mode ? Renderer::Mode::ReSTIR : Renderer::Mode::PathTracer); return RTX_OK;
}
rtx_params* rtxh_renderer_restir_params(rtxh_renderer* r) { return &r->r->RestirParams(); }
rtx_ctx* rtxh_renderer_context(rtxh_renderer* r) { return r->r->Context(); }
int rtxh_renderer_on_init(rtxh_renderer* r) { return guarded_rc([&] { r->r->OnInit(); }); }
int rtxh_renderer_on_update(rtxh_renderer* r) { return guarded_rc([&] { r->r->OnUpdate(); }); }
int rtxh_renderer_set_instance_visible(rtxh_renderer* r, uint32_t instance, int visible) { return guarded_rc([&] { r->r->SetInstanceVisible(instance, visible != 0); }); }
int rtxh_renderer_set_instance_transform(rtxh_renderer* r, uint32_t instance, const float o2w[16]) { return guarded_rc([&] { XMMATRIX m; memcpy(m.data(), o2w, 64); r->r->SetInstanceTransform(instance, m); }); }
int rtxh_renderer_set_mesh_vertices(rtxh_renderer* r, uint32_t mesh, const void* verts28, uint32_t nverts) {
    return guarded_rc([&] { if (!verts28) throw std::invalid_argument("set_mesh_vertices: null array"); const Vertex* v = (const Vertex*)verts28; r->r->SetMeshVertices(mesh, std::vector<Vertex>(v, v + nverts)); });
}
int rtxh_renderer_on_render(rtxh_renderer* r) { return guarded_rc([&] { r->r->OnRender(); }); }
int rtxh_renderer_read_accum(rtxh_renderer* r, float* out, size_t bytes) {
    return guarded_rc([&] { auto v = r->r->ReadAccumulation(); if (bytes < v.size() * 4) throw std::runtime_error("buffer too small"); memcpy(out, v.data(), v.size() * 4); });
}
int rtxh_renderer_read_output(rtxh_renderer* r, uint8_t* out, size_t bytes) {
    return guarded_rc([&] { auto v = r->r->ReadOutput(); if (bytes < v.size()) throw std::runtime_error("buffer too small"); memcpy(out, v.data(), v.size()); });
}
int rtxh_renderer_on_key_up(rtxh_renderer* h, uint8_t key) { return guarded_rc([&] { h->r->OnKeyUp(key); }); }
uint32_t rtxh_renderer_display_layer(const rtxh_renderer* h) { return h->r->CurrentDisplayLayer(); }
void rtxh_renderer_destroy(rtxh_renderer* r) { if (r) { delete r->r; delete r; } }

int rtxh_write_png(const char* path, const uint8_t* rgba8, uint32_t width, uint32_t height) { return path && WritePNG(path, rgba8, width, height) ? RTX_OK : RTX_ERR_INVALID; }
int rtxh_write_ppm(const char* path, const uint8_t* rgba8, uint32_t width, uint32_t height) { return path && WritePPM(path, rgba8, width, height) ? RTX_OK : RTX_ERR_INVALID; }
int rtxh_write_exr(const char* path, const float* rgba32f, uint32_t width, uint32_t height) { return path && WriteEXR(path, rgba32f, width, height) ? RTX_OK : RTX_ERR_INVALID; }

}
```

Measured before the change: 40680 Mrays/s.

## Cull small-scene quad records with two-slab tests and skip far-plane check

For small scenes, each record pair that is a near-rectangular quad gets a precomputed two-slab bound (two plane normals, center and half-width). The wave-wide candidate filter then evaluates two slab distances instead of four edge functions, which cuts ALU and record bytes read per pair. A new OPEN template variant drops the tmax side of the candidate test for closest-hit traversal and instead clears all candidates when tmax is not positive. The cost is extra candidates passed to exact intersection, both from the slab's looser bound on non-rectangular quads and from the missing far-plane test.

```diff
diff --git a/include/rtx.h b/include/rtx.h
--- a/include/rtx.h
+++ b/include/rtx.h
@@ -93,6 +93,7 @@
        RTX_OPT_STACK_CAP = 39,
        RTX_OPT_SHARED_PRIMARY = 41,
        RTX_OPT_DENOISE_LDS_STEP = 42,
+       RTX_OPT_SMALL_SLABS = 43,
        RTX_OPT_BLOCKS_PER_CU = 12     };
 
 int  rtx_create(int device_ordinal, rtx_ctx** out);
diff --git a/include/rtx_host.h b/include/rtx_host.h
--- a/include/rtx_host.h
+++ b/include/rtx_host.h
@@ -67,6 +67,7 @@
 
 int  rtxh_scene_small_records(const rtxh_scene*, float* recs20, int32_t* tri_ids2, uint32_t max_recs, uint32_t* nrec_out, float* delta_out, float* cm_out);
 int  rtxh_scene_small_occluders(const rtxh_scene*, uint32_t* nocc_out);
+int  rtxh_scene_small_slabs(const rtxh_scene*, float* slabs10, float* excess, uint32_t max_recs, uint32_t* nrec_out, uint32_t* pair_mask_out);
 int  rtxh_scene_anyhit_order(const rtxh_scene*, uint32_t* order_out);
 
 typedef struct rtxh_renderer rtxh_renderer;
diff --git a/royaltracer-dx_amd/__init__.py b/royaltracer-dx_amd/__init__.py
--- a/royaltracer-dx_amd/__init__.py
+++ b/royaltracer-dx_amd/__init__.py
@@ -34,6 +34,7 @@
 OPT_DEFORM_REBUILD = 40
 OPT_SHARED_PRIMARY = 41
 OPT_DENOISE_LDS_STEP = 42
+OPT_SMALL_SLABS = 43
 TEX_SRGB = 1
 MAP_KD = 0
 MAP_OPACITY = 2
@@ -238,6 +239,7 @@
 _sig("rtxh_write_ppm", C.c_int, C.c_char_p, _vp, _u32, _u32)
 _sig("rtxh_write_exr", C.c_int, C.c_char_p, _vp, _u32, _u32)
 _sig("rtxh_scene_small_records", C.c_int, _vp, _vp, _vp, _u32, _u32p, _fp, _fp)
+_sig("rtxh_scene_small_slabs", C.c_int, _vp, _vp, _vp, _u32, _u32p, _u32p)
 _sig("rtxh_scene_set_camera", C.c_int, _vp, _fp, _fp, _fp)
 _sig("rtxh_scene_set_mesh_vertices", C.c_int, _vp, _u32, _vp, _u32)
 _sig("rtxh_renderer_set_mesh_vertices", C.c_int, _vp, _u32, _vp, _u32)
@@ -394,6 +396,13 @@
             return None
         return recs[:n.value], ids[:n.value], d.value, cm.value
 
+    def small_slabs(self):
+        slabs, ex = np.zeros((64, 10), np.float32), np.zeros(64, np.float32)
+        n, m = _u32(), _u32()
+        if lib.rtxh_scene_small_slabs(self._h, _ptr(slabs), _ptr(ex), 64, C.byref(n), C.byref(m)) != RTX_OK or n.value == 0:
+            return None
+        return slabs[:n.value], ex[:n.value], m.value
+
     def small_occluders(self):
         n = _u32()
         if lib.rtxh_scene_small_occluders(self._h, C.byref(n)) != RTX_OK:
diff --git a/royaltracer-dx_amd/csrc/rtx_api.hip b/royaltracer-dx_amd/csrc/rtx_api.hip
--- a/royaltracer-dx_amd/csrc/rtx_api.hip
+++ b/royaltracer-dx_amd/csrc/rtx_api.hip
@@ -10,6 +10,7 @@
     if (committed) {
         s.any_order = o.any_order_opt < 0 ? c->scene.built.any_order : (uint32_t)o.any_order_opt;
         s.any_order_occ = o.any_order_opt < 0 ? 0u : (uint32_t)o.any_order_opt;
+        s.small_slab_mask = o.small_slabs ? c->scene.built.small_slab_mask : 0u;
     }
 }
 
@@ -159,6 +160,7 @@
     case RTX_OPT_PARTIAL_REFIT: c->opt.partial_refit = value != 0; return RTX_OK;
     case RTX_OPT_LDS_NODES_CLOSEST: c->opt.lds_closest_opt = (int)value; if (c->committed) pick_lds_closest(c); return RTX_OK;
     case RTX_OPT_SMALL_SCENE: c->opt.small_scene = value != 0; c->committed = false; return RTX_OK;
+    case RTX_OPT_SMALL_SLABS: c->opt.small_slabs = value != 0; options_to_scene(c, c->committed); return RTX_OK;
     case RTX_OPT_FUSED_BOUNCE: c->opt.fused = value != 0; return RTX_OK;
     case RTX_OPT_BOUNCE_VARIANT: c->opt.bounce_variant = value == 2 ? 2 : (value != 0 ? 1 : 0); return RTX_OK;
     case RTX_OPT_SHARED_PRIMARY: c->opt.shared_primary = value != 0; return RTX_OK;
diff --git a/royaltracer-dx_amd/csrc/rtx_commit.hip b/royaltracer-dx_amd/csrc/rtx_commit.hip
--- a/royaltracer-dx_amd/csrc/rtx_commit.hip
+++ b/royaltracer-dx_amd/csrc/rtx_commit.hip
@@ -35,6 +35,7 @@
     if ((r = upload(c, c->scene.d_small, B.small_recs))) return r;
     if ((r = upload(c, c->scene.d_small_tris, B.small_tris))) return r;
     if ((r = upload(c, c->scene.d_small_poly, B.small_poly))) return r;
+    if ((r = upload(c, c->scene.d_small_slabs, B.small_slabs))) return r;
     if ((r = upload(c, c->scene.d_mats, B.mats))) return r;
     if ((r = upload(c, c->scene.d_insts, B.insts))) return r;
     return upload_lights(c);
@@ -336,7 +337,7 @@
     if ((r = upload(c, c->scene.d_insts, B.insts))) return r;
     if ((r = upload_lights(c))) return r;
     if ((r = flatten_on_device(c, nt))) return r; c->scene.objtris_uploaded = true;
-    for (DevBuf* b : {&c->scene.d_small, &c->scene.d_small_tris, &c->scene.d_small_poly}) HIPCHK(c, b->ensure(16));
+    for (DevBuf* b : {&c->scene.d_small, &c->scene.d_small_tris, &c->scene.d_small_poly, &c->scene.d_small_slabs}) HIPCHK(c, b->ensure(16));
     HIPCHK(c, c->scene.d_tris.ensure((size_t)nt * sizeof(TriGPU)));
     if (!c->scene.builder) c->scene.builder.reset(new GpuBvhBuilder());
     BvhBuildOptions bo = c->host.bvh; if (bo.ploc_radius <= 0) bo.ploc_radius = 16;
@@ -448,7 +449,7 @@
     if (c->scene.wide_nodes && c->opt.node_stride == 128) { s.nodes_f = (const F4*)c->scene.d_nodes_wide.p; s.node_v4 = 8u; }
     s.tris = (const TriGPU*)c->scene.d_tris.p; s.ntris = c->scene.n_tris8;
     s.shade = (const TriShade*)c->scene.d_shade.p;
-    s.small = (const SmallRecPair*)c->scene.d_small.p; s.small_tris = (const TriGPU*)c->scene.d_small_tris.p; s.small_poly = (const F4*)c->scene.d_small_poly.p; s.small_cm = B.small_cm; s.small_delta = B.small_delta;
+    s.small = (const SmallRecPair*)c->scene.d_small.p; s.small_tris = (const TriGPU*)c->scene.d_small_tris.p; s.small_poly = (const F4*)c->scene.d_small_poly.p; s.small_slabs = (const SmallSlabPair*)c->scene.d_small_slabs.p; s.small_cm = B.small_cm; s.small_delta = B.small_delta;
     s.mats = (const MatGPU*)c->scene.d_mats.p; s.nmat = (uint32_t)B.mats.size();
     s.insts = (const InstGPU*)c->scene.d_insts.p; s.ninst = (uint32_t)B.insts.size();
     s.lights = (const LightGPU*)c->scene.d_lights.p; s.nlights = (uint32_t)B.lights.size(); s.cdf = (const float*)c->scene.d_cdf.p;
diff --git a/royaltracer-dx_amd/csrc/rtx_ctx.hpp b/royaltracer-dx_amd/csrc/rtx_ctx.hpp
--- a/royaltracer-dx_amd/csrc/rtx_ctx.hpp
+++ b/royaltracer-dx_amd/csrc/rtx_ctx.hpp
@@ -46,6 +46,7 @@
         int partial_refit = 1;
         int lds_closest_opt = -1;
         bool small_scene = true;
+        bool small_slabs = true;
         bool fused = true;
         int bounce_variant = 2;
         bool shared_primary = true;
@@ -85,7 +86,7 @@
     struct Scene {
         BuiltScene built;
         bool committed_once = false;
-        DevBuf d_nodes, d_tris, d_small, d_small_tris, d_small_poly, d_shade, d_mats, d_insts, d_lights, d_cdf;
+        DevBuf d_nodes, d_tris, d_small, d_small_tris, d_small_poly, d_small_slabs, d_shade, d_mats, d_insts, d_lights, d_cdf;
         std::vector<float> h_cdf; std::vector<uint32_t> h_one;
         uint32_t n_nodes8 = 0, n_tris8 = 0; Node8GPU root8{}; bool dev_built = false; std::unique_ptr<GpuBvhBuilder> builder; GpuBuildResult build_info;
         DevBuf d_work_insts; std::vector<FlatInst> h_work; std::vector<uint32_t> pool_dirty;
diff --git a/royaltracer-dx_amd/csrc/rtx_k_bounce_small.hpp b/royaltracer-dx_amd/csrc/rtx_k_bounce_small.hpp
--- a/royaltracer-dx_amd/csrc/rtx_k_bounce_small.hpp
+++ b/royaltracer-dx_amd/csrc/rtx_k_bounce_small.hpp
@@ -144,7 +144,7 @@
                 const uint32_t i = base + threadIdx.x;
                 const bool active = i < n;
                 if (active) S = load_path(p, myq[i]);
-                traverse_small<false>(sc, small, L, S.o, S.d, tmin, active ? kTMax : 0.0f, t, u, v, prim, sc.nsmall, ~0ull, pf, 1);
+                traverse_small<false, true>(sc, small, L, S.o, S.d, tmin, active ? kTMax : 0.0f, t, u, v, prim, sc.nsmall, ~0ull, pf, 1);
                 PF_MARK(2);
                 shade_block<0, LAMBERT, false>(sc, small, L, f, p, T, sh, par, S, sf, t, u, v, prim, active, bounce, nee, last, s_cnt, mynext, 0u, pf);
             }
@@ -168,7 +168,7 @@
                     uint32_t pid = 0; f3 ro = mk3(0, 0, 0), rd = mk3(0, 0, 1);
                     if (act) { pid = myq[i]; const F4 a = p.ray_o[pid], b = p.ray_d[pid]; ro = mk3(a.x, a.y, a.z); rd = mk3(b.x, b.y, b.z); }
                     float ht, hu, hv; uint32_t hp;
-                    traverse_small<false>(sc, small, L, ro, rd, tmin, act ? kTMax : 0.0f, ht, hu, hv, hp, sc.nsmall, ~0ull, pf, 1);
+                    traverse_small<false, true>(sc, small, L, ro, rd, tmin, act ? kTMax : 0.0f, ht, hu, hv, hp, sc.nsmall, ~0ull, pf, 1);
                     const bool hit = act && hp != kMissPrim;
                     const uint32_t slot = prod + block_push(hit, &s_rc[rk]);
                     if (hit) { s_rpid[slot & (kRing - 1u)] = pid; s_rhit[slot & (kRing - 1u)] = {ht, hu, hv, u2f(hp)}; }
diff --git a/royaltracer-dx_amd/csrc/rtx_k_bounce_wave.hpp b/royaltracer-dx_amd/csrc/rtx_k_bounce_wave.hpp
--- a/royaltracer-dx_amd/csrc/rtx_k_bounce_wave.hpp
+++ b/royaltracer-dx_amd/csrc/rtx_k_bounce_wave.hpp
@@ -78,7 +78,7 @@
                 uint32_t pid = 0; f3 ro = mk3(0, 0, 0), rd = mk3(0, 0, 1);
                 if (act) { pid = COMPACT ? i : myq[i]; const uint32_t src = COMPACT ? in0 + i : pid; const F4 a = p.ray_o[src], b = p.ray_d[src]; ro = mk3(a.x, a.y, a.z); rd = mk3(b.x, b.y, b.z); }
                 float ht, hu, hv; uint32_t hp;
-                traverse_small<false>(sc, small, L, ro, rd, tmin, act ? kTMax : 0.0f, ht, hu, hv, hp, sc.nsmall, ~0ull, pf, 1);
+                traverse_small<false, true>(sc, small, L, ro, rd, tmin, act ? kTMax : 0.0f, ht, hu, hv, hp, sc.nsmall, ~0ull, pf, 1);
                 const bool hit = act && hp != kMissPrim;
                 const unsigned long long hmask = __ballot(hit);
                 const uint32_t e = hcnt + __builtin_amdgcn_mbcnt_hi((uint32_t)(hmask >> 32), __builtin_amdgcn_mbcnt_lo((uint32_t)hmask, 0u));
diff --git a/royaltracer-dx_amd/csrc/rtx_k_raygen.hpp b/royaltracer-dx_amd/csrc/rtx_k_raygen.hpp
--- a/royaltracer-dx_amd/csrc/rtx_k_raygen.hpp
+++ b/royaltracer-dx_amd/csrc/rtx_k_raygen.hpp
@@ -87,7 +87,7 @@
         const unsigned long long km = masks[pl >> 6];
         const unsigned long long keep = ((unsigned long long)(uint32_t)__builtin_amdgcn_readfirstlane((int)(uint32_t)(km >> 32)) << 32) | (uint32_t)__builtin_amdgcn_readfirstlane((int)(uint32_t)km);
         float t, u, v; uint32_t prim;
-        traverse_small<false>(sc, small, L, o, d, kTMinCam, valid ? kTMax : 0.0f, t, u, v, prim, sc.nsmall, keep);
+        traverse_small<false, true>(sc, small, L, o, d, kTMinCam, valid ? kTMax : 0.0f, t, u, v, prim, sc.nsmall, keep);
         const bool hit = valid && prim != kMissPrim;
         const unsigned long long hm = __ballot(hit);
         if (lane_id() == 0) p.hitmask[pid >> 6] = hm;
@@ -122,7 +122,7 @@
     f3 o = mk3(0, 0, 0), d = mk3(0, 0, 1);
     if (valid) primary_ray(cam, f.width, f.height, x, y, 0.0f, 0.0f, o, d);
     float t, u, v; uint32_t prim;
-    traverse_small<false>(sc, small, L, o, d, kTMinCam, valid ? kTMax : 0.0f, t, u, v, prim, sc.nsmall, keep);
+    traverse_small<false, true>(sc, small, L, o, d, kTMinCam, valid ? kTMax : 0.0f, t, u, v, prim, sc.nsmall, keep);
     const bool hit = valid && prim != kMissPrim;
     const unsigned long long hm = __ballot(hit);
     const unsigned long long vm = __ballot(valid);
diff --git a/royaltracer-dx_amd/csrc/rtx_kernels.hpp b/royaltracer-dx_amd/csrc/rtx_kernels.hpp
--- a/royaltracer-dx_amd/csrc/rtx_kernels.hpp
+++ b/royaltracer-dx_amd/csrc/rtx_kernels.hpp
@@ -44,6 +44,8 @@
     const int32_t* tri_cut;
     const float* tri_tan;
     const int32_t* map_nrm;
+    const SmallSlabPair* small_slabs;
+    uint32_t small_slab_mask;
 };
 
 struct DevFrame {
diff --git a/royaltracer-dx_amd/csrc/rtx_scene_cache.cpp b/royaltracer-dx_amd/csrc/rtx_scene_cache.cpp
--- a/royaltracer-dx_amd/csrc/rtx_scene_cache.cpp
+++ b/royaltracer-dx_amd/csrc/rtx_scene_cache.cpp
@@ -14,7 +14,7 @@
 namespace {
 
 constexpr char kMagic[8] = {'R', 'T', 'X', 'S', 'C', 'N', '0', '1'};
-constexpr uint32_t kVersion = 3;
+constexpr uint32_t kVersion = 4;
 struct Header { char magic[8]; uint32_t version, endian; uint32_t layout[8]; uint64_t payload, checksum, nsections; };
 struct SecHead { uint32_t tag, elem; uint64_t count; };
 static_assert(sizeof(Header) == 72 && sizeof(SecHead) == 16, "cache header layout");
@@ -22,7 +22,7 @@
 
 void fill_layout(uint32_t l[8]) {
     l[0] = sizeof(Node8GPU); l[1] = sizeof(TriGPU); l[2] = sizeof(TriShade); l[3] = sizeof(MatGPU);
-    l[4] = sizeof(InstGPU); l[5] = sizeof(LightGPU); l[6] = sizeof(SmallRecPair); l[7] = sizeof(InstHost);
+    l[4] = sizeof(InstGPU); l[5] = sizeof(LightGPU); l[6] = sizeof(SmallRecPair) | (uint32_t)(sizeof(SmallSlabPair) << 16); l[7] = sizeof(InstHost);
 }
 
 constexpr size_t kChunk = 4u << 20;
@@ -75,7 +75,7 @@
     }
     template <class T> void vec(uint32_t tag, const std::vector<T>& v) { raw(tag, (uint32_t)sizeof(T), v.size(), v.data()); }
 };
-struct Scalars { uint32_t stack8, small_nrec, small_nocc, max_depth, nmesh, has_cam, pad1, pad2; float bvh_pad, small_cm, small_delta, small_hull_margin, total_weight, f0, f1, f2;
+struct Scalars { uint32_t stack8, small_nrec, small_nocc, max_depth, nmesh, has_cam, small_slab_mask, pad2; float bvh_pad, small_cm, small_delta, small_hull_margin, total_weight, f0, f1, f2;
                  float cam[12]; };
 
 struct Reader {
@@ -97,7 +97,7 @@
 };
 
 enum : uint32_t { T_SCAL = 1, T_MATS128, T_MATIDS, T_INSTH, T_MESHV, T_MESHI, T_MESHB, T_BMATS, T_NODES8, T_SLOTS8, T_TRIS8, T_LEVELS, T_SMALLR, T_SMALLT, T_SMALLP,
-                T_SHADE, T_BINST, T_LIGHTS, T_LIGHTS80, T_AUXREC, T_AUXTXT };
+                T_SHADE, T_BINST, T_LIGHTS, T_LIGHTS80, T_AUXREC, T_AUXTXT, T_SMALLS, T_SMALLX };
 
 }
 
@@ -105,14 +105,14 @@
     if (!path || !*path) { err = "scene cache: empty path"; return false; }
     if (H.topo_dirty || H.mats_dirty || B.tris8.size() < B.shade.size() || B.tris8.size() != B.tri_slots8.size() || (!B.tris8.empty() && B.nodes8.empty())) { err = "scene cache: scene not built"; return false; }
     Writer w;
-    Scalars sc{}; sc.stack8 = B.stack8; sc.small_nrec = B.small_nrec; sc.small_nocc = B.small_nocc; sc.max_depth = B.max_depth; sc.nmesh = (uint32_t)H.meshes.size();
+    Scalars sc{}; sc.stack8 = B.stack8; sc.small_nrec = B.small_nrec; sc.small_nocc = B.small_nocc; sc.max_depth = B.max_depth; sc.nmesh = (uint32_t)H.meshes.size(); sc.small_slab_mask = B.small_slab_mask;
     sc.bvh_pad = B.bvh_pad; sc.small_cm = B.small_cm; sc.small_delta = B.small_delta; sc.small_hull_margin = B.small_hull_margin; sc.total_weight = B.total_weight;
     if (cam12) { sc.has_cam = 1; memcpy(sc.cam, cam12, sizeof(sc.cam)); }
     w.raw(T_SCAL, sizeof(Scalars), 1, &sc);
     w.vec(T_MATS128, H.mats128); w.vec(T_MATIDS, H.matids); w.vec(T_INSTH, H.insts);
     for (const MeshHost& m : H.meshes) { w.vec(T_MESHV, m.verts); w.vec(T_MESHI, m.idx); w.raw(T_MESHB, 4, 1, &m.matid_base); }
     w.vec(T_BMATS, B.mats); w.vec(T_NODES8, B.nodes8); w.vec(T_SLOTS8, B.tri_slots8); w.vec(T_TRIS8, B.tris8); w.vec(T_LEVELS, B.level_start8);
-    w.vec(T_SMALLR, B.small_recs); w.vec(T_SMALLT, B.small_tris); w.vec(T_SMALLP, B.small_poly);
+    w.vec(T_SMALLR, B.small_recs); w.vec(T_SMALLT, B.small_tris); w.vec(T_SMALLP, B.small_poly); w.vec(T_SMALLS, B.small_slabs); w.vec(T_SMALLX, B.small_excess);
     w.vec(T_SHADE, B.shade); w.vec(T_BINST, B.insts); w.vec(T_LIGHTS, B.lights); w.vec(T_LIGHTS80, B.lights80);
     const CacheAux none;
     const CacheAux& ax = aux ? *aux : none;
@@ -161,7 +161,7 @@
         memcpy(&m.matid_base, r.p + r.at, 4); r.at += 16;
     }
     if (!r.vec(T_BMATS, Bn.mats) || !r.vec(T_NODES8, Bn.nodes8) || !r.vec(T_SLOTS8, Bn.tri_slots8) || !r.vec(T_TRIS8, Bn.tris8) || !r.vec(T_LEVELS, Bn.level_start8) ||
-        !r.vec(T_SMALLR, Bn.small_recs) || !r.vec(T_SMALLT, Bn.small_tris) || !r.vec(T_SMALLP, Bn.small_poly) || !r.vec(T_SHADE, Bn.shade) || !r.vec(T_BINST, Bn.insts) ||
+        !r.vec(T_SMALLR, Bn.small_recs) || !r.vec(T_SMALLT, Bn.small_tris) || !r.vec(T_SMALLP, Bn.small_poly) || !r.vec(T_SMALLS, Bn.small_slabs) || !r.vec(T_SMALLX, Bn.small_excess) || !r.vec(T_SHADE, Bn.shade) || !r.vec(T_BINST, Bn.insts) ||
         !r.vec(T_LIGHTS, Bn.lights) || !r.vec(T_LIGHTS80, Bn.lights80)) return false;
     CacheAux ax;
     {
@@ -179,6 +179,7 @@
     bool ok = nrefs >= nt && Bn.tri_slots8.size() == nrefs && Bn.mats.size() == nmat && Bn.insts.size() == Hn.insts.size() && Bn.lights80.size() == Bn.lights.size() * 20 &&
               Hn.mats128.size() % 32 == 0 && (Bn.nodes8.empty() || Bn.level_start8.size() >= 2) && sc.small_nocc <= sc.small_nrec && sc.small_nrec <= kSmallSceneMaxTris &&
               Bn.small_recs.size() * 2 >= nrec_pad && (sc.small_nrec == 0 || (Bn.small_tris.size() >= nrec_pad * 2 && Bn.small_poly.size() >= nrec_pad * 4)) &&
+              Bn.small_slabs.size() == Bn.small_recs.size() && (nrec_pad >= 64 || (sc.small_slab_mask >> (nrec_pad / 2)) == 0u) &&
               nrefs < (1u << 31);
     for (uint32_t id : Hn.matids) ok = ok && id < nmat;
     for (const MeshHost& m : Hn.meshes) {
@@ -225,7 +226,7 @@
         if (nn) levels.push_back((uint32_t)nn);
         if (stack8 != sc.stack8 || (nn && levels != Bn.level_start8)) { err = "scene cache: stack depth / level table do not match the nodes"; return false; }
     }
-    Bn.stack8 = sc.stack8; Bn.small_nrec = sc.small_nrec; Bn.small_nocc = sc.small_nocc; Bn.max_depth = sc.max_depth; Bn.bvh_pad = sc.bvh_pad;
+    Bn.stack8 = sc.stack8; Bn.small_nrec = sc.small_nrec; Bn.small_nocc = sc.small_nocc; Bn.small_slab_mask = sc.small_slab_mask; Bn.max_depth = sc.max_depth; Bn.bvh_pad = sc.bvh_pad;
     Bn.small_cm = sc.small_cm; Bn.small_delta = sc.small_delta; Bn.small_hull_margin = sc.small_hull_margin; Bn.total_weight = sc.total_weight; Bn.refit_count = 0;
     Bn.any_order = probe_anyhit_order(Bn);
     Hn.topo_dirty = false; Hn.mats_dirty = false;
diff --git a/royaltracer-dx_amd/csrc/rtx_scene_host.cpp b/royaltracer-dx_amd/csrc/rtx_scene_host.cpp
--- a/royaltracer-dx_amd/csrc/rtx_scene_host.cpp
+++ b/royaltracer-dx_amd/csrc/rtx_scene_host.cpp
@@ -342,7 +342,7 @@
 static void forget_tree(BuiltScene& B, uint32_t nt) {
     B.shade.clear(); B.shade.shrink_to_fit(); B.objtris.clear(); B.objtris.shrink_to_fit();
     B.bvh_pad = 2e-6f; B.nodes.clear(); B.nodes8.clear(); B.tri_slots8.clear(); B.tris8.clear(); B.tris.clear(); B.leaf_order.clear(); B.level_start8.clear();
-    B.small_recs.clear(); B.small_tris.clear(); B.small_poly.clear(); B.small_nrec = 0; B.small_nocc = 0; B.built_tris = nt; B.refit_count = 0; B.any_order = 0;
+    B.small_recs.clear(); B.small_tris.clear(); B.small_poly.clear(); B.small_slabs.clear(); B.small_excess.clear(); B.small_slab_mask = 0; B.small_nrec = 0; B.small_nocc = 0; B.built_tris = nt; B.refit_count = 0; B.any_order = 0;
 }
 
 bool SceneHost::prepare_device_build(BuiltScene& B) {
@@ -445,7 +445,7 @@
     if (!wide_from_binary(B, bvh)) { err = "build: BVH collapse failed"; return false; }
     sw.lap("collapse_bvh8");
     B.maps_active = maps_active(); B.cutouts_active = cutouts_active(); B.normals_active = normals_active(); B.env_active = env.n != 0;
-    if (B.any_hidden || B.maps_active || B.cutouts_active || B.normals_active || B.env_active) { B.small_recs.clear(); B.small_tris.clear(); B.small_poly.clear(); B.small_nrec = 0; B.small_nocc = 0; }
+    if (B.any_hidden || B.maps_active || B.cutouts_active || B.normals_active || B.env_active) { B.small_recs.clear(); B.small_tris.clear(); B.small_poly.clear(); B.small_slabs.clear(); B.small_excess.clear(); B.small_slab_mask = 0; B.small_nrec = 0; B.small_nocc = 0; }
     else build_small_scene(B, wtri, scale);
     sw.lap("tris8 / small scene");
     B.any_order = probe_anyhit_order(B);
diff --git a/royaltracer-dx_amd/csrc/rtx_scene_host.hpp b/royaltracer-dx_amd/csrc/rtx_scene_host.hpp
--- a/royaltracer-dx_amd/csrc/rtx_scene_host.hpp
+++ b/royaltracer-dx_amd/csrc/rtx_scene_host.hpp
@@ -29,6 +29,8 @@
     std::vector<TriGPU>   tris;
     std::vector<SmallRecPair> small_recs; std::vector<TriGPU> small_tris; uint32_t small_nrec = 0;
     std::vector<F4> small_poly;
+    std::vector<SmallSlabPair> small_slabs; uint32_t small_slab_mask = 0;
+    std::vector<float> small_excess;
     uint32_t small_nocc = 0;
     float small_cm = 0.0f, small_delta = 0.0f;
     float small_hull_margin = 0.0f;
diff --git a/royaltracer-dx_amd/csrc/rtx_small_scene.cpp b/royaltracer-dx_amd/csrc/rtx_small_scene.cpp
--- a/royaltracer-dx_amd/csrc/rtx_small_scene.cpp
+++ b/royaltracer-dx_amd/csrc/rtx_small_scene.cpp
@@ -125,6 +125,49 @@
     recs = occ; recs.insert(recs.end(), hull.begin(), hull.end());
 }
 
+constexpr double kSlabTau = 0.02;
+struct Slab { bool quad = false; double excess = -1.0; float w[2][3] = {{0, 0, 0}, {0, 0, 0}}, c[2] = {0, 0}, h[2] = {-1e30f, -1e30f}; };
+Slab slab_of_quad(const Rec& R, double delta) {
+    Slab S;
+    if (R.s1 < 0) return S;
+    D3 p[4]; for (int k = 0; k < 4; k++) p[k] = D3{R.pv[k][0], R.pv[k][1], R.pv[k][2]};
+    const D3 nu{R.pl[0], R.pl[1], R.pl[2]};
+    const double area = 0.5 * fabs(dt(crs(sub(p[2], p[0]), sub(p[3], p[1])), nu));
+    if (!(area > 0.0)) return S;
+    int best_k = -1; double best = 0.0;
+    for (int k = 0; k < 4; k++) {
+        double width[2];
+        for (int s = 0; s < 2; s++) {
+            const double* m = R.e[(k + s) & 3];
+            double lo = 1e300, hi = -1e300;
+            for (int v = 0; v < 4; v++) { const double q = m[0] * p[v].x + m[1] * p[v].y + m[2] * p[v].z; lo = std::min(lo, q); hi = std::max(hi, q); }
+            width[s] = hi - lo;
+        }
+        const double* m0 = R.e[k]; const double* m1 = R.e[(k + 1) & 3];
+        const double sn = fabs(dt(crs(D3{m0[0], m0[1], m0[2]}, D3{m1[0], m1[1], m1[2]}), nu));
+        if (!(sn > 1e-9)) continue;
+        const double ex = width[0] * width[1] / sn / area - 1.0;
+        if (best_k < 0 || ex < best) { best_k = k; best = ex; }
+    }
+    if (best_k < 0) return S;
+    S.quad = true; S.excess = std::max(best, 0.0);
+    for (int s = 0; s < 2; s++) {
+        const double* m = R.e[(best_k + s) & 3];
+        for (int a = 0; a < 3; a++) S.w[s][a] = (float)m[a];
+        double lo = 1e300, hi = -1e300, mag = 0.0;
+        for (int v = 0; v < 4; v++) {
+            const double q = (double)S.w[s][0] * p[v].x + (double)S.w[s][1] * p[v].y + (double)S.w[s][2] * p[v].z;
+            lo = std::min(lo, q); hi = std::max(hi, q);
+            mag = std::max(mag, fabs((double)S.w[s][0] * p[v].x) + fabs((double)S.w[s][1] * p[v].y) + fabs((double)S.w[s][2] * p[v].z));
+        }
+        S.c[s] = (float)(0.5 * (lo + hi));
+        const double half = std::max(hi - (double)S.c[s], (double)S.c[s] - lo);
+        const double pad = 2e-6 * (mag + fabs((double)S.c[s]) + half + delta);
+        S.h[s] = std::nextafterf((float)(half + delta + pad), INFINITY);
+    }
+    return S;
+}
+
 void pack_records(BuiltScene& B, const std::vector<Rec>& recs, double delta) {
     B.small_nrec = (uint32_t)recs.size();
     B.small_tris.assign(((recs.size() + 1) & ~(size_t)1) * 2, TriGPU{{0, 0, 0, u2f(kMissPrim)}, {0, 0, 0, 0}, {0, 0, 0, 0}});
@@ -145,12 +188,24 @@
         }
         B.small_recs.push_back(P);
     }
+    B.small_excess.assign(recs.size(), -1.0f);
+    for (size_t r = 0; r < recs.size(); r += 2) {
+        SmallSlabPair Q; bool both = true;
+        for (int e = 0; e < 2; e++) {
+            const bool have = r + e < recs.size();
+            const Slab S = have ? slab_of_quad(recs[r + e], delta) : Slab{};
+            if (have) { B.small_excess[r + e] = (float)S.excess; both = both && S.quad && S.excess <= kSlabTau; }
+            for (int s = 0; s < 2; s++) { for (int a = 0; a < 3; a++) Q.r[5 * s + a][e] = S.w[s][a]; Q.r[5 * s + 3][e] = S.c[s]; Q.r[5 * s + 4][e] = S.h[s]; }
+        }
+        if (both) B.small_slab_mask |= 1u << (r / 2);
+        B.small_slabs.push_back(Q);
+    }
 }
 }
 
 void build_small_scene(BuiltScene& B, const std::vector<float>& wtri, float scale) {
     const std::vector<uint32_t>& leaf_order = B.leaf_order;
-    B.small_recs.clear(); B.small_tris.clear(); B.small_poly.clear(); B.small_nrec = 0; B.small_nocc = 0;
+    B.small_recs.clear(); B.small_tris.clear(); B.small_poly.clear(); B.small_slabs.clear(); B.small_excess.clear(); B.small_slab_mask = 0; B.small_nrec = 0; B.small_nocc = 0;
     if (leaf_order.empty() || leaf_order.size() > kSmallSceneMaxTris) return;
     const double delta = 2e-5 * (double)scale, tol = 1e-6 * (double)scale;
     B.small_delta = (float)delta; B.small_cm = 4e-6f * scale; B.small_hull_margin = 2e-6f * scale;
diff --git a/royaltracer-dx_amd/csrc/rtx_traverse.hpp b/royaltracer-dx_amd/csrc/rtx_traverse.hpp
--- a/royaltracer-dx_amd/csrc/rtx_traverse.hpp
+++ b/royaltracer-dx_amd/csrc/rtx_traverse.hpp
@@ -37,6 +37,8 @@
     asm("v_fma_f32 %0, |%1|, %2, %3" : "=v"(r) : "v"(ind), "s"(cm), "v"(a));
     return r;
 }
+__device__ __forceinline__ float slab_slack(float h, float a) { return h - fabsf(a); }
+typedef const __attribute__((address_space(4))) f2v const_f2v;
 typedef uint32_t v2u __attribute__((ext_vector_type(2)));
 typedef uint32_t v4u __attribute__((ext_vector_type(4)));
 typedef __attribute__((address_space(3))) v2u lds_u2;
@@ -250,7 +252,7 @@
 }
 
 
-template <bool ANY>
+template <bool ANY, bool OPEN = false>
 __device__ __forceinline__ void traverse_small(const DevScene& sc, const SmallRecPair* __restrict__ sp, const TraceLds& L, f3 o, f3 d, float tmin, float tmax,
                                                float& bt, float& bu, float& bv, uint32_t& bprim, uint32_t nrec, unsigned long long keep = ~0ull, Prof* pf = nullptr, int pf_sec = 0) {
     bt = tmax; bu = 0.0f; bv = 0.0f; bprim = kMissPrim;
@@ -259,6 +261,7 @@
     const f2v dx = splat2(d.x), dy = splat2(d.y), dz = splat2(d.z), ox = splat2(o.x), oy = splat2(o.y), oz = splat2(o.z);
     const f2v vtmin = splat2(tmin), vtmax = splat2(tmax);
     const float cm = sc.small_cm;
+    const uint32_t slabs = sc.small_slab_mask;
     uint32_t near = ~0u;
     auto pair = [&](uint32_t kp, uint32_t& acc) {
         const f2v* __restrict__ R = (const f2v*)sp[kp].r;
@@ -267,14 +270,23 @@
         f2v ind; ind.x = __builtin_amdgcn_rcpf(nd.x); ind.y = __builtin_amdgcn_rcpf(nd.y);
         const f2v t = no * ind;
         const f2v px = fma2(t, dx, ox), py = fma2(t, dy, oy), pz = fma2(t, dz, oz);
-        const f2v e0 = fma2(R[6], pz, fma2(R[5], py, R[4] * px)) + R[7];
-        const f2v e1 = fma2(R[10], pz, fma2(R[9], py, R[8] * px)) + R[11];
-        const f2v e2 = fma2(R[14], pz, fma2(R[13], py, R[12] * px)) + R[15];
-        const f2v e3 = fma2(R[18], pz, fma2(R[17], py, R[16] * px)) + R[19];
         f2v mt; mt.x = margin_t(cm, ind.x, t.x); mt.y = margin_t(cm, ind.y, t.y);
-        const f2v a0 = (t + mt) - vtmin, a1 = (vtmax + mt) - t;
-        const float ma0 = fminf(a0.x, a1.x), ma1 = fminf(a0.y, a1.y);
-        const float me0 = fminf(e0.x, fminf(fminf(e1.x, e2.x), e3.x)), me1 = fminf(e0.y, fminf(fminf(e1.y, e2.y), e3.y));
+        float me0, me1;
+        if ((slabs >> kp) & 1u) {
+            const const_f2v* S = (const const_f2v*)sc.small_slabs[kp].r;
+            const f2v a = fma2(S[2], pz, fma2(S[1], py, S[0] * px)) - S[3];
+            const f2v b = fma2(S[7], pz, fma2(S[6], py, S[5] * px)) - S[8];
+            me0 = fminf(slab_slack(S[4].x, a.x), slab_slack(S[9].x, b.x)); me1 = fminf(slab_slack(S[4].y, a.y), slab_slack(S[9].y, b.y));
+        } else {
+            const f2v e0 = fma2(R[6], pz, fma2(R[5], py, R[4] * px)) + R[7];
+            const f2v e1 = fma2(R[10], pz, fma2(R[9], py, R[8] * px)) + R[11];
+            const f2v e2 = fma2(R[14], pz, fma2(R[13], py, R[12] * px)) + R[15];
+            const f2v e3 = fma2(R[18], pz, fma2(R[17], py, R[16] * px)) + R[19];
+            me0 = fminf(e0.x, fminf(fminf(e1.x, e2.x), e3.x)); me1 = fminf(e0.y, fminf(fminf(e1.y, e2.y), e3.y));
+        }
+        const f2v a0 = (t + mt) - vtmin;
+        float ma0 = a0.x, ma1 = a0.y;
+        if (!OPEN) { const f2v a1 = (vtmax + mt) - t; ma0 = fminf(a0.x, a1.x); ma1 = fminf(a0.y, a1.y); }
         const unsigned long long c0 = (__builtin_amdgcn_ballot_w64(ma0 >= 0.0f) & __builtin_amdgcn_ballot_w64(me0 >= -mt.x)) | __builtin_amdgcn_ballot_w64(fabsf(nd.x) < 1e-3f);
         const unsigned long long c1 = (__builtin_amdgcn_ballot_w64(ma1 >= 0.0f) & __builtin_amdgcn_ballot_w64(me1 >= -mt.y)) | __builtin_amdgcn_ballot_w64(fabsf(nd.y) < 1e-3f);
         acc = shift_in(shift_in(acc, c1), c0);
@@ -296,6 +308,7 @@
     }
     RTX_PROF_MARK(pf, pf_sec);
     unsigned long long cand = ((unsigned long long)cand_hi << 32) | cand_lo;
+    if (OPEN && !(tmax > 0.0f)) cand = 0ull;
     cand &= nrec >= 64u ? ~0ull : ((1ull << nrec) - 1ull);
     auto exact = [&](uint32_t k) -> bool {
         RTX_PROF_COUNT(pf, pf_sec + 1);
diff --git a/royaltracer-dx_amd/csrc/rtx_types.hpp b/royaltracer-dx_amd/csrc/rtx_types.hpp
--- a/royaltracer-dx_amd/csrc/rtx_types.hpp
+++ b/royaltracer-dx_amd/csrc/rtx_types.hpp
@@ -17,6 +17,8 @@
 
 struct alignas(16) SmallRecPair { float r[20][2]; };
 static_assert(sizeof(SmallRecPair) == 160, "SmallRecPair must be 160 bytes");
+struct alignas(16) SmallSlabPair { float r[10][2]; };
+static_assert(sizeof(SmallSlabPair) == 80, "SmallSlabPair must be 80 bytes");
 constexpr uint32_t kSmallSceneMaxTris = 64;
 
 struct alignas(16) TriShade {
diff --git a/royaltracer-dx_amd/host/rtx_host_c.cpp b/royaltracer-dx_amd/host/rtx_host_c.cpp
--- a/royaltracer-dx_amd/host/rtx_host_c.cpp
+++ b/royaltracer-dx_amd/host/rtx_host_c.cpp
@@ -356,6 +356,17 @@
     }
     return RTX_OK;
 }
+int rtxh_scene_small_slabs(const rtxh_scene* sc, float* slabs10, float* excess, uint32_t max_recs, uint32_t* nrec_out, uint32_t* pair_mask_out) {
+    rtx::BuiltScene B;
+    if (!slabs10 || !excess || !build_for_inspection(sc, B)) return RTX_ERR_INVALID;
+    if (nrec_out) *nrec_out = B.small_nrec;
+    if (pair_mask_out) *pair_mask_out = B.small_slab_mask;
+    for (uint32_t r = 0; r < B.small_nrec && r < max_recs; r++) {
+        for (int row = 0; row < 10; row++) slabs10[(size_t)r * 10 + row] = B.small_slabs[r / 2].r[row][r & 1];
+        excess[r] = B.small_excess[r];
+    }
+    return RTX_OK;
+}
 
 rtxh_renderer* rtxh_renderer_create(uint32_t w, uint32_t h, const char* name, int device) {
     rtxh_renderer* r = new rtxh_renderer(); r->r = new Renderer(w, h, name ? name : "rtx"); r->r->SetDevice(device); return r;
```

Measured after the change: 42360 Mrays/s, median of 6. 4.1% higher.
